# Guoxs/DODT

Measured on AMD Instinct MI355X. Metric: frame-pairs/sec (whole node) KITTI-shape tau=2, higher is better.
Workload: dtype f32

## Files before the change

dodt_amd/_lib.py:

```python
import ctypes as C
import os

_HERE = os.path.dirname(os.path.abspath(__file__))
LIB_PATH = os.environ.get('DODT_HIP_LIB') or os.path.join(_HERE, 'lib', 'libdodt_hip.so')

OK, ERR_INVALID, ERR_HIP, ERR_UNSUPPORTED = 0, 1, 2, 3
PTS_VELO_XYZI, PTS_CAM_3XN = 0, 1
EXTRACTOR_VGG_PYR = 0
EXTRACTOR_VGG = 1
EXTRACTOR_SHARED_GPU = 0x100
EXTRACTOR_BF16 = 0x200
EXTRACTOR_SPLIT = 0x400
FC_RELU = 1
FC_BF16 = 2
CONFLICT_RAISE, CONFLICT_NEXT_BEST = 0, 1


class DodtError(RuntimeError):
    pass


class BevParams(C.Structure):
    _fields_ = [
        ('point_format', C.c_int32),
        ('num_slices', C.c_int32),
        ('velo_to_cam', C.c_double * 12),
        ('p2', C.c_double * 12),
        ('im_w', C.c_double),
        ('im_h', C.c_double),
        ('plane', C.c_double * 4),
        ('extents', C.c_double * 6),
        ('voxel_size', C.c_double),
        ('height_lo', C.c_double),
        ('height_hi', C.c_double),
        ('occ_lo', C.c_double),
        ('occ_hi', C.c_double),
        ('has_pre_transform', C.c_int32),
        ('reserved_', C.c_int32),
        ('pre_translate', C.c_double * 3),
        ('pre_rotate', C.c_double * 9),
    ]


class LayerInfo(C.Structure):
    _fields_ = [('name', C.c_char * 32), ('kernel', C.c_char * 48), ('launches', C.c_int32),
                ('items', C.c_int32), ('flops_direct', C.c_double), ('flops_executed', C.c_double),
                ('bytes', C.c_double), ('ms', C.c_float), ('reserved_', C.c_int32)]


_vp = C.c_void_p
_i = C.c_int
_f = C.c_float
_d = C.c_double
_pi32 = C.c_void_p
_pf = C.c_void_p
_hf = C.c_void_p

SIGNATURES = {
    'dodt_version': (_i, []),
    'dodt_last_error': (C.c_char_p, []),
    'dodt_ctx_create': (_i, [_i, C.POINTER(_vp)]),
    'dodt_mark': (_i, [_vp, _i]),
    'dodt_ctx_wait_mark': (_i, [_vp, _vp, _i]),
    'dodt_mark_elapsed': (_i, [_vp, _i, _vp, _i, C.POINTER(_f)]),
    'dodt_ctx_create_high_priority': (_i, [_i, C.POINTER(_vp)]),
    'dodt_ctx_create_on_stream': (_i, [_i, _vp, C.POINTER(_vp)]),
    'dodt_ctx_destroy': (_i, [_vp]),
    'dodt_ctx_sync': (_i, [_vp]),
    'dodt_ctx_wait_for': (_i, [_vp, _vp]),
    'dodt_malloc': (_i, [_vp, C.c_size_t, C.POINTER(_vp)]),
    'dodt_free': (_i, [_vp, _vp]),
    'dodt_memcpy_h2d': (_i, [_vp, _vp, _vp, C.c_size_t]),
    'dodt_memcpy_d2h': (_i, [_vp, _vp, _vp, C.c_size_t]),
    'dodt_memset': (_i, [_vp, _vp, _i, C.c_size_t]),
    'dodt_pinned_alloc': (_i, [_vp, C.c_size_t, C.POINTER(_vp)]),
    'dodt_pinned_free': (_i, [_vp, _vp]),
    'dodt_memcpy_h2d_async': (_i, [_vp, _vp, _vp, C.c_size_t]),
    'dodt_fetch_i32_begin': (_i, [_vp, _pi32, _i, _i]),
    'dodt_fetch_i32_end': (_i, [_vp, _i, C.POINTER(C.c_int32), _i]),
    'dodt_timer_start': (_i, [_vp]),
    'dodt_timer_stop': (_i, [_vp, C.POINTER(_f)]),
    'dodt_bev_slices': (_i, [_vp, _vp, _i, C.POINTER(BevParams), _pf, _vp]),
    'dodt_bev_status': (_i, [_vp, C.POINTER(_i)]),
    'dodt_bev_support_mask': (_i, [C.POINTER(BevParams), _i, _vp, _i, _i]),
    'dodt_anchor_filter': (_i, [_vp, _vp, _i, _i, _pi32, _i, _i, _pi32, _pi32]),
    'dodt_project_anchors_f64': (_i, [_vp, _vp, _pi32, _i, _pi32,
                                      C.POINTER(_d), C.POINTER(_d), _d, _d,
                                      _pf, _pf, _pf]),
    'dodt_project_anchors_f32': (_i, [_vp, _pf, _i, _pi32, C.POINTER(_f),
                                      C.POINTER(_f), _f, _f, _pf, _pf, _pf]),
    'dodt_img_preprocess': (_i, [_vp, _vp, _i, _i, _i, _i, _i,
                                 C.POINTER(_f), _pf]),
    'dodt_conv_mode': (_i, []),
    'dodt_extractor_create': (_i, [_vp, _i, _i, _i, _i, _i, _i,
                                   C.POINTER(_vp)]),
    'dodt_extractor_destroy': (_i, [_vp]),
    'dodt_extractor_set_layer': (_i, [_vp, C.c_char_p, _vp, _i, _i, _i, _i,
                                      _vp, _vp, _vp]),
    'dodt_extractor_input': (_i, [_vp, C.POINTER(_vp), C.POINTER(C.c_longlong)]),
    'dodt_extractor_forward': (_i, [_vp, _pf, _pf, _pf]),
    'dodt_extractor_forward_padded': (_i, [_vp, _pf, _pf, _pf]),
    'dodt_extractor_set_input': (_i, [_vp, _pf]),
    'dodt_extractor_set_input_support': (_i, [_vp, _vp, _i, _i, C.POINTER(C.c_longlong)]),
    'dodt_extractor_set_frame_tables': (_i, [_vp, _i, C.POINTER(_i)]),
    'dodt_extractor_frame_items': (_i, [_vp, C.POINTER(_i), _i]),
    'dodt_extractor_frame_split': (_i, [_vp, C.POINTER(_i), C.POINTER(_i), _i]),
    'dodt_extractor_store_bytes': (C.c_longlong, [_vp]),
    'dodt_frame_tables_host': (_i, [_vp, _i, _i, _i, _i, _i, _i, _vp, _i, _vp, _vp, C.POINTER(_i)]),
    'dodt_frame_restore_host': (_i, [_vp, _i, _i, _i, _i, _i, _i, _i, _i, _i, _vp, _vp, _vp, _vp]),
    'dodt_frame_lists_host': (_i, [_vp, _i, _i, _i, _i, _i, _i, _vp, _i, _vp, _vp, C.POINTER(_i), _vp, C.POINTER(_i)]),
    'dodt_extractor_read_activation': (_i, [_vp, C.c_char_p, _vp,
                                            C.POINTER(_i), C.POINTER(_i),
                                            C.POINTER(_i)]),
    'dodt_extractor_output_shape': (_i, [_vp, C.POINTER(_i), C.POINTER(_i), C.POINTER(_i)]),
    'dodt_extractor_first_layers_folded': (_i, [_vp]),
    'dodt_extractor_flops': (_d, [_vp]),
    'dodt_extractor_mfma_flops': (_d, [_vp]),
    'dodt_extractor_bytes': (_d, [_vp]),
    'dodt_extractor_layer_count': (_i, [_vp]),
    'dodt_extractor_forward_timed': (_i, [_vp, _pf, _pf, _pf, C.POINTER(LayerInfo), _i]),
    'dodt_crop_and_resize': (_i, [_vp, _pf, _i, _i, _i, _pf, _i, _pi32, _i, _i,
                                  _pf]),
    'dodt_crop_and_resize_strided': (_i, [_vp, _pf, _i, _i, _i, _pf, _i, _pi32, _i, _i, _pf,
                                          C.c_longlong]),
    'dodt_correlation': (_i, [_vp, _pf, _pf, _i, _i, _i, _i, _i, _i, _pf]),
    'dodt_mean_fusion': (_i, [_vp, _pf, _pf, _i, _pi32, _i, _pf]),
    'dodt_fc_create': (_i, [_vp, _i, _i, _hf, _hf, _i, C.POINTER(_vp)]),
    'dodt_fc_create_ex': (_i, [_vp, _i, _i, _hf, _hf, _i, C.POINTER(_vp)]),
    'dodt_fc_destroy': (_i, [_vp]),
    'dodt_fc_forward': (_i, [_vp, _vp, _pf, _pf, _i, _i, _pi32, _pf, _i]),
    'dodt_fc_forward_split': (_i, [_vp, _vp, _pf, _i, _i, _pi32, _i, C.POINTER(_i), C.POINTER(_vp)]),
    'dodt_fc_flops': (_d, [_vp, _i]),
    'dodt_fc_bf16_row_elems': (_i, [_vp]),
    'dodt_fc_forward_bf16': (_i, [_vp, _vp, _vp, _i, _i, _pi32, _vp, _i, _i]),
    'dodt_fc_forward_split_bf16': (_i, [_vp, _vp, _vp, _i, _i, _pi32, _i, C.POINTER(_i), C.POINTER(_vp)]),
    'dodt_rows_to_bf16': (_i, [_vp, _pf, _pf, _i, _pi32, _i, _i, _vp, _i]),
    'dodt_nms': (_i, [_vp, _pf, _pf, _i, _pi32, _i, _f, _pi32, _pi32]),
    'dodt_offset_to_anchor': (_i, [_vp, _pf, _pf, _i, _pi32, _pf]),
    'dodt_softmax_fg': (_i, [_vp, _pf, _i, _pi32, _pf]),
    'dodt_rpn_decode': (_i, [_vp, _pf, _pf, _pf, _i, _pi32, C.POINTER(_f), _pf, _pf, _pf]),
    'dodt_gather_project': (_i, [_vp, _pf, _pi32, _i, _pi32, C.POINTER(_f), C.POINTER(_f), _f, _f, _pf, _pf, _pf]),
    'dodt_final_decode': (_i, [_vp, _pf, _pf, _pf, _pf, _i, _pi32, C.POINTER(_f), C.POINTER(_f),
                               _pf, _pf, _pf, _pf, _pf, _pf]),
    'dodt_gather_rows': (_i, [_vp, _pf, _i, _pi32, _i, _pi32, _pf]),
    'dodt_max_fg_logit': (_i, [_vp, _pf, _i, _i, _pi32, _pf]),
    'dodt_pack_detections': (_i, [_vp, _pf, _pf, _pf, _pf, _pi32, _pi32, _i, _f, _pf, _pi32]),
    'dodt_angle_vector_to_orientation': (_i, [_vp, _pf, _i, _pi32, _pf]),
    'dodt_box_4c_decode': (_i, [_vp, _pf, _pf, _i, _pi32, C.POINTER(_f),
                                C.POINTER(_f), _pf, _pf, _pf]),
    'dodt_comm_unique_id': (_i, [_vp]),
    'dodt_comm_create': (_i, [_vp, _i, _i, _vp, C.POINTER(_vp)]),
    'dodt_comm_destroy': (_i, [_vp]),
    'dodt_comm_attach': (_i, [_vp, _vp]),
    'dodt_comm_rank': (_i, [_vp, C.POINTER(_i), C.POINTER(_i)]),
    'dodt_comm_set_late_peer': (_i, [_vp, _d]),
    'dodt_all_gather_records': (_i, [_vp, _vp, _i, _pf, _pi32, _i, _i, _i, _i, _pf, _pi32]),
    'dodt_comm_join': (_i, [_vp, _i, _vp]),
    'dodt_comm_sync': (_i, [_vp]),
    'dodt_comm_barrier': (_i, [_vp]),
    'dodt_comm_max_f64': (_i, [_vp, C.POINTER(_d)]),
    'dodt_three_d_iou_matrix': (_i, [_vp, _vp, _i, _vp, _i, _vp]),
    'dodt_interpolate_pairs': (_i, [_vp, _vp, _i, _pi32, _i, _i, _i, _d, _i, _vp, C.POINTER(_d), _i, _vp,
                                    _pi32, _pi32]),
    'dodt_track_state_bytes': (_i, [_i, C.POINTER(C.c_size_t)]),
    'dodt_track_reset': (_i, [_vp, _vp, _i]),
    'dodt_track_flush': (_i, [_vp, _vp, _d, _i]),
    'dodt_track_encode': (_i, [_vp, _vp, _i, _pi32, _i, _i, C.POINTER(_d), _d, _d, _d, _pf, _pf, _pi32]),
    'dodt_track_pairs': (_i, [_vp, _vp, _vp, _i, _pi32, _i, _i, C.POINTER(_d), _d, _d, _d, _d, _d, _i]),
    'dodt_track_encoded': (_i, [_vp, _vp, _pf, _pf, _pi32, _i, _i, _d, _d, _i]),
}
COMM_ID_BYTES = 128

_lib = None


def load():
    global _lib
    if _lib is not None:
        return _lib
    if not os.path.exists(LIB_PATH):
        raise DodtError(
            'libdodt_hip.so not found at %s -- build it with '
            '`make -C dodt_amd/csrc` (there is no CPU fallback)' % LIB_PATH)
    lib = C.CDLL(LIB_PATH)
    for name, (res, args) in SIGNATURES.items():
        fn = getattr(lib, name)
        fn.restype = res
        fn.argtypes = args
    _lib = lib
    return lib


def check(rc, what=''):
    if rc == OK:
        return
    msg = load().dodt_last_error().decode('utf-8', 'replace')
    if rc == ERR_INVALID:
        raise ValueError(msg or what)
    raise DodtError('%s: %s (status %d)' % (what, msg, rc))
```

dodt_amd/csrc/anchors.hip:

```cpp
#include "common.h"

namespace {

__device__ __forceinline__ int box_count(const uint32_t* __restrict__ occ, int wpr, int x1,
                                         int z1, int x2, int z2, int thr) {
    int cnt = 0;
    if (x2 <= x1) return 0;
    const int w0 = x1 >> 5, w1 = (x2 - 1) >> 5;
    for (int z = z1; z < z2; ++z) {
        for (int w = w0; w <= w1; ++w) {
            uint32_t word = occ[z * wpr + w];
            const int lo = (w == w0) ? (x1 & 31) : 0;
            const int hi = (w == w1) ? ((x2 - 1) & 31) : 31;
            uint32_t m = (hi == 31 ? 0xFFFFFFFFu : ((1u << (hi + 1)) - 1u)) & ~((1u << lo) - 1u);
            cnt += __popc(word & m);
        }
        if (cnt >= thr) return cnt;
    }
    return cnt;
}

constexpr int kMaskBlock = 64;
__global__ void __launch_bounds__(kMaskBlock)
anchor_mask_kernel(const uint32_t* __restrict__ occ, int wpr, int nx, int nz,
                   const int4* __restrict__ cells, int n, int thr,
                   uint8_t* __restrict__ mask, int* __restrict__ block_counts) {
    const int i = blockIdx.x * blockDim.x + threadIdx.x;
    int keep = 0;
    if (i < n) {
        int4 b = cells[i];
        const int x1 = min(max(b.x, 0), nx), z1 = min(max(b.y, 0), nz);
        const int x2 = min(max(b.z, 0), nx), z2 = min(max(b.w, 0), nz);
        keep = box_count(occ, wpr, x1, z1, x2, z2, thr) >= thr;
        mask[i] = (uint8_t)keep;
    }
    const int total = __popcll(__ballot(keep));
    if (threadIdx.x == 0) block_counts[blockIdx.x] = total;
}

__global__ void __launch_bounds__(256)
anchor_compact_kernel(const uint8_t* __restrict__ mask, const int* __restrict__ block_counts,
                      int n, int* __restrict__ keep_idx, int* __restrict__ count_out) {
    __shared__ int s_part[256];
    __shared__ int s_wave[4];
    const int tid = threadIdx.x;
    int part = 0;
    for (int j = tid; j < (int)blockIdx.x * (256 / kMaskBlock); j += 256) part += block_counts[j];
    s_part[tid] = part;
    __syncthreads();
    for (int s = 128; s > 0; s >>= 1) {
        if (tid < s) s_part[tid] += s_part[tid + s];
        __syncthreads();
    }
    const int block_off = s_part[0];
    const int i = blockIdx.x * 256 + tid;
    const int keep = (i < n) ? mask[i] : 0;
    const unsigned long long bal = __ballot(keep);
    const int lane = tid & 63, wave = tid >> 6;
    const int before = __popcll(bal & ((1ull << lane) - 1ull));
    if (lane == 0) s_wave[wave] = __popcll(bal);
    __syncthreads();
    int wave_off = 0;
    for (int w = 0; w < wave; ++w) wave_off += s_wave[w];
    if (keep) keep_idx[block_off + wave_off + before] = i;
    if (blockIdx.x == gridDim.x - 1 && tid == 0)
        *count_out = block_off + s_wave[0] + s_wave[1] + s_wave[2] + s_wave[3];
}

struct ProjParams64 {
    double x_min, x_max, z_min, z_max;
    double p[12];
    double im_w, im_h;
};

__device__ __forceinline__ void proj_corner64(const double* p, double x, double y, double z,
                                              double& u, double& v) {
    const double un = fma(p[2], z, fma(p[1], y, p[0] * x)) + p[3];
    const double vn = fma(p[6], z, fma(p[5], y, p[4] * x)) + p[7];
    const double w = fma(p[10], z, fma(p[9], y, p[8] * x)) + p[11];
    u = un / w;
    v = vn / w;
}

__global__ void __launch_bounds__(256)
project_f64_kernel(const double* __restrict__ anchors, const int* __restrict__ idx, int n,
                   const int* __restrict__ d_n, const ProjParams64 P,
                   float* __restrict__ bev_norm, float* __restrict__ img_norm,
                   float* __restrict__ anchors_f32) {
    const int i = blockIdx.x * blockDim.x + threadIdx.x;
    const int lim = d_n ? min(*d_n, n) : n;
    if (i >= lim) return;
    const int row = idx ? idx[i] : i;
    const double* a = anchors + (size_t)row * 6;
    const double x = a[0], y = a[1], z = a[2], dx = a[3], dy = a[4], dz = a[5];
    if (anchors_f32) {
        float* o = anchors_f32 + (size_t)i * 6;
        o[0] = (float)x; o[1] = (float)y; o[2] = (float)z;
        o[3] = (float)dx; o[4] = (float)dy; o[5] = (float)dz;
    }
    const double hx = dx / 2.0, hz = dz / 2.0;
    if (bev_norm) {
        const double xr = P.x_max - P.x_min, zr = P.z_max - P.z_min;
        const double x1 = (x - hx) - P.x_min, x2 = (x + hx) - P.x_min;
        const double z1 = (P.z_max - (z + hz)) - P.z_min, z2 = (P.z_max - (z - hz)) - P.z_min;
        float* o = bev_norm + (size_t)i * 4;
        o[0] = (float)(z1 / zr); o[1] = (float)(x1 / xr);
        o[2] = (float)(z2 / zr); o[3] = (float)(x2 / xr);
    }
    if (img_norm) {
        double umin = 1e300, umax = -1e300, vmin = 1e300, vmax = -1e300;
        const double xs[2] = {x + hx, x - hx};
        const double ys[2] = {y, y - dy};
        const double zs[2] = {z + hz, z - hz};
#pragma unroll
        for (int k = 0; k < 8; ++k) {
            double u, v;
            proj_corner64(P.p, xs[(k >> 1) & 1], ys[k >> 2], zs[((k + 1) >> 1) & 1], u, v);
            umin = (u < umin || u != u) ? u : umin; umax = (u > umax || u != u) ? u : umax;
            vmin = (v < vmin || v != v) ? v : vmin; vmax = (v > vmax || v != v) ? v : vmax;
        }
        float* o = img_norm + (size_t)i * 4;
        o[0] = (float)(vmin / P.im_h); o[1] = (float)(umin / P.im_w);
        o[2] = (float)(vmax / P.im_h); o[3] = (float)(umax / P.im_w);
    }
}

struct ProjParams32 {
    float x_min, x_max, z_min, z_max;
    float p[12];
    float im_w, im_h;
};

__device__ __forceinline__ void bev_box32(float x, float z, float dx, float dz,
                                          const ProjParams32& P, float& x1, float& z1,
                                          float& x2, float& z2) {
    const float hx = dx / 2.0f, hz = dz / 2.0f;
    x1 = (x - hx) - P.x_min;
    x2 = (x + hx) - P.x_min;
    z1 = (P.z_max - (z + hz)) - P.z_min;
    z2 = (P.z_max - (z - hz)) - P.z_min;
}

__device__ __forceinline__ void project_f32_elem(int i, float x, float y, float z, float dx, float dy, float dz,
                                                 const ProjParams32& P, float* __restrict__ bev,
                                                 float* __restrict__ bev_norm_tf, float* __restrict__ img_norm_tf) {
    float x1, z1, x2, z2;
    bev_box32(x, z, dx, dz, P, x1, z1, x2, z2);
    if (bev) {
        float* o = bev + (size_t)i * 4;
        o[0] = x1; o[1] = z1; o[2] = x2; o[3] = z2;
    }
    if (bev_norm_tf) {
        const float xr = P.x_max - P.x_min, zr = P.z_max - P.z_min;
        float* o = bev_norm_tf + (size_t)i * 4;
        o[0] = z1 / zr; o[1] = x1 / xr; o[2] = z2 / zr; o[3] = x2 / xr;
    }
    if (img_norm_tf) {
        const float hx = dx / 2.0f, hz = dz / 2.0f;
        const float xs[2] = {x + hx, x - hx};
        const float ys[2] = {y, y - dy};
        const float zs[2] = {z + hz, z - hz};
        float umin = 3.0e38f, umax = -3.0e38f, vmin = 3.0e38f, vmax = -3.0e38f;
#pragma unroll
        for (int k = 0; k < 8; ++k) {
            const float cx = xs[(k >> 1) & 1], cy = ys[k >> 2], cz = zs[((k + 1) >> 1) & 1];
            const float un = ((P.p[0] * cx + P.p[1] * cy) + P.p[2] * cz) + P.p[3];
            const float vn = ((P.p[4] * cx + P.p[5] * cy) + P.p[6] * cz) + P.p[7];
            const float w = ((P.p[8] * cx + P.p[9] * cy) + P.p[10] * cz) + P.p[11];
            const float u = un / w, v = vn / w;
            umin = fminf(umin, u); umax = fmaxf(umax, u);
            vmin = fminf(vmin, v); vmax = fmaxf(vmax, v);
        }
        float* o = img_norm_tf + (size_t)i * 4;
        o[0] = vmin / P.im_h; o[1] = umin / P.im_w; o[2] = vmax / P.im_h; o[3] = umax / P.im_w;
    }
}

__global__ void __launch_bounds__(256)
project_f32_kernel(const float* __restrict__ anchors, int n, const int* __restrict__ d_n,
                   const ProjParams32 P, float* __restrict__ bev, float* __restrict__ bev_norm_tf,
                   float* __restrict__ img_norm_tf) {
    const int i = blockIdx.x * blockDim.x + threadIdx.x;
    const int lim = d_n ? min(*d_n, n) : n;
    if (i >= lim) return;
    const float* a = anchors + (size_t)i * 6;
    project_f32_elem(i, a[0], a[1], a[2], a[3], a[4], a[5], P, bev, bev_norm_tf, img_norm_tf);
}

__device__ __forceinline__ void offset_to_anchor_elem(const float* __restrict__ a, const float* __restrict__ t, float o[6]) {
    o[0] = (t[0] * a[3]) + a[0];
    o[1] = (t[1] * a[4]) + a[1];
    o[2] = (t[2] * a[5]) + a[2];
    o[3] = expf(logf(a[3]) + t[3]);
    o[4] = expf(logf(a[4]) + t[4]);
    o[5] = expf(logf(a[5]) + t[5]);
}

__global__ void __launch_bounds__(256)
offset_to_anchor_kernel(const float* __restrict__ anchors, const float* __restrict__ off, int n,
                        const int* __restrict__ d_n, float* __restrict__ out) {
    const int i = blockIdx.x * blockDim.x + threadIdx.x;
    const int lim = d_n ? min(*d_n, n) : n;
    if (i >= lim) return;
    float o[6];
    offset_to_anchor_elem(anchors + (size_t)i * 6, off + (size_t)i * 6, o);
#pragma unroll
    for (int k = 0; k < 6; ++k) out[(size_t)i * 6 + k] = o[k];
}

__device__ __forceinline__ float softmax_fg_elem(float l0, float l1) {
    const float m = fmaxf(l0, l1);
    const float e0 = expf(l0 - m), e1 = expf(l1 - m);
    return e1 / (e0 + e1);
}

__global__ void __launch_bounds__(256)
softmax_fg_kernel(const float* __restrict__ logits, int n, const int* __restrict__ d_n,
                  float* __restrict__ out) {
    const int i = blockIdx.x * blockDim.x + threadIdx.x;
    const int lim = d_n ? min(*d_n, n) : n;
    if (i >= lim) return;
    out[i] = softmax_fg_elem(logits[2 * (size_t)i], logits[2 * (size_t)i + 1]);
}

__global__ void __launch_bounds__(256)
rpn_decode_kernel(const float* __restrict__ anchors, const float* __restrict__ off, const float* __restrict__ logits,
                  int n, const int* __restrict__ d_n, const ProjParams32 P, float* __restrict__ regressed,
                  float* __restrict__ bev_norm_tf, float* __restrict__ scores) {
    const int i = blockIdx.x * blockDim.x + threadIdx.x;
    const int lim = d_n ? min(*d_n, n) : n;
    if (i >= lim) return;
    float o[6];
    offset_to_anchor_elem(anchors + (size_t)i * 6, off + (size_t)i * 6, o);
#pragma unroll
    for (int k = 0; k < 6; ++k) regressed[(size_t)i * 6 + k] = o[k];
    project_f32_elem(i, o[0], o[1], o[2], o[3], o[4], o[5], P, nullptr, bev_norm_tf, nullptr);
    scores[i] = softmax_fg_elem(logits[2 * (size_t)i], logits[2 * (size_t)i + 1]);
}

__global__ void __launch_bounds__(256)
gather_project_kernel(const float* __restrict__ src, const int* __restrict__ idx, int n, const int* __restrict__ d_n,
                      const ProjParams32 P, float* __restrict__ rows, float* __restrict__ bev_norm_tf,
                      float* __restrict__ img_norm_tf) {
    const int i = blockIdx.x * blockDim.x + threadIdx.x;
    const int lim = d_n ? min(*d_n, n) : n;
    if (i >= lim) return;
    const float* a = src + (size_t)idx[i] * 6;
    float o[6];
#pragma unroll
    for (int k = 0; k < 6; ++k) { o[k] = a[k]; rows[(size_t)i * 6 + k] = o[k]; }
    project_f32_elem(i, o[0], o[1], o[2], o[3], o[4], o[5], P, nullptr, bev_norm_tf, img_norm_tf);
}

__global__ void __launch_bounds__(256)
gather_rows_kernel(const float* __restrict__ src, int width, const int* __restrict__ idx, int n,
                   const int* __restrict__ d_n, float* __restrict__ out) {
    const int t = blockIdx.x * blockDim.x + threadIdx.x;
    const int lim = d_n ? min(*d_n, n) : n;
    const int i = t / width, c = t - i * width;
    if (i >= lim) return;
    out[(size_t)i * width + c] = src[(size_t)idx[i] * width + c];
}

__global__ void __launch_bounds__(256)
max_fg_logit_kernel(const float* __restrict__ logits, int n_cls, int n,
                    const int* __restrict__ d_n, float* __restrict__ out) {
    const int i = blockIdx.x * blockDim.x + threadIdx.x;
    const int lim = d_n ? min(*d_n, n) : n;
    if (i >= lim) return;
    float m = logits[(size_t)i * n_cls + 1];
    for (int c = 2; c < n_cls; ++c) m = fmaxf(m, logits[(size_t)i * n_cls + c]);
    out[i] = m;
}

__device__ __forceinline__ void orientation_correct(float b[7], float ori) {
    const float kPi = (float)M_PI, kTwoPi = (float)(2.0 * M_PI);
    const float q1 = (float)(0.25 * M_PI), q2 = (float)(0.50 * M_PI), q3 = (float)(0.75 * M_PI);
    float diff = b[6] - ori;
    if (diff < -kPi) diff += kTwoPi;
    if (diff > kPi) diff -= kTwoPi;
    const bool pos = q1 < diff && diff < q3;
    const bool neg = -q1 > diff && diff > -q3;
    if (pos || neg) {
        const float l = b[3];
        b[3] = b[4];
        b[4] = l;
    }
    if (pos) b[6] += q2;
    if (neg) b[6] -= q2;
    if (fabsf(diff) >= q3) b[6] += kPi;
    if (b[6] > kPi) b[6] -= kTwoPi;
}

__global__ void __launch_bounds__(256)
pack_detections_kernel(const float* __restrict__ boxes_3d, const float* __restrict__ scores,
                       const float* __restrict__ orientations, const float* __restrict__ corr,
                       const int* __restrict__ sel, const int* __restrict__ d_count, int max_det,
                       float frame_mark, float* __restrict__ rec, int* __restrict__ count_out) {
    const int t = blockIdx.x * blockDim.x + threadIdx.x;
    const int cnt = min(*d_count, max_det);
    if (t == 0) *count_out = cnt;
    if (t >= max_det * 17) return;
    const int row = t / 17, col = t - row * 17;
    float v = 0.0f;
    if (row < cnt) {
        const int src = sel[row];
        if (col == 7) v = scores[src];
        else if (col == 16) v = frame_mark;
        else if (col < 7 || (col >= 9 && corr)) {
            float b[7];
#pragma unroll
            for (int k = 0; k < 7; ++k) b[k] = boxes_3d[(size_t)src * 7 + k];
            if (orientations) orientation_correct(b, orientations[src]);
            if (col >= 9) {
                b[0] += corr[(size_t)src * 3 + 0];
                b[2] += corr[(size_t)src * 3 + 1];
                b[6] += corr[(size_t)src * 3 + 2];
            }
            const int c = col < 7 ? col : col - 9;
#pragma unroll
            for (int k = 0; k < 7; ++k)
                if (k == c) v = b[k];
        }
    }
    rec[t] = v;
}

__global__ void __launch_bounds__(256)
angle_vector_to_orientation_kernel(const float* __restrict__ vec, int n,
                                   const int* __restrict__ d_n, float* __restrict__ out) {
    const int i = blockIdx.x * blockDim.x + threadIdx.x;
    if (d_n) n = min(n, *d_n);
    if (i < n) out[i] = atan2f(vec[2 * i + 1], vec[2 * i]);
}

__device__ __forceinline__ void box_info32(float vx, float vz, float mag, const float* px,
                                           const float* pz, float mx, float mz, float& cx,
                                           float& cz, float& len, float& wid, float& ry) {
    const float nx = vx / mag, nz = vz / mag;
    const float ox = -nz, oz = nx;
    float lmin = 3.0e38f, lmax = -3.0e38f, wmin = 3.0e38f, wmax = -3.0e38f;
#pragma unroll
    for (int k = 0; k < 4; ++k) {
        const float rx = px[k] - mx, rz = pz[k] - mz;
        const float l = rx * nx + rz * nz;
        const float w = rx * ox + rz * oz;
        lmin = fminf(lmin, l); lmax = fmaxf(lmax, l);
        wmin = fminf(wmin, w); wmax = fmaxf(wmax, w);
    }
    len = lmax - lmin;
    wid = wmax - wmin;
    const float wdiff = wmax + wmin;
    ry = -atan2f(vz, vx);
    const float half = (lmin + lmax);
    cx = (mx + (nx * half) / 2.0f) + ox * wdiff;
    cz = (mz + (nz * half) / 2.0f) + oz * wdiff;
}

struct DecodeParams {
    float a, b, c, d;
    float x_min, x_max, z_min, z_max;
};

__device__ __forceinline__ void box_4c_decode_elem(int i, const float* __restrict__ top_anchors,
                                                   const float* __restrict__ offsets, const DecodeParams& P,
                                                   float* __restrict__ boxes_3d, float* __restrict__ pred_anchors,
                                                   float* __restrict__ bev_tf) {
    const float* a = top_anchors + (size_t)i * 6;
    const float half_pi = (float)(M_PI / 2);
    float bx = a[0], by = a[1], bz = a[2];
    float bl = a[3], bw = a[5], bh = a[4], bry = 0.0f;
    if (bw > bl) { const float t = bl; bl = bw; bw = t; bry = -half_pi; }
    float ortho = rintf(bry / half_pi) * half_pi;
    float co = fabsf(cosf(ortho)), si = fabsf(sinf(ortho));
    const float dimx = bl * co + bw * si, dimy = bh, dimz = bw * co + bl * si;
    const float hx = dimx / 2, hz = dimz / 2;
    const float diff = bry - ortho;
    const float cd = cosf(diff), sd = sinf(diff);
    const float xs[4] = {hx, hx, -hx, -hx};
    const float zs[4] = {hz, -hz, -hz, hz};
    float px[4], pz[4];
    const float* t = offsets + (size_t)i * 10;
#pragma unroll
    for (int k = 0; k < 4; ++k) {
        px[k] = ((cd * xs[k] + sd * zs[k]) + bx) + t[k];
        pz[k] = (((-sd) * xs[k] + cd * zs[k]) + bz) + t[4 + k];
    }
    const float gy = -((P.a * bx + P.c * bz) + P.d) / P.b;
    const float h1 = (gy - by) + t[8];
    const float h2 = ((gy - by) + dimy) + t[9];
    const float m12x = (px[0] + px[1]) / 2.0f, m12z = (pz[0] + pz[1]) / 2.0f;
    const float m23x = (px[1] + px[2]) / 2.0f, m23z = (pz[1] + pz[2]) / 2.0f;
    const float m34x = (px[2] + px[3]) / 2.0f, m34z = (pz[2] + pz[3]) / 2.0f;
    const float m14x = (px[0] + px[3]) / 2.0f, m14z = (pz[0] + pz[3]) / 2.0f;
    const float vax = m12x - m34x, vaz = m12z - m34z;
    const float vbx = m14x - m23x, vbz = m14z - m23z;
    const float ma = sqrtf(vax * vax + vaz * vaz), mb = sqrtf(vbx * vbx + vbz * vbz);
    float cax, caz, la, wa, ra, cbx, cbz, lb, wb, rb;
    box_info32(vax, vaz, ma, px, pz, m34x, m34z, cax, caz, la, wa, ra);
    box_info32(vbx, vbz, mb, px, pz, m23x, m23z, cbx, cbz, lb, wb, rb);
    const float fa = (ma > mb) ? 1.0f : 0.0f, fb = 1.0f - fa;
    const float cx = cax * fa + cbx * fb, cz = caz * fa + cbz * fb;
    const float len = la * fa + lb * fb, wid = wa * fa + wb * fb, ry = ra * fa + rb * fb;
    const float gy2 = -((P.a * cx + P.c * cz) + P.d) / P.b;
    const float cy = gy2 - h1, hgt = h2 - h1;
    if (boxes_3d) {
        float* o = boxes_3d + (size_t)i * 7;
        o[0] = cx; o[1] = cy; o[2] = cz; o[3] = len; o[4] = wid; o[5] = hgt; o[6] = ry;
    }
    ortho = rintf(ry / half_pi) * half_pi;
    co = fabsf(cosf(ortho));
    si = fabsf(sinf(ortho));
    const float adx = len * co + wid * si, adz = wid * co + len * si;
    if (pred_anchors) {
        float* o = pred_anchors + (size_t)i * 6;
        o[0] = cx; o[1] = cy; o[2] = cz; o[3] = adx; o[4] = hgt; o[5] = adz;
    }
    if (bev_tf) {
        const float ahx = adx / 2.0f, ahz = adz / 2.0f;
        const float x1 = (cx - ahx) - P.x_min, x2 = (cx + ahx) - P.x_min;
        const float z1 = (P.z_max - (cz + ahz)) - P.z_min, z2 = (P.z_max - (cz - ahz)) - P.z_min;
        float* o = bev_tf + (size_t)i * 4;
        o[0] = z1; o[1] = x1; o[2] = z2; o[3] = x2;
    }
}

__global__ void __launch_bounds__(256)
box_4c_decode_kernel(const float* __restrict__ top_anchors, const float* __restrict__ offsets,
                     int n, const int* __restrict__ d_n, const DecodeParams P,
                     float* __restrict__ boxes_3d, float* __restrict__ pred_anchors,
                     float* __restrict__ bev_tf) {
    const int i = blockIdx.x * blockDim.x + threadIdx.x;
    const int lim = d_n ? min(*d_n, n) : n;
    if (i >= lim) return;
    box_4c_decode_elem(i, top_anchors, offsets, P, boxes_3d, pred_anchors, bev_tf);
}

__global__ void __launch_bounds__(256)
final_decode_kernel(const float* __restrict__ top_anchors, const float* __restrict__ offsets,
                    const float* __restrict__ cls_logits, const float* __restrict__ angle_vec, int n,
                    const int* __restrict__ d_n, const DecodeParams P, float* __restrict__ boxes_3d,
                    float* __restrict__ pred_anchors, float* __restrict__ bev_tf, float* __restrict__ nms_scores,
                    float* __restrict__ det_scores, float* __restrict__ orientations) {
    const int i = blockIdx.x * blockDim.x + threadIdx.x;
    const int lim = d_n ? min(*d_n, n) : n;
    if (i >= lim) return;
    box_4c_decode_elem(i, top_anchors, offsets, P, boxes_3d, pred_anchors, bev_tf);
    const float l0 = cls_logits[2 * (size_t)i], l1 = cls_logits[2 * (size_t)i + 1];
    nms_scores[i] = l1;
    det_scores[i] = softmax_fg_elem(l0, l1);
    if (orientations) orientations[i] = atan2f(angle_vec[2 * i + 1], angle_vec[2 * i]);
}

}

extern "C" {

int dodt_anchor_filter(dodt_ctx* ctx, const uint32_t* d_occ_bits, int nx, int nz,
                       const int32_t* d_anchor_cells, int n_anchors, int density_threshold,
                       int32_t* d_keep_idx_out, int32_t* d_count_out) {
    DODT_REQUIRE(ctx && d_occ_bits && d_anchor_cells && d_keep_idx_out && d_count_out,
                 "dodt_anchor_filter: NULL argument");
    DODT_REQUIRE(nx > 0 && nz > 0 && n_anchors >= 0, "dodt_anchor_filter: bad sizes");
    if (n_anchors == 0) {
        DODT_HIP_CHECK(hipMemsetAsync(d_count_out, 0, sizeof(int32_t), ctx->stream));
        return DODT_OK;
    }
    const int blocks = dodt::ceil_div(n_anchors, 256), mask_blocks = dodt::ceil_div(n_anchors, kMaskBlock);
    const size_t mask_bytes = dodt::align_up((size_t)n_anchors, 256);
    int rc = ctx->anchor_ws.reserve(mask_bytes + (size_t)mask_blocks * sizeof(int));
    if (rc) return rc;
    uint8_t* mask = reinterpret_cast<uint8_t*>(ctx->anchor_ws.ptr);
    int* block_counts = reinterpret_cast<int*>(mask + mask_bytes);
    hipLaunchKernelGGL(anchor_mask_kernel, dim3(mask_blocks), dim3(kMaskBlock), 0, ctx->stream, d_occ_bits,
                       dodt::ceil_div(nx, 32), nx, nz,
                       reinterpret_cast<const int4*>(d_anchor_cells), n_anchors,
                       density_threshold, mask, block_counts);
    DODT_LAUNCH_CHECK();
    hipLaunchKernelGGL(anchor_compact_kernel, dim3(blocks), dim3(256), 0, ctx->stream, mask,
                       block_counts, n_anchors, d_keep_idx_out, d_count_out);
    DODT_LAUNCH_CHECK();
    return DODT_OK;
}

int dodt_project_anchors_f64(dodt_ctx* ctx, const double* d_anchors, const int32_t* d_idx, int n,
                             const int32_t* d_n, const double bev_extents[4],
                             const double p2[12], double im_w, double im_h,
                             float* d_bev_norm_out, float* d_img_norm_out,
                             float* d_anchors_f32_out) {
    DODT_REQUIRE(ctx && d_anchors && bev_extents && p2, "dodt_project_anchors_f64: NULL argument");
    if (n <= 0) return DODT_OK;
    ProjParams64 P;
    P.x_min = bev_extents[0]; P.x_max = bev_extents[1];
    P.z_min = bev_extents[2]; P.z_max = bev_extents[3];
    for (int k = 0; k < 12; ++k) P.p[k] = p2[k];
    P.im_w = im_w; P.im_h = im_h;
    hipLaunchKernelGGL(project_f64_kernel, dim3(dodt::ceil_div(n, 256)), dim3(256), 0,
                       ctx->stream, d_anchors, d_idx, n, d_n, P, d_bev_norm_out, d_img_norm_out,
                       d_anchors_f32_out);
    DODT_LAUNCH_CHECK();
    return DODT_OK;
}

int dodt_project_anchors_f32(dodt_ctx* ctx, const float* d_anchors, int n, const int32_t* d_n,
                             const float bev_extents[4], const float p2[12], float im_w,
                             float im_h, float* d_bev_out, float* d_bev_norm_tf_out,
                             float* d_img_norm_tf_out) {
    DODT_REQUIRE(ctx && d_anchors && bev_extents && p2, "dodt_project_anchors_f32: NULL argument");
    if (n <= 0) return DODT_OK;
    ProjParams32 P;
    P.x_min = bev_extents[0]; P.x_max = bev_extents[1];
    P.z_min = bev_extents[2]; P.z_max = bev_extents[3];
    for (int k = 0; k < 12; ++k) P.p[k] = p2[k];
    P.im_w = im_w; P.im_h = im_h;
    hipLaunchKernelGGL(project_f32_kernel, dim3(dodt::ceil_div(n, 256)), dim3(256), 0,
                       ctx->stream, d_anchors, n, d_n, P, d_bev_out, d_bev_norm_tf_out,
                       d_img_norm_tf_out);
    DODT_LAUNCH_CHECK();
    return DODT_OK;
}

int dodt_rpn_decode(dodt_ctx* ctx, const float* d_anchors, const float* d_offsets, const float* d_logits2, int n,
                    const int32_t* d_n, const float bev_extents[4], float* d_regressed_out,
                    float* d_bev_norm_tf_out, float* d_scores_out) {
    DODT_REQUIRE(ctx && d_anchors && d_offsets && d_logits2 && bev_extents && d_regressed_out && d_bev_norm_tf_out &&
                     d_scores_out, "dodt_rpn_decode: NULL argument");
    if (n <= 0) return DODT_OK;
    ProjParams32 P = {};
    P.x_min = bev_extents[0]; P.x_max = bev_extents[1];
    P.z_min = bev_extents[2]; P.z_max = bev_extents[3];
    hipLaunchKernelGGL(rpn_decode_kernel, dim3(dodt::ceil_div(n, 256)), dim3(256), 0, ctx->stream, d_anchors,
                       d_offsets, d_logits2, n, d_n, P, d_regressed_out, d_bev_norm_tf_out, d_scores_out);
    DODT_LAUNCH_CHECK();
    return DODT_OK;
}

int dodt_gather_project(dodt_ctx* ctx, const float* d_src, const int32_t* d_idx, int n, const int32_t* d_n,
                        const float bev_extents[4], const float p2[12], float im_w, float im_h,
                        float* d_rows_out, float* d_bev_norm_tf_out, float* d_img_norm_tf_out) {
    DODT_REQUIRE(ctx && d_src && d_idx && bev_extents && p2 && d_rows_out && d_bev_norm_tf_out && d_img_norm_tf_out,
                 "dodt_gather_project: NULL argument");
    if (n <= 0) return DODT_OK;
    ProjParams32 P;
    P.x_min = bev_extents[0]; P.x_max = bev_extents[1];
    P.z_min = bev_extents[2]; P.z_max = bev_extents[3];
    for (int k = 0; k < 12; ++k) P.p[k] = p2[k];
    P.im_w = im_w; P.im_h = im_h;
    hipLaunchKernelGGL(gather_project_kernel, dim3(dodt::ceil_div(n, 256)), dim3(256), 0, ctx->stream, d_src, d_idx,
                       n, d_n, P, d_rows_out, d_bev_norm_tf_out, d_img_norm_tf_out);
    DODT_LAUNCH_CHECK();
    return DODT_OK;
}

int dodt_final_decode(dodt_ctx* ctx, const float* d_top_anchors, const float* d_offsets, const float* d_cls_logits2,
                      const float* d_angle_vectors, int n, const int32_t* d_n, const float plane[4],
                      const float bev_extents[4], float* d_boxes_3d_out, float* d_pred_anchors_out,
                      float* d_bev_tf_out, float* d_nms_scores_out, float* d_det_scores_out,
                      float* d_orientations_out) {
    DODT_REQUIRE(ctx && d_top_anchors && d_offsets && d_cls_logits2 && plane && bev_extents && d_nms_scores_out &&
                     d_det_scores_out && (d_angle_vectors != nullptr) == (d_orientations_out != nullptr),
                 "dodt_final_decode: bad argument");
    if (n <= 0) return DODT_OK;
    DecodeParams P;
    P.a = plane[0]; P.b = plane[1]; P.c = plane[2]; P.d = plane[3];
    P.x_min = bev_extents[0]; P.x_max = bev_extents[1];
    P.z_min = bev_extents[2]; P.z_max = bev_extents[3];
    hipLaunchKernelGGL(final_decode_kernel, dim3(dodt::ceil_div(n, 256)), dim3(256), 0, ctx->stream, d_top_anchors,
                       d_offsets, d_cls_logits2, d_angle_vectors, n, d_n, P, d_boxes_3d_out, d_pred_anchors_out,
                       d_bev_tf_out, d_nms_scores_out, d_det_scores_out, d_orientations_out);
    DODT_LAUNCH_CHECK();
    return DODT_OK;
}

int dodt_offset_to_anchor(dodt_ctx* ctx, const float* d_anchors, const float* d_offsets, int n,
                          const int32_t* d_n, float* d_out) {
    DODT_REQUIRE(ctx && d_anchors && d_offsets && d_out, "dodt_offset_to_anchor: NULL argument");
    if (n <= 0) return DODT_OK;
    hipLaunchKernelGGL(offset_to_anchor_kernel, dim3(dodt::ceil_div(n, 256)), dim3(256), 0,
                       ctx->stream, d_anchors, d_offsets, n, d_n, d_out);
    DODT_LAUNCH_CHECK();
    return DODT_OK;
}

int dodt_softmax_fg(dodt_ctx* ctx, const float* d_logits2, int n, const int32_t* d_n,
                    float* d_scores_out) {
    DODT_REQUIRE(ctx && d_logits2 && d_scores_out, "dodt_softmax_fg: NULL argument");
    if (n <= 0) return DODT_OK;
    hipLaunchKernelGGL(softmax_fg_kernel, dim3(dodt::ceil_div(n, 256)), dim3(256), 0,
                       ctx->stream, d_logits2, n, d_n, d_scores_out);
    DODT_LAUNCH_CHECK();
    return DODT_OK;
}

int dodt_gather_rows(dodt_ctx* ctx, const float* d_src, int width, const int32_t* d_idx, int n,
                     const int32_t* d_n, float* d_out) {
    DODT_REQUIRE(ctx && d_src && d_idx && d_out && width > 0, "dodt_gather_rows: bad argument");
    if (n <= 0) return DODT_OK;
    hipLaunchKernelGGL(gather_rows_kernel, dim3(dodt::ceil_div(n * width, 256)), dim3(256), 0,
                       ctx->stream, d_src, width, d_idx, n, d_n, d_out);
    DODT_LAUNCH_CHECK();
    return DODT_OK;
}

int dodt_max_fg_logit(dodt_ctx* ctx, const float* d_logits, int n_cls, int n, const int32_t* d_n,
                      float* d_scores_out) {
    DODT_REQUIRE(ctx && d_logits && d_scores_out && n_cls >= 2, "dodt_max_fg_logit: bad argument");
    if (n <= 0) return DODT_OK;
    hipLaunchKernelGGL(max_fg_logit_kernel, dim3(dodt::ceil_div(n, 256)), dim3(256), 0,
                       ctx->stream, d_logits, n_cls, n, d_n, d_scores_out);
    DODT_LAUNCH_CHECK();
    return DODT_OK;
}

int dodt_pack_detections(dodt_ctx* ctx, const float* d_boxes_3d, const float* d_scores,
                         const float* d_orientations, const float* d_corr_offsets,
                         const int32_t* d_sel, const int32_t* d_count, int max_det,
                         float frame_mark, float* d_rec_out, int32_t* d_count_out) {
    DODT_REQUIRE(ctx && d_boxes_3d && d_scores && d_sel && d_count && d_rec_out && d_count_out &&
                     max_det > 0,
                 "dodt_pack_detections: bad argument");
    hipLaunchKernelGGL(pack_detections_kernel, dim3(dodt::ceil_div(max_det * 17, 256)), dim3(256),
                       0, ctx->stream, d_boxes_3d, d_scores, d_orientations, d_corr_offsets, d_sel,
                       d_count, max_det, frame_mark, d_rec_out, d_count_out);
    DODT_LAUNCH_CHECK();
    return DODT_OK;
}

int dodt_angle_vector_to_orientation(dodt_ctx* ctx, const float* d_angle_vectors, int n,
                                     const int32_t* d_n, float* d_orientations_out) {
    DODT_REQUIRE(ctx && d_angle_vectors && d_orientations_out,
                 "dodt_angle_vector_to_orientation: NULL argument");
    if (n <= 0) return DODT_OK;
    hipLaunchKernelGGL(angle_vector_to_orientation_kernel, dim3(dodt::ceil_div(n, 256)), dim3(256),
                       0, ctx->stream, d_angle_vectors, n, d_n, d_orientations_out);
    DODT_LAUNCH_CHECK();
    return DODT_OK;
}

int dodt_box_4c_decode(dodt_ctx* ctx, const float* d_top_anchors, const float* d_offsets, int n,
                       const int32_t* d_n, const float plane[4], const float bev_extents[4],
                       float* d_boxes_3d_out, float* d_pred_anchors_out, float* d_bev_tf_out) {
    DODT_REQUIRE(ctx && d_top_anchors && d_offsets && plane && bev_extents,
                 "dodt_box_4c_decode: NULL argument");
    if (n <= 0) return DODT_OK;
    DecodeParams P;
    P.a = plane[0]; P.b = plane[1]; P.c = plane[2]; P.d = plane[3];
    P.x_min = bev_extents[0]; P.x_max = bev_extents[1];
    P.z_min = bev_extents[2]; P.z_max = bev_extents[3];
    hipLaunchKernelGGL(box_4c_decode_kernel, dim3(dodt::ceil_div(n, 256)), dim3(256), 0,
                       ctx->stream, d_top_anchors, d_offsets, n, d_n, P, d_boxes_3d_out,
                       d_pred_anchors_out, d_bev_tf_out);
    DODT_LAUNCH_CHECK();
    return DODT_OK;
}

}
```

dodt_amd/csrc/correlation.hip:

```cpp
#include <algorithm>
#include <mutex>
#include <type_traits>
#include <vector>

#include "common.h"
#include "lds_dma.h"

namespace {

constexpr int kTW = 16;
constexpr int kTH = 32;
constexpr int kC = 32;
constexpr int kCH = 16;
constexpr int kPS = kCH + 4;

typedef float f32x4 __attribute__((ext_vector_type(4)));
typedef float f32x2 __attribute__((ext_vector_type(2)));

template <int S2, int CH, int WGS>
__global__ void __launch_bounds__(256, WGS)
correlation_kernel(const float* __restrict__ A, const float* __restrict__ B, int H, int W,
                   int d, int pad, int OH, int OW, int tiles_x, int n_tiles, float* __restrict__ out) {
    constexpr int r = 2, R = r * S2, GW = 2 * r + 1, K = GW * GW, PS = CH + 4;
    constexpr int PW = kTW + 2 * R, PH = kTH + 2 * R;
    static_assert(S2 == 2, "a lane's pixel pair (y, y + 2) shares neighbourhood rows only for stride_2 = 2");
    extern __shared__ __attribute__((aligned(16))) float smem[];
    const int tid = threadIdx.x;
    const int per = (n_tiles + 7) / 8;
    const int tile = (blockIdx.x % 8) * per + blockIdx.x / 8;
    if (tile >= n_tiles) return;
    const int oy0 = (tile / tiles_x) * kTH, ox0 = (tile % tiles_x) * kTW;
    const int shift = d - pad;
    const int l5 = tid & 31;
    const bool grp_a = l5 < 4 || (l5 >= 12 && l5 < 16) || (l5 >= 20 && l5 < 28);
    const int lx = grp_a ? (l5 < 4 ? l5 : l5 < 16 ? l5 - 8 : l5 - 12)
                         : (l5 < 12 ? l5 - 4 : l5 < 20 ? l5 - 8 : l5 - 16);
    const int lr = (tid >> 5) * 2 + (grp_a ? 0 : 1);
    const int ly = 4 * (lr >> 1) + (lr & 1);
    f32x2 res[2][K];
#pragma unroll
    for (int px = 0; px < 2; ++px)
#pragma unroll
        for (int k = 0; k < K; ++k) res[px][k] = f32x2{0.f, 0.f};
#pragma unroll 1
    for (int pass = 0; pass < kC / CH; ++pass) {
        if (pass) __syncthreads();
        f32x4 ah[2][CH / 4];
#pragma unroll
        for (int px = 0; px < 2; ++px) {
            const int ay = oy0 + ly + 2 * px + shift, ax = ox0 + lx + shift;
            const bool in = ay >= 0 && ay < H && ax >= 0 && ax < W;
#pragma unroll
            for (int q = 0; q < CH / 4; ++q) {
                ah[px][q] = f32x4{0.f, 0.f, 0.f, 0.f};
                if (in)
                    ah[px][q] = *reinterpret_cast<const f32x4*>(A + ((size_t)ay * W + ax) * kC + pass * CH + q * 4);
            }
        }
        constexpr int kQuads = PW * PH * (CH / 4), kTrips = (kQuads + 255) / 256, kGroup = kTrips < 8 ? kTrips : 8;
        int stid = tid;
        asm volatile("" : "+v"(stid));
#pragma unroll
        for (int g0 = 0; g0 < kTrips; g0 += kGroup) {
            f32x4 stage[kGroup];
#pragma unroll
            for (int i = 0; i < kGroup; ++i) {
                const int t = stid + 256 * (g0 + i);
                const int q = t % (CH / 4), p = t / (CH / 4);
                const int py = p / PW, pxl = p - py * PW;
                const int gy = oy0 + shift - R + py, gx = ox0 + shift - R + pxl;
                stage[i] = f32x4{0.f, 0.f, 0.f, 0.f};
                if (g0 + i < kTrips && t < kQuads && gy >= 0 && gy < H && gx >= 0 && gx < W)
                    stage[i] = *reinterpret_cast<const f32x4*>(B + ((size_t)gy * W + gx) * kC + pass * CH + q * 4);
            }
#pragma unroll
            for (int i = 0; i < kGroup; ++i) {
                const int t = stid + 256 * (g0 + i);
                const int q = t % (CH / 4), p = t / (CH / 4);
                if (g0 + i < kTrips && t < kQuads)
                    *reinterpret_cast<f32x4*>(smem + p * PS + q * 4) = stage[i];
            }
            __builtin_amdgcn_sched_barrier(0);
        }
        __syncthreads();
#pragma unroll
        for (int tr = 0; tr < GW + 1; ++tr) {
#pragma unroll
            for (int j = 0; j < GW; ++j) {
                const float* b = smem + (ly * PW + lx) * PS + (S2 * tr * PW + S2 * j) * PS;
                f32x4 bv[CH / 4];
#pragma unroll
                for (int q = 0; q < CH / 4; ++q) bv[q] = *reinterpret_cast<const f32x4*>(b + q * 4);
#pragma unroll
                for (int px = 0; px < 2; ++px) {
                    const int krow = tr - px;
                    if (krow < 0 || krow >= GW) continue;
                    f32x2 sum = res[px][krow * GW + j];
#pragma unroll
                    for (int q = 0; q < CH / 4; ++q) {
                        const f32x4 av = ah[px][q];
                        sum = __builtin_elementwise_fma(f32x2{av[0], av[1]}, f32x2{bv[q][0], bv[q][1]}, sum);
                        sum = __builtin_elementwise_fma(f32x2{av[2], av[3]}, f32x2{bv[q][2], bv[q][3]}, sum);
                    }
                    res[px][krow * GW + j] = sum;
                }
            }
            __builtin_amdgcn_sched_barrier(0);
        }
    }
    __syncthreads();
#pragma unroll
    for (int px = 0; px < 2; ++px)
#pragma unroll
        for (int k = 0; k < K; ++k)
            smem[((ly + 2 * px) * kTW + lx) * K + k] = (res[px][k][0] + res[px][k][1]) * (1.0f / (float)kC);
    __syncthreads();
    constexpr int kRow = kTW * K;
    if ((OW * K) % 4 == 0 && kRow % 4 == 0 && ox0 + kTW <= OW) {
        for (int t = tid; t < kTH * (kRow / 4); t += 256) {
            const int row = t / (kRow / 4), off = t - row * (kRow / 4);
            const int y = oy0 + row;
            if (y < OH)
                *reinterpret_cast<f32x4*>(out + ((size_t)y * OW + ox0) * K + off * 4) =
                    *reinterpret_cast<const f32x4*>(smem + row * kRow + off * 4);
        }
    } else {
        for (int t = tid; t < kTH * kRow; t += 256) {
            const int row = t / kRow, off = t - row * kRow;
            const int y = oy0 + row, x = ox0 + off / K;
            if (y < OH && x < OW) out[((size_t)y * OW + ox0) * K + off] = smem[t];
        }
    }
}

constexpr int kSpT = 16;
constexpr int kSpR = 4;
constexpr int kSpP = kSpT + 2 * kSpR;
constexpr int kSpLds = kSpP * kSpP * kC * 4;

template <int HALVES>
__global__ void __launch_bounds__(256 * HALVES, 2 * HALVES)
correlation_sp_kernel(const float* __restrict__ A, const float* __restrict__ B, int H, int W, int d, int pad,
                      int OH, int OW, const int* __restrict__ tile_list, int n_tiles, float* __restrict__ out,
                      int* __restrict__ stamps) {
    constexpr int GW = 5, K = GW * GW, S2 = 2, QH = kC / 4 / HALVES;
    constexpr int NW = 4 * HALVES;
    extern __shared__ __attribute__((aligned(16))) float smem[];
    const int tid = threadIdx.x;
    const bool stamp = stamps != nullptr && blockIdx.x == 9 && tid == 0;
    int n_stamp = 0;
#define CORR_STAMP(i) do { if (stamp && n_stamp < 6) stamps[n_stamp * 8 + (i)] = (int)__builtin_amdgcn_s_memrealtime(); } while (0)
    const int per = (n_tiles + 7) / 8;
    const int xcd = blockIdx.x % 8, wg = blockIdx.x / 8, stride = gridDim.x / 8;
    const int first = xcd * per, last = min(first + per, n_tiles);
    const int shift = d - pad;
    const int lane = tid & 63, wave = tid >> 6;
    const int half = HALVES == 2 ? lane >> 5 : 0;
    const int l5 = lane & 31;
    const bool grp_a = l5 < 4 || (l5 >= 12 && l5 < 16) || (l5 >= 20 && l5 < 28);
    const int lx = grp_a ? (l5 < 4 ? l5 : l5 < 16 ? l5 - 8 : l5 - 12)
                         : (l5 < 12 ? l5 - 4 : l5 < 20 ? l5 - 8 : l5 - 16);
    const int ly = (HALVES == 2 ? wave * 2 : (tid >> 5) * 2) + (grp_a ? 0 : 1);
    const dodt::i32x4_t rsrc = dodt::make_rsrc(B, (unsigned)((size_t)H * W * kC * 4));

    auto load_a = [&](int oy0, int ox0, f32x4 (&ah)[QH]) {
        const int ay = oy0 + ly + shift, ax = ox0 + lx + shift;
        const bool in = ay >= 0 && ay < H && ax >= 0 && ax < W;
#pragma unroll
        for (int q = 0; q < QH; ++q) {
            ah[q] = f32x4{0.f, 0.f, 0.f, 0.f};
            if (in) ah[q] = *reinterpret_cast<const f32x4*>(A + ((size_t)ay * W + ax) * kC + (half * QH + q) * 4);
        }
    };
    constexpr int kOutCopies = (kSpT * kSpT * K * 4 + 1023) / 1024;
    auto stage_b = [&](int oy0, int ox0, auto part) {
        constexpr int PART = decltype(part)::value;
        int slane = lane;
        asm volatile("" : "+v"(slane));
#pragma unroll
        for (int k = 0; k < (kSpP * kSpP * 8 / 64) / NW; ++k) {
            const int j = wave + NW * k;
            if (PART == 1 && j < kOutCopies) continue;
            if (PART == 2 && j >= kOutCopies) continue;
            const int s = j * 64 + slane;
            const int p = s >> 3, q = (s & 7) ^ ((p >> 1) & 7);
            const int py = p / kSpP, px = p - py * kSpP;
            const int gy = oy0 + shift - kSpR + py, gx = ox0 + shift - kSpR + px;
            const bool ok = gy >= 0 && gy < H && gx >= 0 && gx < W;
            dodt::blds16(rsrc, ok ? ((gy * W + gx) * kC + q * 4) * 4 : dodt::kOob, 0, smem + j * 256);
        }
    };
    using All = std::integral_constant<int, 0>;
    using Early = std::integral_constant<int, 1>;
    using Late = std::integral_constant<int, 2>;
    int slot = first + wg;
    if (slot >= last) return;
    int tile = tile_list[slot];
    f32x4 ah[QH];
    load_a((tile >> 16) * kSpT, (tile & 0xffff) * kSpT, ah);
    stage_b((tile >> 16) * kSpT, (tile & 0xffff) * kSpT, All{});
    const int p0_lane = ly * kSpP + lx;
    while (true) {
        const int oy0 = (tile >> 16) * kSpT, ox0 = (tile & 0xffff) * kSpT;
        int p0 = p0_lane;
        asm volatile("" : "+v"(p0));
        const char* lane_base = reinterpret_cast<const char*>(smem) + p0 * (kC * 4);
        CORR_STAMP(0);
        __builtin_amdgcn_s_waitcnt(0);
        CORR_STAMP(1);
        __syncthreads();
        CORR_STAMP(2);
        const int nslot = slot + stride;
        const bool more = nslot < last;
        const int ntile = more ? tile_list[nslot] : 0;
        f32x4 an[QH];
        if (more) load_a((ntile >> 16) * kSpT, (ntile & 0xffff) * kSpT, an);
        f32x2 res[K];
#pragma unroll
        for (int k = 0; k < K; ++k) res[k] = f32x2{0.f, 0.f};
        f32x4 bv[2][QH];
        auto read_step = [&](int st, f32x4 (&dst)[QH]) {
            const int j = st / GW, i = st % GW;
            const int sj = ((p0 >> 1) + j) & 7;
#pragma unroll
            for (int q = 0; q < QH; ++q)
                dst[q] = *reinterpret_cast<const f32x4*>(lane_base + (((half * QH + q) ^ sj) << 4) + S2 * j * (kC * 4) +
                                                         S2 * i * kSpP * (kC * 4));
        };
        read_step(0, bv[0]);
#pragma unroll
        for (int st = 0; st < K; ++st) {
            if (st + 1 < K) read_step(st + 1, bv[(st + 1) & 1]);
            __builtin_amdgcn_sched_barrier(0);
            const int j = st / GW, i = st % GW;
            float s0 = res[i * GW + j][0], s1 = res[i * GW + j][1];
#pragma unroll
            for (int q = 0; q < QH; ++q) {
                s0 = __builtin_fmaf(ah[q][0], bv[st & 1][q][0], s0);
                s1 = __builtin_fmaf(ah[q][1], bv[st & 1][q][1], s1);
                s0 = __builtin_fmaf(ah[q][2], bv[st & 1][q][2], s0);
                s1 = __builtin_fmaf(ah[q][3], bv[st & 1][q][3], s1);
            }
            res[i * GW + j] = f32x2{s0, s1};
            __builtin_amdgcn_sched_barrier(0);
        }
        float tot[K];
#pragma unroll
        for (int k = 0; k < K; ++k) {
            tot[k] = res[k][0] + res[k][1];
            if (HALVES == 2) {
                const float other = __shfl_xor(tot[k], 32, 64);
                tot[k] = half == 0 ? tot[k] + other : other + tot[k];
            }
        }
#pragma unroll
        for (int k = 0; k < K; ++k) asm volatile("" : "+v"(tot[k]));
        CORR_STAMP(3);
        __syncthreads();
        CORR_STAMP(4);
        if (more) stage_b((ntile >> 16) * kSpT, (ntile & 0xffff) * kSpT, Early{});
        if (half == 0) {
#pragma unroll
            for (int k = 0; k < K; ++k) smem[(ly * kSpT + lx) * K + k] = tot[k] * (1.0f / (float)kC);
        }
        __syncthreads();
        CORR_STAMP(5);
        {
            constexpr int kRow = kSpT * K;
            if ((OW * K) % 4 == 0 && ox0 + kSpT <= OW) {
                for (int t = tid; t < kSpT * (kRow / 4); t += 256 * HALVES) {
                    const int row = t / (kRow / 4), off = t - row * (kRow / 4);
                    const int y = oy0 + row;
                    if (y < OH)
                        *reinterpret_cast<f32x4*>(out + ((size_t)y * OW + ox0) * K + off * 4) =
                            *reinterpret_cast<const f32x4*>(smem + row * kRow + off * 4);
                }
            } else {
                for (int t = tid; t < kSpT * kRow; t += 256 * HALVES) {
                    const int row = t / kRow, off = t - row * kRow;
                    const int y = oy0 + row, x = ox0 + off / K;
                    if (y < OH && x < OW) out[((size_t)y * OW + ox0) * K + off] = smem[t];
                }
            }
        }
        CORR_STAMP(6);
        if (!more) break;
        __syncthreads();
        stage_b((ntile >> 16) * kSpT, (ntile & 0xffff) * kSpT, Late{});
        CORR_STAMP(7);
        ++n_stamp;
        slot = nslot;
        tile = ntile;
#pragma unroll
        for (int q = 0; q < QH; ++q) ah[q] = an[q];
    }
#undef CORR_STAMP
}

struct SpTileList {
    int device, tiles_y, tiles_x;
    int* d_list;
};
int sp_tile_list(dodt_ctx* ctx, int tiles_y, int tiles_x, const int** out) {
    static std::mutex mu;
    static std::vector<SpTileList> cache;
    std::lock_guard<std::mutex> lock(mu);
    for (const SpTileList& e : cache)
        if (e.device == ctx->device && e.tiles_y == tiles_y && e.tiles_x == tiles_x) {
            *out = e.d_list;
            return DODT_OK;
        }
    std::vector<int> h;
    h.reserve((size_t)tiles_y * tiles_x);
    for (int by = 0; by < tiles_y; by += 8)
        for (int bx = 0; bx < tiles_x; bx += 8)
            for (int ty = by; ty < std::min(by + 8, tiles_y); ++ty)
                for (int tx = bx; tx < std::min(bx + 8, tiles_x); ++tx) h.push_back(ty << 16 | tx);
    int* d = nullptr;
    DODT_HIP_CHECK(hipMalloc(&d, h.size() * sizeof(int)));
    DODT_HIP_CHECK(hipMemcpy(d, h.data(), h.size() * sizeof(int), hipMemcpyHostToDevice));
    cache.push_back(SpTileList{ctx->device, tiles_y, tiles_x, d});
    *out = d;
    return DODT_OK;
}

constexpr int kT = 16;


__global__ void __launch_bounds__(256, 3)
correlation_generic_kernel(const float* __restrict__ A, const float* __restrict__ B, int H, int W,
                   int d, int pad, int s2, int r, int OH, int OW, float* __restrict__ out) {
    extern __shared__ __attribute__((aligned(16))) float smem[];
    const int R = r * s2;
    const int PT = kT + 2 * R;
    const int gw = 2 * r + 1, K = gw * gw;
    const int tid = threadIdx.x;
    const int oy0 = blockIdx.y * kT, ox0 = blockIdx.x * kT;
    const int shift = d - pad;
    const int ly = tid / kT, lx = tid % kT;
    const int oy = oy0 + ly, ox = ox0 + lx;
    const int ay = oy + shift, ax = ox + shift;
    f32x4 a[kC / 4];
    const bool a_in = ay >= 0 && ay < H && ax >= 0 && ax < W;
#pragma unroll
    for (int q = 0; q < kC / 4; ++q) {
        a[q] = f32x4{0.f, 0.f, 0.f, 0.f};
        if (a_in) a[q] = *reinterpret_cast<const f32x4*>(A + ((size_t)ay * W + ax) * kC + q * 4);
    }
    float res[32];
#pragma unroll
    for (int k = 0; k < 32; ++k) res[k] = 0.0f;
#pragma unroll
    for (int pass = 0; pass < kC / kCH; ++pass) {
        if (pass) __syncthreads();
        for (int t = tid; t < PT * PT * (kCH / 4); t += 256) {
            const int q = t % (kCH / 4), p = t / (kCH / 4);
            const int py = p / PT, px = p - py * PT;
            const int gy = oy0 + shift - R + py, gx = ox0 + shift - R + px;
            f32x4 v = {0.f, 0.f, 0.f, 0.f};
            if (gy >= 0 && gy < H && gx >= 0 && gx < W)
                v = *reinterpret_cast<const f32x4*>(B + ((size_t)gy * W + gx) * kC + pass * kCH +
                                                    q * 4);
            *reinterpret_cast<f32x4*>(smem + p * kPS + q * 4) = v;
        }
        __syncthreads();
        for (int k = 0; k < K; ++k) {
            const int s2p = (k / gw - r) * s2, s2o = (k % gw - r) * s2;
            const float* b = smem + ((ly + R + s2p) * PT + (lx + R + s2o)) * kPS;
            float sum = res[k];
#pragma unroll
            for (int q = 0; q < kCH / 4; ++q) {
                const f32x4 bv = *reinterpret_cast<const f32x4*>(b + q * 4);
                const f32x4 av = a[pass * (kCH / 4) + q];
                sum += av[0] * bv[0];
                sum += av[1] * bv[1];
                sum += av[2] * bv[2];
                sum += av[3] * bv[3];
            }
            res[k] = sum;
        }
    }
    for (int k = 0; k < K; ++k) res[k] = res[k] / (float)kC;
    __syncthreads();
    for (int k = 0; k < K; ++k) smem[tid * K + k] = res[k];
    __syncthreads();
    for (int t = tid; t < kT * kT * K; t += 256) {
        const int row = t / (kT * K), off = t - row * (kT * K);
        const int y = oy0 + row, x = ox0 + off / K;
        if (y < OH && x < OW) out[((size_t)y * OW + ox0) * K + off] = smem[t];
    }
}

}

extern "C" int dodt_correlation(dodt_ctx* ctx, const float* d_a, const float* d_b, int H, int W,
                                int C, int max_displacement, int stride_2, int pad,
                                float* d_out) {
    DODT_REQUIRE(ctx && d_a && d_b && d_out, "dodt_correlation: NULL argument");
    DODT_REQUIRE(C == kC, "dodt_correlation: C = %d, only %d channels are supported", C, kC);
    DODT_REQUIRE(H > 0 && W > 0 && max_displacement >= 0 && stride_2 >= 1 && pad >= 0,
                 "dodt_correlation: bad sizes");
    const int r = max_displacement / stride_2;
    const int K = (2 * r + 1) * (2 * r + 1);
    DODT_REQUIRE(K <= 32, "dodt_correlation: %d displacement channels exceed 32", K);
    const int OH = H + 2 * pad - 2 * max_displacement, OW = W + 2 * pad - 2 * max_displacement;
    DODT_REQUIRE(OH >= 1 && OW >= 1, "dodt_correlation: empty output");
    if (!(stride_2 == 2 && r == 2)) {
        const int PT = kT + 2 * r * stride_2;
        size_t glds = (size_t)PT * PT * kPS * sizeof(float);
        const size_t lds_out = (size_t)kT * kT * K * sizeof(float);
        if (glds < lds_out) glds = lds_out;
        DODT_REQUIRE(glds <= 160 * 1024, "dodt_correlation: neighbourhood does not fit LDS");
        static bool gprepared = false;
        if (!gprepared) {
            DODT_HIP_CHECK(hipFuncSetAttribute(reinterpret_cast<const void*>(&correlation_generic_kernel),
                                               hipFuncAttributeMaxDynamicSharedMemorySize, 160 * 1024));
            gprepared = true;
        }
        hipLaunchKernelGGL(correlation_generic_kernel, dim3(dodt::ceil_div(OW, kT), dodt::ceil_div(OH, kT)),
                           dim3(256), glds, ctx->stream, d_a, d_b, H, W, max_displacement, pad, stride_2, r, OH,
                           OW, d_out);
        DODT_LAUNCH_CHECK();
        return DODT_OK;
    }
    static const bool two_pass = getenv("DODT_CORR_TWO_PASS") && atoi(getenv("DODT_CORR_TWO_PASS")) != 0;
    if (!two_pass && (size_t)H * W * kC * 4 < (1ull << 31) && H < 65536 * kSpT && W < 65536 * kSpT) {
        const int ty = dodt::ceil_div(OH, kSpT), tx = dodt::ceil_div(OW, kSpT);
        const int* d_list = nullptr;
        if (int rc = sp_tile_list(ctx, ty, tx, &d_list)) return rc;
        static const int halves = getenv("DODT_CORR_HALVES") && atoi(getenv("DODT_CORR_HALVES")) == 2 ? 2 : 1;
        static bool prepared = false;
        if (!prepared) {
            DODT_HIP_CHECK(hipFuncSetAttribute(reinterpret_cast<const void*>(&correlation_sp_kernel<1>),
                                               hipFuncAttributeMaxDynamicSharedMemorySize, kSpLds));
            DODT_HIP_CHECK(hipFuncSetAttribute(reinterpret_cast<const void*>(&correlation_sp_kernel<2>),
                                               hipFuncAttributeMaxDynamicSharedMemorySize, kSpLds));
            prepared = true;
        }
        const int n = ty * tx;
        static const int grid_env = getenv("DODT_CORR_GRID") ? atoi(getenv("DODT_CORR_GRID")) : 0;
        int grid = grid_env > 0 ? grid_env / 8 * 8 : 2 * ctx->num_cus / 8 * 8;
        if (grid > 8 * dodt::ceil_div(n, 8)) grid = 8 * dodt::ceil_div(n, 8);
        static const bool want_stamps = getenv("DODT_CORR_STAMPS") != nullptr;
        static int* d_stamps = nullptr;
        if (want_stamps && !d_stamps) {
            DODT_HIP_CHECK(hipMalloc(&d_stamps, 64 * sizeof(int)));
            DODT_HIP_CHECK(hipMemset(d_stamps, 0, 64 * sizeof(int)));
        }
        if (halves == 2)
            hipLaunchKernelGGL(correlation_sp_kernel<2>, dim3(grid), dim3(512), kSpLds, ctx->stream,
                               d_a, d_b, H, W, max_displacement, pad, OH, OW, d_list, n, d_out, d_stamps);
        else
            hipLaunchKernelGGL(correlation_sp_kernel<1>, dim3(grid), dim3(256), kSpLds, ctx->stream,
                               d_a, d_b, H, W, max_displacement, pad, OH, OW, d_list, n, d_out, d_stamps);
        DODT_LAUNCH_CHECK();
        if (want_stamps) {
            int h[64];
            (void)hipStreamSynchronize(ctx->stream);
            (void)hipMemcpy(h, d_stamps, sizeof(h), hipMemcpyDeviceToHost);
            fprintf(stderr, "[dodt] correlation, workgroup 9, us per phase: wait copies | barrier | arithmetic | barrier | "
                            "early copies + outputs to LDS | stores | barrier + late copies\n");
            for (int t = 0; t < 4; ++t) {
                fprintf(stderr, "[dodt]   tile %d:", t);
                for (int k = 0; k < 7; ++k) fprintf(stderr, " %6.2f", (h[t * 8 + k + 1] - h[t * 8 + k]) / 100.0);
                fprintf(stderr, "   next tile's top +%.2f\n", (h[(t + 1) * 8] - h[t * 8]) / 100.0);
            }
        }
        return DODT_OK;
    }
    const int R = r * stride_2;
    const int tiles_x = dodt::ceil_div(OW, kTW), n_tiles = tiles_x * dodt::ceil_div(OH, kTH);
    auto go = [&](auto kernel, int CH) -> int {
        size_t lds = (size_t)(kTW + 2 * R) * (kTH + 2 * R) * (CH + 4) * sizeof(float);
        const size_t lds_out = (size_t)kTW * kTH * K * sizeof(float);
        if (lds < lds_out) lds = lds_out;
        static bool prepared = false;
        if (!prepared) {
            DODT_HIP_CHECK(hipFuncSetAttribute(reinterpret_cast<const void*>(kernel),
                                               hipFuncAttributeMaxDynamicSharedMemorySize, 160 * 1024));
            prepared = true;
        }
        hipLaunchKernelGGL(kernel, dim3(8 * dodt::ceil_div(n_tiles, 8)), dim3(256), lds, ctx->stream,
                           d_a, d_b, H, W, max_displacement, pad, OH, OW, tiles_x, n_tiles, d_out);
        return DODT_OK;
    };
    if (int rc = go(&correlation_kernel<2, 16, 2>, 16)) return rc;
    DODT_LAUNCH_CHECK();
    return DODT_OK;
}
```

dodt_amd/csrc/crop.hip:

```cpp
#include "common.h"

namespace {

template <int VEC>
__global__ void __launch_bounds__(256)
crop_kernel(const float* __restrict__ img, int H, int W, int C, const float* __restrict__ boxes,
            int n, const int* __restrict__ d_n, int ch, int cw, float* __restrict__ out,
            long long out_stride) {
    const int groups = C / VEC;
    const long long t = (long long)blockIdx.x * blockDim.x + threadIdx.x;
    const int lim = d_n ? min(*d_n, n) : n;
    const long long total = (long long)lim * ch * cw * groups;
    if (t >= total) return;
    const int g = (int)(t % groups);
    long long r = t / groups;
    const int ix = (int)(r % cw); r /= cw;
    const int iy = (int)(r % ch);
    const int b = (int)(r / ch);
    const float4 bx = reinterpret_cast<const float4*>(boxes)[b];
    const float y1 = bx.x, x1 = bx.y, y2 = bx.z, x2 = bx.w;
    const float hm1 = (float)(H - 1), wm1 = (float)(W - 1);
    const float hs = (ch > 1) ? (y2 - y1) * hm1 / (float)(ch - 1) : 0.0f;
    const float ws = (cw > 1) ? (x2 - x1) * wm1 / (float)(cw - 1) : 0.0f;
    const float in_y = (ch > 1) ? y1 * hm1 + (float)iy * hs : 0.5f * (y1 + y2) * hm1;
    const float in_x = (cw > 1) ? x1 * wm1 + (float)ix * ws : 0.5f * (x1 + x2) * wm1;
    float* o = out + (size_t)b * out_stride + (((size_t)iy * cw + ix) * C + (size_t)g * VEC);
    const bool ok = (in_y >= 0.0f) && (in_y <= hm1) && (in_x >= 0.0f) && (in_x <= wm1);
    if (!ok) {
#pragma unroll
        for (int k = 0; k < VEC; ++k) o[k] = 0.0f;
        return;
    }
    const int ty = (int)floorf(in_y), by = (int)ceilf(in_y);
    const int lx_i = (int)floorf(in_x), rx_i = (int)ceilf(in_x);
    const float ly = in_y - (float)ty, lx = in_x - (float)lx_i;
    const float* ptl = img + ((size_t)ty * W + lx_i) * C + (size_t)g * VEC;
    const float* ptr = img + ((size_t)ty * W + rx_i) * C + (size_t)g * VEC;
    const float* pbl = img + ((size_t)by * W + lx_i) * C + (size_t)g * VEC;
    const float* pbr = img + ((size_t)by * W + rx_i) * C + (size_t)g * VEC;
#pragma unroll
    for (int k = 0; k < VEC; ++k) {
        const float tl = ptl[k], tr = ptr[k], bl = pbl[k], br = pbr[k];
        const float top = tl + (tr - tl) * lx;
        const float bot = bl + (br - bl) * lx;
        o[k] = top + (bot - top) * ly;
    }
}

}

extern "C" int dodt_crop_and_resize(dodt_ctx* ctx, const float* d_image, int H, int W, int C,
                                    const float* d_boxes, int n, const int32_t* d_n, int crop_h,
                                    int crop_w, float* d_out) {
    return dodt_crop_and_resize_strided(ctx, d_image, H, W, C, d_boxes, n, d_n, crop_h, crop_w, d_out,
                                        (long long)crop_h * crop_w * C);
}

extern "C" int dodt_crop_and_resize_strided(dodt_ctx* ctx, const float* d_image, int H, int W, int C,
                                            const float* d_boxes, int n, const int32_t* d_n, int crop_h,
                                            int crop_w, float* d_out, long long out_box_stride) {
    DODT_REQUIRE(ctx && d_image && d_out && (n == 0 || d_boxes),
                 "dodt_crop_and_resize: NULL argument");
    DODT_REQUIRE(H > 0 && W > 0 && C > 0 && crop_h > 0 && crop_w > 0 && n >= 0,
                 "dodt_crop_and_resize: bad sizes");
    DODT_REQUIRE(out_box_stride >= (long long)crop_h * crop_w * C,
                 "dodt_crop_and_resize: output stride %lld shorter than a crop", out_box_stride);
    if (n == 0) return DODT_OK;
    const int vec = (C % 4 == 0 && out_box_stride % 4 == 0) ? 4 : 1;
    const long long total = (long long)n * crop_h * crop_w * (C / vec);
    const int blocks = (int)((total + 255) / 256);
    if (vec == 4)
        hipLaunchKernelGGL(crop_kernel<4>, dim3(blocks), dim3(256), 0, ctx->stream, d_image, H, W,
                           C, d_boxes, n, d_n, crop_h, crop_w, d_out, out_box_stride);
    else
        hipLaunchKernelGGL(crop_kernel<1>, dim3(blocks), dim3(256), 0, ctx->stream, d_image, H, W,
                           C, d_boxes, n, d_n, crop_h, crop_w, d_out, out_box_stride);
    DODT_LAUNCH_CHECK();
    return DODT_OK;
}
```

dodt_amd/ops.py:

```python
import ctypes as C
import os

import numpy as np

from dodt_amd import _lib


def _arr(ctype, values):
    values = [float(v) for v in np.asarray(values, dtype=np.float64).reshape(-1)]
    return (ctype * len(values))(*values)


def _p(a):
    return None if a is None else C.c_void_p(a.ptr)


def make_bev_params(cfg, velo_to_cam=None, p2=None, im_wh=None,
                    point_format=_lib.PTS_VELO_XYZI, ground_plane=None,
                    area_extents=None, voxel_size=None):
    bp = _lib.BevParams()
    bp.point_format = point_format
    bp.num_slices = int(cfg['num_slices'])
    m = np.zeros(12) if velo_to_cam is None else \
        np.asarray(velo_to_cam, dtype=np.float64).reshape(-1)[:12]
    p = np.zeros(12) if p2 is None else np.asarray(p2, dtype=np.float64).reshape(-1)
    bp.velo_to_cam = (C.c_double * 12)(*m)
    bp.p2 = (C.c_double * 12)(*p)
    bp.im_w, bp.im_h = (0.0, 0.0) if im_wh is None else (float(im_wh[0]), float(im_wh[1]))
    plane = cfg['ground_plane'] if ground_plane is None else ground_plane
    bp.plane = (C.c_double * 4)(*[float(v) for v in plane])
    ext = cfg['area_extents'] if area_extents is None else area_extents
    bp.extents = (C.c_double * 6)(*[float(v) for v in np.asarray(ext).reshape(-1)])
    bp.voxel_size = float(cfg['voxel_size'] if voxel_size is None else voxel_size)
    bp.height_lo = float(cfg['height_lo'])
    bp.height_hi = float(cfg['height_hi'])
    bp.occ_lo = float(cfg['anchor_filter_lo'])
    bp.occ_hi = float(cfg['anchor_filter_hi'])
    bp.has_pre_transform = 0
    return bp


def with_ego_motion(bev_params, trans, matrix):
    bp = _lib.BevParams.from_buffer_copy(bev_params)
    t = np.asarray(trans, np.float64).reshape(3)
    m = np.asarray(matrix, np.float64).reshape(9)
    bp.has_pre_transform = 1
    bp.pre_translate = (C.c_double * 3)(*t)
    bp.pre_rotate = (C.c_double * 9)(*m)
    return bp


def bev_slices(ctx, d_points, n_points, bev_params, d_bev_out, d_occ_bits=None):
    _lib.check(ctx.lib.dodt_bev_slices(ctx.handle, _p(d_points), int(n_points),
                                       C.byref(bev_params), _p(d_bev_out),
                                       _p(d_occ_bits)), 'dodt_bev_slices')


def bev_support_mask(bev_params, pad_top=0, lib=None):
    lib = lib or _lib.load()
    vs = bev_params.voxel_size
    ext = list(bev_params.extents)
    nx = int(np.ceil(ext[1] / vs - 1) - np.floor(ext[0] / vs) + 1)
    nz = int(np.ceil(ext[5] / vs - 1) - np.floor(ext[4] / vs) + 1)
    out = np.zeros((int(pad_top) + nz, nx), np.uint8)
    _lib.check(lib.dodt_bev_support_mask(C.byref(bev_params), int(pad_top), out.ctypes.data, out.shape[0],
                                         out.shape[1]), 'dodt_bev_support_mask')
    return out


def frame_tables_host(masks, layer, th, tw, items, prev=None, lib=None):
    lib = lib or _lib.load()
    masks = np.ascontiguousarray(masks, dtype=np.uint8)
    items = np.ascontiguousarray(items, dtype=np.int32).reshape(-1, 4)
    prev = None if prev is None else np.ascontiguousarray(prev, dtype=np.uint8)
    run = np.zeros((max(len(items), 1), 4), np.int32)
    n = C.c_int()
    _lib.check(lib.dodt_frame_tables_host(masks.ctypes.data, masks.shape[0], masks.shape[1], masks.shape[2], int(layer),
                                          int(th), int(tw), items.ctypes.data, len(items),
                                          None if prev is None else prev.ctypes.data, run.ctypes.data, C.byref(n)),
               'dodt_frame_tables_host')
    return run[:n.value].copy()


def frame_lists_host(masks, layer, th, tw, items, prev=None, lib=None):
    lib = lib or _lib.load()
    masks = np.ascontiguousarray(masks, dtype=np.uint8)
    items = np.ascontiguousarray(items, dtype=np.int32).reshape(-1, 4)
    prev = None if prev is None else np.ascontiguousarray(prev, dtype=np.uint8)
    run = np.zeros((max(len(items), 1), 4), np.int32)
    restore = np.zeros((max(len(items), 1), 4), np.int32)
    n, nr = C.c_int(), C.c_int()
    _lib.check(lib.dodt_frame_lists_host(masks.ctypes.data, masks.shape[0], masks.shape[1], masks.shape[2], int(layer),
                                         int(th), int(tw), items.ctypes.data, len(items),
                                         None if prev is None else prev.ctypes.data, run.ctypes.data, C.byref(n),
                                         restore.ctypes.data, C.byref(nr)),
               'dodt_frame_lists_host')
    return run[:n.value].copy(), restore[:nr.value].copy()


def frame_restore_host(item, f, th, tw, bn, ch0, dst, src, dst2=None, src2=None, pad_top=-1, lib=None):
    lib = lib or _lib.load()
    for a in (dst, src, dst2, src2):
        assert a is None or (a.dtype == np.float32 and a.flags.c_contiguous)
    item = np.ascontiguousarray(item, dtype=np.int32)
    if pad_top < 0:
        rows, cols, channels = dst.shape[2], dst.shape[3], dst.shape[1] * 8
    else:
        rows, cols, channels = dst.shape[1] + pad_top, dst.shape[2], dst.shape[3]
    _lib.check(lib.dodt_frame_restore_host(item.ctypes.data, int(f), int(th), int(tw), int(bn), int(ch0), rows, cols,
                                           channels, int(pad_top), dst.ctypes.data, src.ctypes.data,
                                           None if dst2 is None else dst2.ctypes.data,
                                           None if src2 is None else src2.ctypes.data), 'dodt_frame_restore_host')


def bev_status(ctx):
    f = C.c_int()
    _lib.check(ctx.lib.dodt_bev_status(ctx.handle, C.byref(f)), 'dodt_bev_status')
    return f.value


def anchor_filter(ctx, d_occ_bits, nx, nz, d_cells, n_anchors, d_keep_idx, d_count,
                  density_threshold=1):
    _lib.check(ctx.lib.dodt_anchor_filter(
        ctx.handle, _p(d_occ_bits), int(nx), int(nz), _p(d_cells), int(n_anchors),
        int(density_threshold), _p(d_keep_idx), _p(d_count)), 'dodt_anchor_filter')


def project_anchors_f64(ctx, d_anchors, d_idx, n, d_n, bev_extents, p2, im_wh,
                        d_bev_norm=None, d_img_norm=None, d_anchors_f32=None):
    _lib.check(ctx.lib.dodt_project_anchors_f64(
        ctx.handle, _p(d_anchors), _p(d_idx), int(n), _p(d_n),
        _arr(C.c_double, bev_extents), _arr(C.c_double, p2),
        float(im_wh[0]), float(im_wh[1]), _p(d_bev_norm), _p(d_img_norm),
        _p(d_anchors_f32)), 'dodt_project_anchors_f64')


def project_anchors_f32(ctx, d_anchors, n, d_n, bev_extents, p2, im_wh,
                        d_bev=None, d_bev_norm_tf=None, d_img_norm_tf=None):
    _lib.check(ctx.lib.dodt_project_anchors_f32(
        ctx.handle, _p(d_anchors), int(n), _p(d_n), _arr(C.c_float, bev_extents),
        _arr(C.c_float, p2), float(im_wh[0]), float(im_wh[1]), _p(d_bev),
        _p(d_bev_norm_tf), _p(d_img_norm_tf)), 'dodt_project_anchors_f32')


def img_preprocess(ctx, d_img_u8, in_hw, out_hw, out_c, mean_rgb, d_out):
    _lib.check(ctx.lib.dodt_img_preprocess(
        ctx.handle, _p(d_img_u8), int(in_hw[0]), int(in_hw[1]), int(out_hw[0]),
        int(out_hw[1]), int(out_c), _arr(C.c_float, mean_rgb), _p(d_out)),
        'dodt_img_preprocess')


def crop_and_resize(ctx, d_image, hwc, d_boxes, n, d_n, crop_hw, d_out, out_box_stride=None):
    if out_box_stride is None:
        out_box_stride = int(crop_hw[0]) * int(crop_hw[1]) * int(hwc[2])
    _lib.check(ctx.lib.dodt_crop_and_resize_strided(
        ctx.handle, _p(d_image), int(hwc[0]), int(hwc[1]), int(hwc[2]), _p(d_boxes),
        int(n), _p(d_n), int(crop_hw[0]), int(crop_hw[1]), _p(d_out), int(out_box_stride)),
        'dodt_crop_and_resize')


def nms(ctx, d_boxes, d_scores, n, d_n, max_out, iou_threshold, d_sel, d_count):
    _lib.check(ctx.lib.dodt_nms(
        ctx.handle, _p(d_boxes), _p(d_scores), int(n), _p(d_n), int(max_out),
        float(iou_threshold), _p(d_sel), _p(d_count)), 'dodt_nms')


def offset_to_anchor(ctx, d_anchors, d_offsets, n, d_n, d_out):
    _lib.check(ctx.lib.dodt_offset_to_anchor(
        ctx.handle, _p(d_anchors), _p(d_offsets), int(n), _p(d_n), _p(d_out)),
        'dodt_offset_to_anchor')


def softmax_fg(ctx, d_logits, n, d_n, d_scores):
    _lib.check(ctx.lib.dodt_softmax_fg(
        ctx.handle, _p(d_logits), int(n), _p(d_n), _p(d_scores)), 'dodt_softmax_fg')


def rpn_decode(ctx, d_anchors, d_offsets, d_logits, n, d_n, bev_extents, d_regressed, d_bev_norm_tf, d_scores):
    _lib.check(ctx.lib.dodt_rpn_decode(
        ctx.handle, _p(d_anchors), _p(d_offsets), _p(d_logits), int(n), _p(d_n), _arr(C.c_float, bev_extents),
        _p(d_regressed), _p(d_bev_norm_tf), _p(d_scores)), 'dodt_rpn_decode')


def gather_project(ctx, d_src, d_idx, n, d_n, bev_extents, p2, im_wh, d_rows, d_bev_norm_tf, d_img_norm_tf):
    _lib.check(ctx.lib.dodt_gather_project(
        ctx.handle, _p(d_src), _p(d_idx), int(n), _p(d_n), _arr(C.c_float, bev_extents), _arr(C.c_float, p2),
        float(im_wh[0]), float(im_wh[1]), _p(d_rows), _p(d_bev_norm_tf), _p(d_img_norm_tf)), 'dodt_gather_project')


def final_decode(ctx, d_top_anchors, d_offsets, d_cls_logits, d_angle_vectors, n, d_n, plane, bev_extents,
                 d_boxes_3d, d_pred_anchors, d_bev_tf, d_nms_scores, d_det_scores, d_orientations):
    _lib.check(ctx.lib.dodt_final_decode(
        ctx.handle, _p(d_top_anchors), _p(d_offsets), _p(d_cls_logits), _p(d_angle_vectors), int(n), _p(d_n),
        _arr(C.c_float, plane), _arr(C.c_float, bev_extents), _p(d_boxes_3d), _p(d_pred_anchors), _p(d_bev_tf),
        _p(d_nms_scores), _p(d_det_scores), _p(d_orientations)), 'dodt_final_decode')


def gather_rows(ctx, d_src, width, d_idx, n, d_n, d_out):
    _lib.check(ctx.lib.dodt_gather_rows(
        ctx.handle, _p(d_src), int(width), _p(d_idx), int(n), _p(d_n), _p(d_out)),
        'dodt_gather_rows')


def box_4c_decode(ctx, d_top_anchors, d_offsets, n, d_n, plane, bev_extents,
                  d_boxes_3d=None, d_pred_anchors=None, d_bev_tf=None):
    _lib.check(ctx.lib.dodt_box_4c_decode(
        ctx.handle, _p(d_top_anchors), _p(d_offsets), int(n), _p(d_n),
        _arr(C.c_float, plane), _arr(C.c_float, bev_extents), _p(d_boxes_3d),
        _p(d_pred_anchors), _p(d_bev_tf)), 'dodt_box_4c_decode')


def max_fg_logit(ctx, d_logits, n_cls, n, d_n, d_scores):
    _lib.check(ctx.lib.dodt_max_fg_logit(
        ctx.handle, _p(d_logits), int(n_cls), int(n), _p(d_n), _p(d_scores)),
        'dodt_max_fg_logit')


def angle_vector_to_orientation(ctx, d_angle_vectors, n, d_n, d_orientations):
    _lib.check(ctx.lib.dodt_angle_vector_to_orientation(
        ctx.handle, _p(d_angle_vectors), int(n), _p(d_n), _p(d_orientations)),
        'dodt_angle_vector_to_orientation')


def pack_detections(ctx, d_boxes_3d, d_scores, d_sel, d_count, max_det, frame_mark,
                    d_rec, d_count_out, d_corr_offsets=None, d_orientations=None):
    _lib.check(ctx.lib.dodt_pack_detections(
        ctx.handle, _p(d_boxes_3d), _p(d_scores), _p(d_orientations), _p(d_corr_offsets),
        _p(d_sel), _p(d_count), int(max_det), float(frame_mark), _p(d_rec), _p(d_count_out)),
        'dodt_pack_detections')


def fetch_i32_begin(ctx, d_src, n, slot):
    _lib.check(ctx.lib.dodt_fetch_i32_begin(ctx.handle, _p(d_src), int(n), int(slot)),
               'dodt_fetch_i32_begin')


def fetch_i32_end(ctx, slot, n):
    buf = (C.c_int32 * n)()
    _lib.check(ctx.lib.dodt_fetch_i32_end(ctx.handle, int(slot), buf, int(n)),
               'dodt_fetch_i32_end')
    return list(buf)


def correlation(ctx, d_a, d_b, hwc, max_displacement, stride_2, pad, d_out):
    _lib.check(ctx.lib.dodt_correlation(
        ctx.handle, _p(d_a), _p(d_b), int(hwc[0]), int(hwc[1]), int(hwc[2]),
        int(max_displacement), int(stride_2), int(pad), _p(d_out)), 'dodt_correlation')


def mean_fusion(ctx, d_a, d_b, rows, d_n, row_floats, d_out):
    _lib.check(ctx.lib.dodt_mean_fusion(ctx.handle, _p(d_a), _p(d_b), int(rows), _p(d_n),
                                        int(row_floats), _p(d_out)), 'dodt_mean_fusion')


def rows_to_bf16(ctx, d_a, d_b, rows, d_n, row_floats, in_ld, d_out, out_ld):
    _lib.check(ctx.lib.dodt_rows_to_bf16(ctx.handle, _p(d_a), _p(d_b), int(rows), _p(d_n), int(row_floats),
                                         int(in_ld), _p(d_out), int(out_ld)), 'dodt_rows_to_bf16')


def bf16_to_float(a):
    return (np.asarray(a, np.uint16).astype(np.uint32) << 16).view(np.float32)


class FullyConnected(object):

    def __init__(self, ctx, w, b, relu, dtype='f32'):
        if dtype not in ('f32', 'bf16'):
            raise ValueError("dtype must be 'f32' or 'bf16'")
        w = np.ascontiguousarray(w, dtype=np.float32)
        b = np.ascontiguousarray(b, dtype=np.float32)
        if w.ndim != 2 or b.shape != (w.shape[1],):
            raise ValueError('weights must be (K,N) and bias (N,)')
        self.ctx, self.K, self.N, self.dtype = ctx, int(w.shape[0]), int(w.shape[1]), dtype
        h = C.c_void_p()
        flags = (_lib.FC_RELU if relu else 0) | (_lib.FC_BF16 if dtype == 'bf16' else 0)
        _lib.check(ctx.lib.dodt_fc_create_ex(ctx.handle, self.K, self.N,
                                             w.ctypes.data_as(C.c_void_p),
                                             b.ctypes.data_as(C.c_void_p), flags, C.byref(h)),
                   'dodt_fc_create_ex')
        self.handle = h

    def forward(self, d_x, M, d_y, ldx=None, ldy=None, d_x2=None, d_m=None, ctx=None):
        c = ctx or self.ctx
        _lib.check(c.lib.dodt_fc_forward(
            self.handle, c.handle, _p(d_x), _p(d_x2), int(self.K if ldx is None else ldx),
            int(M), _p(d_m), _p(d_y), int(self.N if ldy is None else ldy)), 'dodt_fc_forward')

    def can_split(self, ldx=None):
        return self.N <= 32 and self.K % 16 == 0 and \
            (self.K if ldx is None else ldx) % 4 == 0 and os.environ.get('DODT_FC_SKINNY') != '0'

    def forward_split(self, d_x, M, d_ys, widths, ldx=None, d_m=None, ctx=None):
        c = ctx or self.ctx
        w = (C.c_int * len(widths))(*[int(v) for v in widths])
        ys = (C.c_void_p * len(d_ys))(*[_p(y) for y in d_ys])
        _lib.check(c.lib.dodt_fc_forward_split(
            self.handle, c.handle, _p(d_x), int(self.K if ldx is None else ldx), int(M), _p(d_m),
            len(widths), w, ys), 'dodt_fc_forward_split')

    def bf16_row_elems(self):
        return int(self.ctx.lib.dodt_fc_bf16_row_elems(self.handle)) if self.dtype == 'bf16' else 0

    def forward_bf16(self, d_x, M, d_y, ldx, ldy=None, d_m=None, y_bf16=True, ctx=None):
        c = ctx or self.ctx
        _lib.check(c.lib.dodt_fc_forward_bf16(self.handle, c.handle, _p(d_x), int(ldx), int(M), _p(d_m), _p(d_y),
                                              int(self.N if ldy is None else ldy), 1 if y_bf16 else 0),
                   'dodt_fc_forward_bf16')

    def forward_split_bf16(self, d_x, M, d_ys, widths, ldx, d_m=None, ctx=None):
        c = ctx or self.ctx
        w = (C.c_int * len(widths))(*[int(v) for v in widths])
        ys = (C.c_void_p * len(d_ys))(*[_p(y) for y in d_ys])
        _lib.check(c.lib.dodt_fc_forward_split_bf16(
            self.handle, c.handle, _p(d_x), int(ldx), int(M), _p(d_m), len(widths), w, ys), 'dodt_fc_forward_split_bf16')

    def flops(self, M):
        return 2.0 * M * self.K * self.N

    def close(self):
        if self.handle is not None:
            self.ctx.lib.dodt_fc_destroy(self.handle)
            self.handle = None


def three_d_iou_matrix(ctx, d_a, na, d_b, nb, d_iou_out):
    _lib.check(ctx.lib.dodt_three_d_iou_matrix(ctx.handle, _p(d_a), int(na), _p(d_b), int(nb), _p(d_iou_out)),
               'dodt_three_d_iou_matrix')


def temporal_calib(r0_rect, tr_velo_to_cam):
    r0 = np.asarray(r0_rect, np.float64).reshape(3, 3)
    tr = np.asarray(tr_velo_to_cam, np.float64).reshape(3, 4)
    inv = np.zeros_like(tr)
    inv[0:3, 0:3] = np.transpose(tr[0:3, 0:3])
    inv[0:3, 3] = np.dot(-np.transpose(tr[0:3, 0:3]), tr[0:3, 3])
    return np.concatenate([np.linalg.inv(r0).reshape(-1), inv.reshape(-1), tr.reshape(-1), r0.reshape(-1)])


def temporal_ego(ego, n_frames):
    if len(ego) != n_frames - 1:
        raise ValueError('recovery needs one (trans, matrix, delta) per frame 1..n_frames-1')
    out = np.zeros((n_frames, 13))
    for i, (trans, matrix, delta) in enumerate(ego):
        out[i + 1, 0:3] = np.asarray(trans, np.float64).reshape(3)
        out[i + 1, 3:12] = np.linalg.inv(np.asarray(matrix, np.float64).reshape(3, 3)).reshape(-1)
        out[i + 1, 12] = float(delta)
    return out


def interpolate_pairs(ctx, d_records, d_counts, n_pairs, max_det, n_frames, threshold, on_conflict, d_out,
                      d_out_counts, d_status, d_recover=None, calib=None, max_out=None):
    if on_conflict not in ('raise', 'next_best'):
        raise ValueError("on_conflict must be 'raise' or 'next_best'")
    if d_records.dtype not in (np.float32, np.float64):
        raise ValueError('records must be float32 or float64')
    cal = None if calib is None else _arr(C.c_double, calib)
    _lib.check(ctx.lib.dodt_interpolate_pairs(
        ctx.handle, _p(d_records), int(d_records.dtype == np.float64), _p(d_counts), int(n_pairs), int(max_det),
        int(n_frames), float(threshold), _lib.CONFLICT_NEXT_BEST if on_conflict == 'next_best' else _lib.CONFLICT_RAISE,
        _p(d_recover), cal, int(2 * max_det if max_out is None else max_out), _p(d_out), _p(d_out_counts),
        _p(d_status)), 'dodt_interpolate_pairs')


def track_state_bytes(log_capacity):
    n = C.c_size_t()
    _lib.check(_lib.load().dodt_track_state_bytes(int(log_capacity), C.byref(n)), 'dodt_track_state_bytes')
    return int(n.value)


def track_reset(ctx, d_state, log_capacity):
    _lib.check(ctx.lib.dodt_track_reset(ctx.handle, _p(d_state), int(log_capacity)), 'dodt_track_reset')


def track_flush(ctx, d_state, high_threshold, t_min):
    _lib.check(ctx.lib.dodt_track_flush(ctx.handle, _p(d_state), float(high_threshold), int(t_min)), 'dodt_track_flush')


def track_encode(ctx, d_records, d_counts, n_pairs, max_det, p2, image_wh, threshold, d_track, d_ious, d_enc_counts):
    if d_records.dtype not in (np.float32, np.float64):
        raise ValueError('records must be float32 or float64')
    _lib.check(ctx.lib.dodt_track_encode(
        ctx.handle, _p(d_records), int(d_records.dtype == np.float64), _p(d_counts), int(n_pairs), int(max_det),
        _arr(C.c_double, np.asarray(p2, np.float64).reshape(12)), float(image_wh[0]), float(image_wh[1]),
        float(threshold), _p(d_track), _p(d_ious), _p(d_enc_counts)), 'dodt_track_encode')


def track_pairs(ctx, d_state, d_records, d_counts, n_pairs, max_det, p2, image_wh, score_threshold, high_threshold,
                iou_threshold, t_min):
    if d_records.dtype not in (np.float32, np.float64):
        raise ValueError('records must be float32 or float64')
    _lib.check(ctx.lib.dodt_track_pairs(
        ctx.handle, _p(d_state), _p(d_records), int(d_records.dtype == np.float64), _p(d_counts), int(n_pairs),
        int(max_det), _arr(C.c_double, np.asarray(p2, np.float64).reshape(12)), float(image_wh[0]),
        float(image_wh[1]), float(score_threshold), float(high_threshold), float(iou_threshold), int(t_min)),
        'dodt_track_pairs')


def track_encoded(ctx, d_state, d_track, d_ious, d_counts, n_pairs, max_rows, high_threshold, iou_threshold, t_min):
    _lib.check(ctx.lib.dodt_track_encoded(
        ctx.handle, _p(d_state), _p(d_track), _p(d_ious), _p(d_counts), int(n_pairs), int(max_rows),
        float(high_threshold), float(iou_threshold), int(t_min)), 'dodt_track_encoded')
```

dodt_amd/pipeline.py:

```python
import os

import numpy as np

from dodt_amd import config as _config
from dodt_amd import _lib, device, ops, tracking
from dodt_amd.core.anchor_generators import grid_anchor_3d_generator as gen
from dodt_amd.core.avod_fc_layers.fusion_fc_layers import EarlyFusionFcLayers
from dodt_amd.core.feature_extractors.vgg import BevVgg, ImgVgg
from dodt_amd.core.feature_extractors.vgg_pyramid import BevVggPyr, ImgVggPyr
from dodt_amd.core.models.anchor_predictor import AnchorPredictor
from dodt_amd.temporal import unpack_frames

EXTRACTORS = {'vgg_pyr': (BevVggPyr, ImgVggPyr), 'vgg': (BevVgg, ImgVgg)}

MAX_DET = 100
REC_COLS = 17
ROI = 7
CORR_MAX_DISP, CORR_STRIDE2, CORR_PAD = 5, 2, 5
CORR_CH = (2 * (CORR_MAX_DISP // CORR_STRIDE2) + 1) ** 2


class FramePairPipeline(object):

    def __init__(self, ctx, cfg, bev_params, img_params, p2=_config.KITTI_P2,
                 r0_rect=_config.KITTI_R0_RECT, tr_velo_to_cam=_config.KITTI_TR_VELO_TO_CAM,
                 image_wh=_config.KITTI_IMAGE_WH, n_points_max=120000, rpn_nms_size=1024,
                 pairs_per_step=1, side_streams=None, head_params=None, conv_dtype='f32',
                 head_dtype='f32', reuse_streams_of=None, tail_sets=None, temporal=None, tracker=None,
                 bev_input_skip=True, bev_frame_tables=True):
        self.ctx = ctx
        self.cfg = cfg
        self.p2 = np.asarray(p2, dtype=np.float64)
        self.image_wh = tuple(image_wh)
        self.P = int(rpn_nms_size)
        self.n_points_max = int(n_points_max)
        self.pairs = int(pairs_per_step)
        self.fps = int(cfg.get('frames_per_sample', 2))
        if self.fps not in (1, 2):
            raise ValueError('frames_per_sample must be 1 or 2')
        self.temporal = None
        if temporal is not None:
            if self.fps != 2:
                raise ValueError('temporal: needs frame pairs (frames_per_sample == 2)')
            t = dict(temporal)
            tm = dict(n_frames=int(t.pop('n_frames')), threshold=float(t.pop('threshold', 0.1)),
                      on_conflict=t.pop('on_conflict', 'raise'))
            if t:
                raise ValueError('temporal: unknown keys %s' % sorted(t))
            if tm['on_conflict'] not in ('raise', 'next_best'):
                raise ValueError("temporal: on_conflict must be 'raise' or 'next_best'")
            if not 1 <= tm['n_frames'] <= 64:
                raise ValueError('temporal: n_frames must be 1..64')
            self.temporal = tm
        self.tracker = None
        if tracker is not None:
            if self.fps != 2:
                raise ValueError('tracker: needs frame pairs (frames_per_sample == 2)')
            t = dict(tracker)
            tk = dict(score_threshold=float(t.pop('score_threshold', 0.1)),
                      high_threshold=float(t.pop('high_threshold', 0.5)),
                      iou_threshold=float(t.pop('iou_threshold', 0.005)), t_min=int(t.pop('t_min', 3)),
                      classes=tuple(t.pop('classes', ('Car',))), max_sequence_dets=int(t.pop('max_sequence_dets', 65536)))
            if t:
                raise ValueError('tracker: unknown keys %s' % sorted(t))
            if tk['max_sequence_dets'] < 1:
                raise ValueError('tracker: max_sequence_dets must be >= 1')
            self.tracker = tk
        self.nf = self.fps * self.pairs
        self.bev_h, self.bev_w = cfg['bev_dims']
        self.img_h, self.img_w = cfg['img_dims']
        self.n_slices = cfg['num_slices']
        self.bev_extents_flat = np.asarray(cfg['bev_extents'], np.float64).reshape(-1)
        self.bp = ops.make_bev_params(cfg, _config.velo_to_cam(r0_rect, tr_velo_to_cam),
                                      self.p2, self.image_wh)
        if tail_sets is None:
            tail_sets = 1
        tail_sets = int(os.environ.get('DODT_PIPE_TAIL_SETS', tail_sets))
        if tail_sets not in (1, 2):
            raise ValueError('tail_sets must be 1 or 2')
        if reuse_streams_of is not None:
            self.img_ctx = reuse_streams_of.img_ctx
            self.stream_sets = list(reuse_streams_of.stream_sets)
            while len(self.stream_sets) < tail_sets:
                self.stream_sets.append(self._make_side_streams(ctx, side_streams))
            self.stream_sets = self.stream_sets[:tail_sets]
        else:
            self.img_ctx = device.Context(ctx.device_id)
            self.stream_sets = [self._make_side_streams(ctx, side_streams) for _ in range(tail_sets)]
        self.sides, self.preps = self.stream_sets[0]
        boxes = gen.tile_anchors_3d(cfg['area_extents'], cfg['anchor_sizes'],
                                    cfg['anchor_stride'], cfg['ground_plane'])
        self.anchors_all = gen.box_3d_to_anchor(boxes)
        cells, self.nx, self.nz = gen.anchor_grid_cells(
            self.anchors_all, cfg['area_extents'], cfg['voxel_size'])
        self.n_all = len(self.anchors_all)
        self.d_anchor_table = ctx.array(self.anchors_all)
        self.d_cells = ctx.array(cells)

        bev_cls, img_cls = EXTRACTORS[cfg.get('extractor', 'vgg_pyr')]
        self.bev_net = bev_cls(ctx=ctx, shared_gpu=True, conv_dtype=conv_dtype)
        self.bev_net.load_params(bev_params)
        self.bev_net._ensure(self.nf, self.bev_h, self.bev_w, cfg['bev_depth'])
        self.bev_skipped_items = 0
        if bev_input_skip and conv_dtype == 'f32' and hasattr(self.bev_net, 'set_input_support') \
                and self.bp.point_format == _lib.PTS_VELO_XYZI:
            self.bev_skipped_items = self.bev_net.set_input_support(
                ops.bev_support_mask(self.bp, self.bev_net.PAD_TOP, ctx.lib), frame_tables=bev_frame_tables)
        self.img_net = img_cls(ctx=self.img_ctx, shared_gpu=True, conv_dtype=conv_dtype)
        self.img_net.load_params(img_params)
        self.img_net._ensure(self.nf, self.img_h, self.img_w, 4)
        self.bev_fh, self.bev_fw, self.feat_c = self.bev_net.output_shape()
        self.img_fh, self.img_fw, img_c = self.img_net.output_shape()
        if img_c != self.feat_c:
            raise ValueError('mean fusion needs equal feature depths')
        self.bev_pad = self.bev_net.PAD_TOP
        self.in_bev = [ctx.zeros((self.nf, self.bev_pad + self.bev_h, self.bev_w, cfg['bev_depth']), np.float32)
                       for _ in range(2)]
        self.in_img = [ctx.zeros((self.nf, self.img_net.PAD_TOP + self.img_h, self.img_w, 4), np.float32)
                       for _ in range(2)]
        self.d_bev_in = self._views(self.in_bev[0], (self.bev_h, self.bev_w, cfg['bev_depth']), self.bev_pad)

        f32, i32 = np.float32, np.int32
        N, P = self.n_all, self.P
        self.rpn_head = self.avod_head = self.corr_head = None
        rep = cfg.get('box_representation', 'box_4ca')
        if rep not in ('box_4c', 'box_4ca'):
            raise NotImplementedError('Regression not implemented for %s' % rep)
        self.box_4ca = rep == 'box_4ca'
        if head_params is not None:
            self.rpn_head = AnchorPredictor(ctx, head_params['rpn'], dtype=head_dtype)
            self.avod_head = EarlyFusionFcLayers(
                ctx, head_params['avod'], dtype=head_dtype,
                outputs=('cls_out', 'off_out') + (('ang_out',) if self.box_4ca else ()))
            if self.fps == 2:
                self.corr_head = EarlyFusionFcLayers(ctx, head_params['corr'],
                                                     outputs=('off_out',), dtype=head_dtype)
            self.head_scratch_sets = [[dict(rpn=self.rpn_head.make_scratch(N),
                                            fc=self.avod_head.make_scratch(P),
                                            corr_map=ctx.empty((self.bev_fh, self.bev_fw, CORR_CH), f32)
                                            if self.fps == 2 else None)
                                       for _ in sides] for sides, _ in self.stream_sets]
            self.head_scratch = self.head_scratch_sets[0]
            self.corr_maps = [[ctx.empty((self.bev_fh, self.bev_fw, CORR_CH), f32) for _ in range(self.pairs)]
                              for _ in range(2)] if self.fps == 2 else None

        FC = self.feat_c
        self.feat = [dict(
            bev_feat=ctx.empty((self.nf, self.bev_fh, self.bev_fw, FC), f32),
            bev_bneck=ctx.empty((self.nf, self.bev_fh, self.bev_fw, 1), f32),
            img_feat=ctx.empty((self.nf, self.img_fh, self.img_fw, FC), f32),
            img_bneck=ctx.empty((self.nf, self.img_fh, self.img_fw, 1), f32)) for _ in range(2)]
        self.prep3 = [[dict(occ=ctx.empty((self.nz, (self.nx + 31) // 32), np.uint32),
                            keep=ctx.empty((N,), i32), count=ctx.zeros((1,), i32),
                            bev_norm=ctx.empty((N, 4), f32), img_norm=ctx.empty((N, 4), f32),
                            anchors=ctx.empty((N, 6), f32)) for _ in range(self.nf)] for _ in range(3)]
        if 3 * self.nf > 32:
            raise ValueError('at most 10 frames per step (count fetch slots)')
        self.fr2 = [[], []]
        for f in range(2 * self.nf):
            b = dict(
                rpn_bev_roi=ctx.empty((N, 3, 3, 1), f32), rpn_img_roi=ctx.empty((N, 3, 3, 1), f32),
                regressed=ctx.empty((N, 6), f32), prop_bev=ctx.empty((N, 4), f32),
                scores=ctx.empty((N,), f32),
                top_idx=ctx.empty((P,), i32), top_count=ctx.zeros((1,), i32),
                top_anchors=ctx.empty((P, 6), f32),
                top_bev=ctx.empty((P, 4), f32), top_img=ctx.empty((P, 4), f32),
                bev_rois=ctx.empty((P, ROI, ROI, FC), f32),
                img_rois=ctx.empty((P, ROI, ROI, FC), f32),
                boxes_3d=ctx.empty((P, 7), f32), pred_anchors=ctx.empty((P, 6), f32),
                nms2_boxes=ctx.empty((P, 4), f32), nms2_scores=ctx.empty((P,), f32),
                det_idx=ctx.empty((MAX_DET,), i32), det_count=ctx.zeros((1,), i32),
                det_scores=ctx.empty((P,), f32), orientations=ctx.empty((P,), f32))
            if head_params is not None:
                b.update(rpn_logits=ctx.empty((N, 2), f32), rpn_offsets=ctx.empty((N, 6), f32),
                         cls_logits=ctx.empty((P, 2), f32), offsets_4c=ctx.empty((P, 10), f32))
                if self.box_4ca:
                    b.update(angle_vectors=ctx.empty((P, 2), f32))
                if self.fps == 2 and f % 2 == 0:
                    b.update(corr_rois=ctx.zeros((P, self.corr_head.in_ld), f32),
                             corr_offsets=ctx.empty((P, 3), f32))
            self.fr2[f // self.nf].append(b)
        self.fr = [dict(b, **p) for b, p in zip(self.fr2[0], self.prep3[0])]
        self.prepped = -1
        self.step_idx = 0
        self.pending = None
        self.rec2 = [ctx.empty((self.pairs, self.fps, MAX_DET, REC_COLS), f32) for _ in range(2)]
        self.cnt2 = [ctx.zeros((self.pairs, self.fps), i32) for _ in range(2)]
        self.d_records, self.d_rec_counts = self.rec2[0], self.cnt2[0]
        self.last_anchor_counts = [0] * self.nf
        self.on_records_reuse = None
        if self.temporal is not None:
            self.temporal_calib = ops.temporal_calib(r0_rect, tr_velo_to_cam)
            self._alloc_frames()
        if self.tracker is not None:
            tk = self.tracker
            self.track_state = tracking.Tracker(self.ctx, tk['max_sequence_dets'], tk['high_threshold'],
                                                tk['iou_threshold'], tk['t_min'], tk['score_threshold'])
            self.img_ctx.wait_for(self.ctx)
            self.last_sequence_tracks = None
        self.mark_steps = ()
        self.early_prep = os.environ.get('DODT_PIPE_EARLY_PREP', '1') != '0'
        self.marks = {}
        ctx.sync()

    def _mark(self, c, step, name):
        if step in self.mark_steps:
            slot = sum(1 for (cc, _) in self.marks.values() if cc is c)
            if slot < 64:
                c.mark(slot)
                self.marks['%d:%s' % (step, name)] = (c, slot)

    def _make_side_streams(self, ctx, side_streams):
        n_side = min(self.nf, 2) if side_streams is None else int(side_streams)
        hp = os.environ.get('DODT_PIPE_PRIO', '0') == '1'
        sides = [device.Context(ctx.device_id, high_priority=hp)
                 for _ in range(max(n_side, 1))]
        mode = os.environ.get('DODT_PIPE_STREAMS', 'shared')
        if mode == 'shared':
            preps = sides
        elif mode == 'conv':
            preps = [ctx if i % 2 == 0 else self.img_ctx for i in range(len(sides))]
        elif mode == 'one':
            one = device.Context(ctx.device_id, high_priority=hp)
            preps = [one for _ in sides]
        else:
            preps = [device.Context(ctx.device_id, high_priority=hp)
                     for _ in range(max(n_side, 1))]
        return sides, preps

    def _streams(self, cur):
        return self.stream_sets[cur % len(self.stream_sets)]

    def _views(self, arr, shape, pad_top=0):
        row = int(np.prod(shape[1:])) * 4
        frame = (pad_top + shape[0]) * row
        return [arr.offset(frame * f + pad_top * row, shape) for f in range(self.nf)]

    def use_record_buffers(self, rec_ptrs, cnt_ptrs):
        if len(rec_ptrs) < 2 or len(rec_ptrs) != len(cnt_ptrs):
            raise ValueError('use_record_buffers: at least two record and count buffers, as many of each')
        self.rec2 = [self.ctx.wrap(p, (self.pairs, self.fps, MAX_DET, REC_COLS), np.float32)
                     for p in rec_ptrs]
        self.cnt2 = [self.ctx.wrap(p, (self.pairs, self.fps), np.int32) for p in cnt_ptrs]
        self.d_records, self.d_rec_counts = self.rec2[0], self.cnt2[0]
        self._alloc_frames()

    def _alloc_frames(self):
        if self.temporal is None:
            return
        R, n = len(self.rec2), self.temporal['n_frames']
        self.frames2 = [self.ctx.empty((self.pairs, n, 2 * MAX_DET, 13), np.float64) for _ in range(R)]
        self.fcnt2 = [self.ctx.zeros((self.pairs, n), np.int32) for _ in range(R)]
        self.fst2 = [self.ctx.zeros((self.pairs,), np.int32) for _ in range(R)]
        self.ego2 = [self.img_ctx.zeros((self.pairs, n, 13), np.float64) for _ in range(R)]
        self.d_frames, self.d_frame_counts, self.d_frame_status = self.frames2[0], self.fcnt2[0], self.fst2[0]

    def use_record_ring(self, d_rec_ring, d_cnt_ring):
        R = d_rec_ring.shape[0]
        if tuple(d_rec_ring.shape[1:]) != (self.pairs, self.fps, MAX_DET, REC_COLS) or \
                tuple(d_cnt_ring.shape) != (R, self.pairs, self.fps):
            raise ValueError('use_record_ring: shapes do not match the pipeline')
        nr, nc = 4 * self.pairs * self.fps * MAX_DET * REC_COLS, 4 * self.pairs * self.fps
        self.use_record_buffers([d_rec_ring.ptr + nr * i for i in range(R)],
                                [d_cnt_ring.ptr + nc * i for i in range(R)])

    def _stage_from_host(self, k, h_points, n_points, h_images):
        cur = k & 1
        _, preps = self._streams(cur)
        ns = len(preps)
        if not hasattr(self, 'stage'):
            H, W = self.image_wh[1], self.image_wh[0]
            self.stage = [[(self.ctx.empty((self.n_points_max, 4), np.float32),
                            self.ctx.empty((H, W, 3), np.uint8)) for _ in range(self.nf)]
                          for _ in range(2)]
        d_pts, d_imgs = [], []
        for f in range(self.nf):
            c = preps[f % ns]
            dp, di = self.stage[cur][f]
            if n_points[f] > self.n_points_max:
                raise ValueError('frame %d has more than n_points_max points' % f)
            dp.upload_async(h_points[f], ctx=c, nbytes=16 * int(n_points[f]))
            di.upload_async(h_images[f], ctx=c)
            d_pts.append(dp)
            d_imgs.append(di)
        return d_pts, d_imgs

    def run_from_host(self, h_points, n_points, h_images, heads=None, ego_motion=None, lookahead=None):
        if self.prepped == self.step_idx:
            d_pts = d_imgs = None
        else:
            d_pts, d_imgs = self._stage_from_host(self.step_idx, h_points, n_points, h_images)
        if lookahead is not None:
            la = tuple(lookahead) + (None,) * (4 - len(lookahead))
            nd_pts, nd_imgs = self._stage_from_host(self.step_idx + 1, la[0], la[1], la[2])
            lookahead = (nd_pts, la[1], nd_imgs, la[3])
        return self.run(d_pts, n_points, d_imgs, heads, ego_motion, lookahead)

    PREP_DONE_MARK = 244

    def _prep(self, k, d_points, n_points, d_images, ego_motion, ahead):
        nf = self.nf
        mean = (self.img_net._R_MEAN, self.img_net._G_MEAN, self.img_net._B_MEAN)
        cur = k & 1
        sides, preps = self._streams(cur)
        ns = len(sides)
        bev_in = self._views(self.in_bev[cur], (self.bev_h, self.bev_w, self.cfg['bev_depth']), self.bev_pad)
        img_in = self._views(self.in_img[cur], (self.img_h, self.img_w, 4), self.img_net.PAD_TOP)
        if ahead and k >= 2:
            for c in set(preps):
                c.wait_mark(self.ctx, self.CONV_DONE_MARK + cur)
                c.wait_mark(self.img_ctx, self.CONV_DONE_MARK + cur)
        for f in range(nf):
            c, b = preps[f % ns], self.prep3[k % 3][f]
            self._mark(c, k, 'prep%d_start' % f)
            bp = self.bp
            if ego_motion is not None and self.fps == 2 and f % 2 == 1 \
                    and ego_motion[f // 2] is not None:
                bp = ops.with_ego_motion(self.bp, *ego_motion[f // 2])
            ops.bev_slices(c, d_points[f], n_points[f], bp, bev_in[f], b['occ'])
            ops.anchor_filter(c, b['occ'], self.nx, self.nz, self.d_cells, self.n_all,
                              b['keep'], b['count'])
            ops.fetch_i32_begin(c, b['count'], 1, 3 * f + k % 3)
            ops.project_anchors_f64(c, self.d_anchor_table, b['keep'], self.n_all, b['count'],
                                    self.bev_extents_flat, self.p2, self.image_wh,
                                    b['bev_norm'], b['img_norm'], b['anchors'])
            ops.img_preprocess(c, d_images[f], (self.image_wh[1], self.image_wh[0]),
                               (self.img_h, self.img_w), 4, mean, img_in[f])
            self._mark(c, k, 'prep%d_end' % f)
        for c in set(preps):
            c.mark(self.PREP_DONE_MARK + k % 3)
        self.prepped = k

    def run(self, d_points, n_points, d_images, heads=None, ego_motion=None, lookahead=None, recover=None):
        main, nf = self.ctx, self.nf
        if (heads is None) != (self.rpn_head is not None):
            raise ValueError('pass `heads` exactly when the pipeline has no head_params')
        if recover is not None:
            if self.temporal is None:
                raise ValueError('recover: the pipeline has no temporal module')
            if len(recover) != self.pairs:
                raise ValueError('recover: one entry per pair of the step')
            n = self.temporal['n_frames']
            self.ego2[self.step_idx % len(self.rec2)].upload(np.stack([ops.temporal_ego(e, n) for e in recover]))
        cur = self.step_idx & 1
        sides, preps = self._streams(cur)
        ns = len(sides)
        fr, feat = self.fr2[cur], self.feat[cur]
        k = self.step_idx
        if self.prepped != k:
            self._prep(k, d_points, n_points, d_images, ego_motion, ahead=False)
        for c in set(preps):
            main.wait_mark(c, self.PREP_DONE_MARK + k % 3)
            self.img_ctx.wait_mark(c, self.PREP_DONE_MARK + k % 3)
        self._mark(main, k, 'bev_start')
        self._mark(self.img_ctx, k, 'img_start')
        self.bev_net.forward_device_padded(self.in_bev[cur], feat['bev_feat'], feat['bev_bneck'])
        self.img_net.forward_device_padded(self.in_img[cur], feat['img_feat'], feat['img_bneck'])
        self._mark(main, k, 'bev_end')
        self._mark(self.img_ctx, k, 'img_end')
        main.mark(self.CONV_DONE_MARK + cur)
        self.img_ctx.mark(self.CONV_DONE_MARK + cur)
        if self._corr_on_img():
            self.img_ctx.wait_mark(main, self.CONV_DONE_MARK + cur)
            bev_hw, px = (self.bev_fh, self.bev_fw), self.bev_fh * self.bev_fw
            for pair in range(self.pairs):
                fb0 = feat['bev_feat'].offset(4 * px * self.feat_c * (2 * pair), bev_hw + (self.feat_c,))
                fb1 = feat['bev_feat'].offset(4 * px * self.feat_c * (2 * pair + 1), bev_hw + (self.feat_c,))
                ops.correlation(self.img_ctx, fb0, fb1, bev_hw + (self.feat_c,), CORR_MAX_DISP, CORR_STRIDE2, CORR_PAD,
                                self.corr_maps[cur][pair])
            self.img_ctx.mark(self.CORR_MAP_MARK + cur)
        if lookahead is not None:
            la = tuple(lookahead) + (None,) * (4 - len(lookahead))
            self._prep(k + 1, la[0], la[1], la[2], la[3], ahead=True)
        if self.pending is not None:
            self._wait_convs(self.pending)
            self._tail(self.pending)
            p_sides, p_preps = self._streams(self.pending['cur'])
            for i, s in enumerate(p_sides):
                s.mark(self.TAIL_DONE_MARK)
                main.wait_mark(s, self.TAIL_DONE_MARK)
                if os.environ.get('DODT_PIPE_IMG_WAIT', 'tail') != 'none':
                    self.img_ctx.wait_mark(s, self.TAIL_DONE_MARK)
                if p_preps[i] is not s:
                    p_preps[i].wait_mark(s, self.TAIL_DONE_MARK)
            self._temporal_step(self.pending)
            self._tracker_step(self.pending)
        self.pending = dict(cur=cur, heads=heads, step=k, rslot=k % len(self.rec2), recover=recover is not None)
        if not self.early_prep:
            for s in sides:
                s.wait_for(main)
                s.wait_for(self.img_ctx)
        self.step_idx += 1
        return cur

    def finish(self):
        st = self.pending
        if st is not None:
            self._wait_convs(st)
            self._tail(st)
            self.pending = None
        for sides, preps in self.stream_sets:
            for s in set(sides) | set(preps):
                self.ctx.wait_for(s)
        self.ctx.wait_for(self.img_ctx)
        if st is not None and (self.temporal is not None or self.tracker is not None):
            self.img_ctx.wait_for(self.ctx)
            self._temporal_step(st)
            self._tracker_step(st)
            self.ctx.wait_for(self.img_ctx)

    def _temporal_step(self, st):
        if self.temporal is None:
            return
        T, r, c = self.temporal, st['rslot'], self.img_ctx
        if os.environ.get('DODT_PIPE_IMG_WAIT', 'tail') == 'none':
            for s in self._streams(st['cur'])[0]:
                c.wait_mark(s, self.TAIL_DONE_MARK)
        self._mark(c, st['step'], 'temporal_start')
        ops.interpolate_pairs(c, self.rec2[r], self.cnt2[r], self.pairs, MAX_DET, T['n_frames'], T['threshold'],
                              T['on_conflict'], self.frames2[r], self.fcnt2[r], self.fst2[r],
                              d_recover=self.ego2[r] if st['recover'] else None,
                              calib=self.temporal_calib if st['recover'] else None, max_out=2 * MAX_DET)
        self._mark(c, st['step'], 'temporal_end')
        self.d_frames, self.d_frame_counts, self.d_frame_status = self.frames2[r], self.fcnt2[r], self.fst2[r]

    def _tracker_step(self, st):
        if self.tracker is None:
            return
        r, c = st['rslot'], self.img_ctx
        if self.temporal is None and os.environ.get('DODT_PIPE_IMG_WAIT', 'tail') == 'none':
            for s in self._streams(st['cur'])[0]:
                c.wait_mark(s, self.TAIL_DONE_MARK)
        self._mark(c, st['step'], 'tracker_start')
        self.track_state.track_records(self.rec2[r], self.cnt2[r], self.pairs, MAX_DET, self.p2, self.image_wh, ctx=c)
        self._mark(c, st['step'], 'tracker_end')

    def _frame_ids(self, frame_ids):
        if frame_ids is not None:
            ids = [tuple(f) for f in frame_ids]
            return lambda pair, kf: ids[pair][kf]
        tau = self.temporal['n_frames'] - 1 if self.temporal is not None else 1
        return lambda pair, kf: pair * tau + kf * tau

    def tracks_so_far(self, frame_ids=None):
        if self.tracker is None:
            raise ValueError('tracks_so_far: the pipeline has no tracker')
        self.ctx.wait_for(self.img_ctx)
        return tracking.tracks_from_log(self.track_state.read(), self._frame_ids(frame_ids), self.tracker['classes'])

    def end_sequence(self, frame_ids=None):
        if self.tracker is None:
            raise ValueError('end_sequence: the pipeline has no tracker')
        if self.pending is not None:
            raise ValueError('end_sequence: call finish() first (the last step is not tracked yet)')
        self.track_state.flush(ctx=self.img_ctx)
        tracks = self.tracks_so_far(frame_ids)
        self.track_state.reset(ctx=self.img_ctx)
        self.last_sequence_tracks = tracks
        return tracks

    def kitti_tracking_rows(self, tracks=None):
        from dodt_amd.core.dt_evaluator_utils import convert_trajectory_to_kitti_format
        if tracks is None:
            if self.tracker is None or self.last_sequence_tracks is None:
                raise ValueError('kitti_tracking_rows: no sequence has ended')
            tracks = self.last_sequence_tracks
        return convert_trajectory_to_kitti_format(tracks)

    def frames(self):
        if self.temporal is None:
            raise ValueError('frames: the pipeline has no temporal module')
        self.ctx.wait_for(self.img_ctx)
        return unpack_frames(self.d_frames.download(), self.d_frame_counts.download(),
                             self.d_frame_status.download(), self.temporal['on_conflict'])

    CONV_DONE_MARK = 250
    CORR_MAP_MARK = 248

    def _corr_on_img(self):
        return (self.rpn_head is not None and self.fps == 2 and len(self.sides) >= 2
                and not os.environ.get('DODT_PIPE_NO_CORR') and os.environ.get('DODT_PIPE_CORR_ON_F1', '1') != '0'
                and os.environ.get('DODT_PIPE_CORR_MAP', 'img') == 'img')

    def _wait_convs(self, st):
        if self.early_prep:
            for s in self._streams(st['cur'])[0]:
                s.wait_mark(self.ctx, self.CONV_DONE_MARK + st['cur'])
                s.wait_mark(self.img_ctx, self.CONV_DONE_MARK + st['cur'])

    def _tail(self, st):
        cfg, nf = self.cfg, self.nf
        cur = st['cur']
        sides, preps = self._streams(cur)
        ns = len(sides)
        head_scratch = self.head_scratch_sets[cur % len(self.stream_sets)] if self.rpn_head is not None else None
        fr, feat = self.fr2[cur], self.feat[cur]
        heads = st['heads']
        k3 = st['step'] % 3
        counts = [ops.fetch_i32_end(preps[f % ns], 3 * f + k3, 1)[0]
                  for f in range(nf)]
        self.last_anchor_counts = counts
        fr = [dict(b, **p) for b, p in zip(fr, self.prep3[k3])]
        self.fr = fr
        self.d_records, self.d_rec_counts = self.rec2[st['rslot']], self.cnt2[st['rslot']]
        self.d_bev_in = self._views(self.in_bev[cur], (self.bev_h, self.bev_w, self.cfg['bev_depth']), self.bev_pad)
        bev_px = self.bev_fh * self.bev_fw
        img_px = self.img_fh * self.img_fw
        FC = self.feat_c
        bev_hw, img_hw = (self.bev_fh, self.bev_fw), (self.img_fh, self.img_fw)
        plane = cfg['ground_plane']
        if os.environ.get('DODT_PIPE_NO_TAIL'):
            return
        if self.on_records_reuse is not None:
            self.on_records_reuse(st['rslot'], sides)
        computed = heads is None
        split_t = computed and self.fps == 2 and ns >= 2 and not os.environ.get('DODT_PIPE_NO_CORR') \
            and os.environ.get('DODT_PIPE_CORR_ON_F1', '1') != '0'
        corr_img = split_t and self._corr_on_img()
        fused_tail = os.environ.get('DODT_PIPE_FUSED_TAIL', '1') != '0'

        def t_branch_crops(cc, f0, scratch):
            fb0 = feat['bev_feat'].offset(4 * bev_px * FC * f0, bev_hw + (FC,))
            fb1 = feat['bev_feat'].offset(4 * bev_px * FC * (f0 + 1), bev_hw + (FC,))
            ops.correlation(cc, fb0, fb1, bev_hw + (FC,), CORR_MAX_DISP, CORR_STRIDE2, CORR_PAD,
                            scratch['corr_map'])
            ops.crop_and_resize(cc, scratch['corr_map'], bev_hw + (CORR_CH,), fr[f0]['top_bev'], self.P,
                                fr[f0]['top_count'], (ROI, ROI), fr[f0]['corr_rois'],
                                out_box_stride=self.corr_head.in_ld)

        def frame(f):
            c, b, A = sides[f % ns], fr[f], counts[f]
            h = b if computed else heads[f]
            scratch = head_scratch[f % ns] if computed else None
            self._mark(c, st['step'], 'tail%d_start' % f)
            bneck_b = feat['bev_bneck'].offset(4 * bev_px * f, bev_hw + (1,))
            bneck_i = feat['img_bneck'].offset(4 * img_px * f, img_hw + (1,))
            feat_b = feat['bev_feat'].offset(4 * bev_px * FC * f, bev_hw + (FC,))
            feat_i = feat['img_feat'].offset(4 * img_px * FC * f, img_hw + (FC,))
            ops.crop_and_resize(c, bneck_b, bev_hw + (1,), b['bev_norm'], A, None,
                                (3, 3), b['rpn_bev_roi'])
            ops.crop_and_resize(c, bneck_i, img_hw + (1,), b['img_norm'], A, None,
                                (3, 3), b['rpn_img_roi'])
            self._mark(c, st['step'], 'tail%d_crops' % f)
            if computed and not os.environ.get('DODT_PIPE_NO_RPN'):
                self.rpn_head.forward(c, b['rpn_bev_roi'], b['rpn_img_roi'], A, b['rpn_logits'],
                                      b['rpn_offsets'], scratch['rpn'])
            self._mark(c, st['step'], 'tail%d_rpn' % f)
            if fused_tail:
                ops.rpn_decode(c, b['anchors'], h['rpn_offsets'], h['rpn_logits'], A, None, self.bev_extents_flat,
                               b['regressed'], b['prop_bev'], b['scores'])
            else:
                ops.offset_to_anchor(c, b['anchors'], h['rpn_offsets'], A, None, b['regressed'])
                ops.project_anchors_f32(c, b['regressed'], A, None, self.bev_extents_flat, self.p2,
                                        self.image_wh, d_bev_norm_tf=b['prop_bev'])
                ops.softmax_fg(c, h['rpn_logits'], A, None, b['scores'])
            ops.nms(c, b['prop_bev'], b['scores'], A, None, self.P,
                    cfg['rpn_nms_iou_thresh'], b['top_idx'], b['top_count'])
            if fused_tail:
                ops.gather_project(c, b['regressed'], b['top_idx'], self.P, b['top_count'], self.bev_extents_flat,
                                   self.p2, self.image_wh, b['top_anchors'], b['top_bev'], b['top_img'])
                self._mark(c, st['step'], 'tail%d_nms1' % f)
            else:
                ops.gather_rows(c, b['regressed'], 6, b['top_idx'], self.P, b['top_count'],
                                b['top_anchors'])
                self._mark(c, st['step'], 'tail%d_nms1' % f)
                ops.project_anchors_f32(c, b['top_anchors'], self.P, b['top_count'],
                                        self.bev_extents_flat, self.p2, self.image_wh,
                                        d_bev_norm_tf=b['top_bev'], d_img_norm_tf=b['top_img'])
            ops.crop_and_resize(c, feat_b, bev_hw + (FC,), b['top_bev'], self.P,
                                b['top_count'], (ROI, ROI), b['bev_rois'])
            ops.crop_and_resize(c, feat_i, img_hw + (FC,), b['top_img'], self.P,
                                b['top_count'], (ROI, ROI), b['img_rois'])
            yield 'crops'
            pair = self.fps == 2
            corr_offsets = h.get('corr_offsets') if pair and f % 2 == 0 else None
            self._mark(c, st['step'], 'tail%d_crops2' % f)
            if computed:
                self.avod_head.forward(c, b['bev_rois'], b['img_rois'], self.P, b['top_count'],
                                       [b['cls_logits'], b['offsets_4c']]
                                       + ([b['angle_vectors']] if self.box_4ca else []),
                                       scratch['fc'])
                self._mark(c, st['step'], 'tail%d_fc2' % f)
                yield 'head'
                if pair and f % 2 == 0 and not os.environ.get('DODT_PIPE_NO_CORR'):
                    if corr_img:
                        pass
                    else:
                        if split_t:
                            c.wait_mark(sides[(f + 1) % ns], self.CORR_ROIS_MARK)
                        else:
                            t_branch_crops(c, f, scratch)
                        self._mark(c, st['step'], 'tail%d_corrmap' % f)
                        self.corr_head.forward(c, b['corr_rois'], None, self.P, b['top_count'],
                                               [b['corr_offsets']], scratch['fc'])
            self._mark(c, st['step'], 'tail%d_heads' % f)
            if fused_tail:
                ops.final_decode(c, b['top_anchors'], h['offsets_4c'], h['cls_logits'],
                                 h['angle_vectors'] if self.box_4ca else None, self.P, b['top_count'], plane,
                                 self.bev_extents_flat, b['boxes_3d'], b['pred_anchors'], b['nms2_boxes'],
                                 b['nms2_scores'], b['det_scores'], b['orientations'] if self.box_4ca else None)
                ops.nms(c, b['nms2_boxes'], b['nms2_scores'], self.P, b['top_count'], MAX_DET,
                        cfg['avod_nms_iou_thresh'], b['det_idx'], b['det_count'])
            else:
                ops.box_4c_decode(c, b['top_anchors'], h['offsets_4c'], self.P, b['top_count'],
                                  plane, self.bev_extents_flat, b['boxes_3d'], b['pred_anchors'],
                                  b['nms2_boxes'])
                ops.max_fg_logit(c, h['cls_logits'], 2, self.P, b['top_count'], b['nms2_scores'])
                ops.nms(c, b['nms2_boxes'], b['nms2_scores'], self.P, b['top_count'], MAX_DET,
                        cfg['avod_nms_iou_thresh'], b['det_idx'], b['det_count'])
                ops.softmax_fg(c, h['cls_logits'], self.P, b['top_count'], b['det_scores'])
                if self.box_4ca:
                    ops.angle_vector_to_orientation(c, h['angle_vectors'], self.P, b['top_count'],
                                                    b['orientations'])
            yield 'pack'
            ops.pack_detections(
                c, b['boxes_3d'], b['det_scores'], b['det_idx'], b['det_count'], MAX_DET,
                float(f % self.fps),
                self.d_records.offset(4 * MAX_DET * REC_COLS * f, (MAX_DET, REC_COLS)),
                self.d_rec_counts.offset(4 * f, (1,), np.int32), d_corr_offsets=corr_offsets,
                d_orientations=b['orientations'] if self.box_4ca else None)
            self._mark(c, st['step'], 'tail%d_end' % f)

        def drain(g):
            for _ in g:
                pass

        if not split_t:
            for f in range(nf):
                drain(frame(f))
            return
        for f0 in range(0, nf, 2):
            c0, c1 = sides[f0 % ns], sides[(f0 + 1) % ns]
            g0, g1 = frame(f0), frame(f0 + 1)
            while next(g0) != 'crops':
                pass
            c0.mark(self.PROPOSALS_MARK)
            if corr_img:
                while next(g0) != 'pack':
                    pass
                while next(g1) != 'crops':
                    pass
                c1.wait_mark(c0, self.PROPOSALS_MARK)
                c1.wait_mark(self.img_ctx, self.CORR_MAP_MARK + cur)
                ops.crop_and_resize(c1, self.corr_maps[cur][f0 // 2], bev_hw + (CORR_CH,), fr[f0]['top_bev'], self.P,
                                    fr[f0]['top_count'], (ROI, ROI), fr[f0]['corr_rois'],
                                    out_box_stride=self.corr_head.in_ld)
                self.corr_head.forward(c1, fr[f0]['corr_rois'], None, self.P, fr[f0]['top_count'],
                                       [fr[f0]['corr_offsets']], head_scratch[(f0 + 1) % ns]['fc'])
                c1.mark(self.CORR_ROIS_MARK)
                c0.wait_mark(c1, self.CORR_ROIS_MARK)
                drain(g0)
                drain(g1)
                continue
            while next(g0) != 'head':
                pass
            while next(g1) != 'crops':
                pass
            c1.wait_mark(c0, self.PROPOSALS_MARK)
            t_branch_crops(c1, f0, head_scratch[(f0 + 1) % ns])
            c1.mark(self.CORR_ROIS_MARK)
            drain(g1)
            drain(g0)

    PROPOSALS_MARK, CORR_ROIS_MARK = 252, 253
    TAIL_DONE_MARK = 247

    def sync(self):
        self.ctx.sync()

    def flops_per_step(self):
        return self.bev_net.flops() + self.img_net.flops()

    def mfma_flops_per_step(self):
        return self.bev_net.mfma_flops() + self.img_net.mfma_flops()

    def conv_bytes_per_step(self):
        return self.bev_net.bytes() + self.img_net.bytes()

    def head_flops_per_step(self, anchor_counts=None):
        if self.rpn_head is None:
            return 0.0
        counts = anchor_counts or self.last_anchor_counts
        return (sum(self.rpn_head.flops(a) for a in counts)
                + self.nf * self.avod_head.flops(self.P)
                + (self.pairs * self.corr_head.flops(self.P) if self.corr_head else 0.0))

    def flops_per_pair(self):
        return self.flops_per_step() / self.pairs

    def close(self):
        self.bev_net.close()
        self.img_net.close()
        for hd in (self.rpn_head, self.avod_head, self.corr_head):
            if hd is not None:
                hd.close()
```

include/dodt_hip.h:

```cpp
#ifndef DODT_HIP_H
#define DODT_HIP_H

#include <stddef.h>
#include <stdint.h>

#ifdef __cplusplus
extern "C" {
#endif

#define DODT_OK 0
#define DODT_ERR_INVALID 1
#define DODT_ERR_HIP 2
#define DODT_ERR_UNSUPPORTED 3

typedef struct dodt_ctx dodt_ctx;

int dodt_version(void);
const char* dodt_last_error(void);
int dodt_ctx_create(int device_id, dodt_ctx** out);
int dodt_ctx_create_high_priority(int device_id, dodt_ctx** out);
int dodt_ctx_create_on_stream(int device_id, void* hip_stream, dodt_ctx** out);
int dodt_ctx_destroy(dodt_ctx* ctx);
int dodt_ctx_sync(dodt_ctx* ctx);
int dodt_mark(dodt_ctx* ctx, int slot);
int dodt_ctx_wait_mark(dodt_ctx* ctx, dodt_ctx* other, int slot);
int dodt_mark_elapsed(dodt_ctx* from, int from_slot, dodt_ctx* to, int to_slot, float* ms);
int dodt_ctx_wait_for(dodt_ctx* ctx, dodt_ctx* other);
int dodt_malloc(dodt_ctx* ctx, size_t bytes, void** d_out);
int dodt_free(dodt_ctx* ctx, void* d_ptr);
int dodt_memcpy_h2d(dodt_ctx* ctx, void* d_dst, const void* src, size_t bytes);
int dodt_memcpy_d2h(dodt_ctx* ctx, void* dst, const void* d_src, size_t bytes);
int dodt_memset(dodt_ctx* ctx, void* d_dst, int value, size_t bytes);
int dodt_pinned_alloc(dodt_ctx* ctx, size_t bytes, void** out);
int dodt_pinned_free(dodt_ctx* ctx, void* ptr);
int dodt_memcpy_h2d_async(dodt_ctx* ctx, void* d_dst, const void* pinned_src, size_t bytes);

int dodt_fetch_i32_begin(dodt_ctx* ctx, const int32_t* d_src, int n, int slot);
int dodt_fetch_i32_end(dodt_ctx* ctx, int slot, int32_t* dst, int n);

int dodt_timer_start(dodt_ctx* ctx);
int dodt_timer_stop(dodt_ctx* ctx, float* ms_out);

#define DODT_PTS_VELO_XYZI 0
#define DODT_PTS_CAM_3XN 1

typedef struct dodt_bev_params {
    int32_t point_format;
    int32_t num_slices;
    double velo_to_cam[12];
    double p2[12];
    double im_w, im_h;
    double plane[4];
    double extents[6];
    double voxel_size;
    double height_lo, height_hi;
    double occ_lo, occ_hi;
    int32_t has_pre_transform;
    int32_t reserved_;
    double pre_translate[3];
    double pre_rotate[9];
} dodt_bev_params;

int dodt_bev_slices(dodt_ctx* ctx, const void* d_points, int n_points,
                    const dodt_bev_params* params, float* d_bev_out,
                    uint32_t* d_occ_bits_out);
int dodt_bev_status(dodt_ctx* ctx, int* flags);
int dodt_bev_support_mask(const dodt_bev_params* params, int pad_top, uint8_t* mask_out, int rows, int cols);

int dodt_anchor_filter(dodt_ctx* ctx, const uint32_t* d_occ_bits, int nx, int nz,
                       const int32_t* d_anchor_cells, int n_anchors,
                       int density_threshold, int32_t* d_keep_idx_out,
                       int32_t* d_count_out);

int dodt_project_anchors_f64(dodt_ctx* ctx, const double* d_anchors,
                             const int32_t* d_idx, int n, const int32_t* d_n,
                             const double bev_extents[4], const double p2[12],
                             double im_w, double im_h, float* d_bev_norm_out,
                             float* d_img_norm_out, float* d_anchors_f32_out);

int dodt_project_anchors_f32(dodt_ctx* ctx, const float* d_anchors, int n,
                             const int32_t* d_n, const float bev_extents[4],
                             const float p2[12], float im_w, float im_h,
                             float* d_bev_out, float* d_bev_norm_tf_out,
                             float* d_img_norm_tf_out);

int dodt_img_preprocess(dodt_ctx* ctx, const uint8_t* d_img_u8, int in_h, int in_w,
                        int out_h, int out_w, int out_c, const float mean_rgb[3],
                        float* d_out);

typedef struct dodt_extractor dodt_extractor;
#define DODT_EXTRACTOR_VGG_PYR 0
#define DODT_EXTRACTOR_VGG 1
#define DODT_EXTRACTOR_SHARED_GPU 0x100
#define DODT_EXTRACTOR_BF16 0x200
#define DODT_EXTRACTOR_SPLIT 0x400
#define DODT_CONV_MODE_DEFAULT 2
int dodt_conv_mode(void);
int dodt_extractor_create(dodt_ctx* ctx, int kind, int in_h, int in_w, int in_c,
                          int pad_top, int batch, dodt_extractor** out);
int dodt_extractor_destroy(dodt_extractor* ex);
int dodt_extractor_set_layer(dodt_extractor* ex, const char* name, const float* w,
                             int kh, int kw, int c_a, int c_b, const float* beta,
                             const float* mean, const float* var);
int dodt_extractor_input(dodt_extractor* ex, float** d_ptr, long long* frame_stride_floats);
int dodt_extractor_forward(dodt_extractor* ex, const float* d_in, float* d_feat_out,
                           float* d_bottleneck_out);
int dodt_extractor_forward_padded(dodt_extractor* ex, const float* d_x0, float* d_feat_out,
                                  float* d_bottleneck_out);
int dodt_extractor_set_input(dodt_extractor* ex, const float* d_x0);
int dodt_extractor_set_input_support(dodt_extractor* ex, const uint8_t* mask, int rows, int cols,
                                     long long* skipped_items);
int dodt_extractor_set_frame_tables(dodt_extractor* ex, int on, int* enabled);
int dodt_extractor_frame_items(dodt_extractor* ex, int* items, int n);
int dodt_extractor_frame_split(dodt_extractor* ex, int* computed, int* restored, int n);
long long dodt_extractor_store_bytes(const dodt_extractor* ex);
int dodt_frame_tables_host(const uint8_t* masks, int frames, int rows, int cols, int layer, int th, int tw,
                           const int* items, int n_items, const uint8_t* prev, int* run, int* n_run);
int dodt_frame_lists_host(const uint8_t* masks, int frames, int rows, int cols, int layer, int th, int tw,
                          const int* items, int n_items, const uint8_t* prev, int* run, int* n_run, int* restore,
                          int* n_restore);
int dodt_frame_restore_host(const int* item, int f, int th, int tw, int bn, int ch0, int rows, int cols, int channels,
                            int pad_top, float* dst, const float* src, float* dst2, const float* src2);
int dodt_extractor_output_shape(const dodt_extractor* ex, int* h, int* w, int* c);
int dodt_extractor_first_layers_folded(const dodt_extractor* ex);
int dodt_extractor_read_activation(dodt_extractor* ex, const char* name, float* dst,
                                   int* h, int* w, int* c);
double dodt_extractor_flops(const dodt_extractor* ex);
double dodt_extractor_mfma_flops(const dodt_extractor* ex);
double dodt_extractor_bytes(const dodt_extractor* ex);
typedef struct dodt_layer_info {
    char name[32];
    char kernel[48];
    int32_t launches;
    int32_t items;
    double flops_direct;
    double flops_executed;
    double bytes;
    float ms;
    int32_t reserved_;
} dodt_layer_info;
int dodt_extractor_layer_count(const dodt_extractor* ex);
int dodt_extractor_forward_timed(dodt_extractor* ex, const float* d_in, float* d_feat_out,
                                 float* d_bottleneck_out, dodt_layer_info* info, int n_info);

int dodt_crop_and_resize(dodt_ctx* ctx, const float* d_image, int H, int W, int C,
                         const float* d_boxes, int n, const int32_t* d_n, int crop_h,
                         int crop_w, float* d_out);
int dodt_crop_and_resize_strided(dodt_ctx* ctx, const float* d_image, int H, int W, int C,
                                 const float* d_boxes, int n, const int32_t* d_n, int crop_h,
                                 int crop_w, float* d_out, long long out_box_stride);

int dodt_correlation(dodt_ctx* ctx, const float* d_a, const float* d_b, int H, int W, int C,
                     int max_displacement, int stride_2, int pad, float* d_out);

int dodt_mean_fusion(dodt_ctx* ctx, const float* d_a, const float* d_b, int rows, const int32_t* d_n,
                     int row_floats, float* d_out);
typedef struct dodt_fc dodt_fc;
int dodt_fc_create(dodt_ctx* ctx, int K, int N, const float* w, const float* bias, int relu,
                   dodt_fc** out);
#define DODT_FC_RELU 1
#define DODT_FC_BF16 2
int dodt_fc_create_ex(dodt_ctx* ctx, int K, int N, const float* w, const float* bias, int flags,
                      dodt_fc** out);
int dodt_fc_destroy(dodt_fc* fc);
int dodt_fc_forward(dodt_fc* fc, dodt_ctx* ctx, const float* d_x, const float* d_x2, int ldx,
                    int M, const int32_t* d_m, float* d_y, int ldy);
int dodt_fc_forward_split(dodt_fc* fc, dodt_ctx* ctx, const float* d_x, int ldx, int M, const int32_t* d_m,
                          int parts, const int* widths, float* const* d_ys);
int dodt_fc_bf16_row_elems(const dodt_fc* fc);
int dodt_fc_forward_bf16(dodt_fc* fc, dodt_ctx* ctx, const void* d_x_bf16, int ldx, int M, const int32_t* d_m,
                         void* d_y, int ldy, int y_bf16);
int dodt_fc_forward_split_bf16(dodt_fc* fc, dodt_ctx* ctx, const void* d_x_bf16, int ldx, int M, const int32_t* d_m,
                               int parts, const int* widths, float* const* d_ys);
int dodt_rows_to_bf16(dodt_ctx* ctx, const float* d_a, const float* d_b, int rows, const int32_t* d_n,
                      int row_floats, int in_ld, void* d_out_bf16, int out_ld);
double dodt_fc_flops(const dodt_fc* fc, int M);

int dodt_nms(dodt_ctx* ctx, const float* d_boxes, const float* d_scores, int n,
             const int32_t* d_n, int max_out, float iou_threshold, int32_t* d_sel_out,
             int32_t* d_count_out);

int dodt_offset_to_anchor(dodt_ctx* ctx, const float* d_anchors, const float* d_offsets,
                          int n, const int32_t* d_n, float* d_out);
int dodt_softmax_fg(dodt_ctx* ctx, const float* d_logits2, int n, const int32_t* d_n,
                    float* d_scores_out);
int dodt_rpn_decode(dodt_ctx* ctx, const float* d_anchors, const float* d_offsets, const float* d_logits2, int n,
                    const int32_t* d_n, const float bev_extents[4], float* d_regressed_out,
                    float* d_bev_norm_tf_out, float* d_scores_out);
int dodt_gather_project(dodt_ctx* ctx, const float* d_src, const int32_t* d_idx, int n, const int32_t* d_n,
                        const float bev_extents[4], const float p2[12], float im_w, float im_h,
                        float* d_rows_out, float* d_bev_norm_tf_out, float* d_img_norm_tf_out);
int dodt_final_decode(dodt_ctx* ctx, const float* d_top_anchors, const float* d_offsets, const float* d_cls_logits2,
                      const float* d_angle_vectors, int n, const int32_t* d_n, const float plane[4],
                      const float bev_extents[4], float* d_boxes_3d_out, float* d_pred_anchors_out,
                      float* d_bev_tf_out, float* d_nms_scores_out, float* d_det_scores_out,
                      float* d_orientations_out);
int dodt_gather_rows(dodt_ctx* ctx, const float* d_src, int width, const int32_t* d_idx,
                     int n, const int32_t* d_n, float* d_out);
int dodt_max_fg_logit(dodt_ctx* ctx, const float* d_logits, int n_cls, int n,
                      const int32_t* d_n, float* d_scores_out);
int dodt_angle_vector_to_orientation(dodt_ctx* ctx, const float* d_angle_vectors, int n,
                                     const int32_t* d_n, float* d_orientations_out);
int dodt_pack_detections(dodt_ctx* ctx, const float* d_boxes_3d, const float* d_scores,
                         const float* d_orientations, const float* d_corr_offsets,
                         const int32_t* d_sel, const int32_t* d_count, int max_det,
                         float frame_mark, float* d_rec_out, int32_t* d_count_out);
int dodt_box_4c_decode(dodt_ctx* ctx, const float* d_top_anchors, const float* d_offsets,
                       int n, const int32_t* d_n, const float plane[4],
                       const float bev_extents[4], float* d_boxes_3d_out,
                       float* d_pred_anchors_out, float* d_bev_tf_out);

int dodt_three_d_iou_matrix(dodt_ctx* ctx, const double* d_a, int na, const double* d_b, int nb,
                            double* d_iou_out);
#define DODT_CONFLICT_RAISE 0
#define DODT_CONFLICT_NEXT_BEST 1
int dodt_interpolate_pairs(dodt_ctx* ctx, const void* d_records, int records_f64, const int32_t* d_counts,
                           int n_pairs, int max_det, int n_frames, double threshold, int on_conflict,
                           const double* d_recover, const double* calib, int max_out, double* d_out,
                           int32_t* d_out_counts, int32_t* d_status);

int dodt_track_state_bytes(int log_capacity, size_t* bytes);
int dodt_track_reset(dodt_ctx* ctx, void* d_state, int log_capacity);
int dodt_track_flush(dodt_ctx* ctx, void* d_state, double high_threshold, int t_min);
int dodt_track_encode(dodt_ctx* ctx, const void* d_records, int records_f64, const int32_t* d_counts,
                      int n_pairs, int max_det, const double* p2, double image_w, double image_h,
                      double score_threshold, float* d_track_out, float* d_ious_out, int32_t* d_counts_out);
int dodt_track_pairs(dodt_ctx* ctx, void* d_state, const void* d_records, int records_f64,
                     const int32_t* d_counts, int n_pairs, int max_det, const double* p2, double image_w,
                     double image_h, double score_threshold, double high_threshold, double iou_threshold,
                     int t_min);
int dodt_track_encoded(dodt_ctx* ctx, void* d_state, const float* d_track, const float* d_ious,
                       const int32_t* d_counts, int n_pairs, int max_rows, double high_threshold,
                       double iou_threshold, int t_min);

typedef struct dodt_comm dodt_comm;
#define DODT_COMM_ID_BYTES 128
int dodt_comm_unique_id(uint8_t* id_out);
int dodt_comm_create(dodt_ctx* ctx, int rank, int world, const uint8_t* id, dodt_comm** out);
int dodt_comm_destroy(dodt_comm* comm);
int dodt_comm_attach(dodt_comm* comm, dodt_ctx* ctx);
int dodt_comm_rank(const dodt_comm* comm, int* rank, int* world);
int dodt_comm_set_late_peer(dodt_comm* comm, double microseconds);
int dodt_all_gather_records(dodt_comm* comm, dodt_ctx* producer, int slot, const float* d_records,
                            const int32_t* d_counts, int pairs, int frames, int max_det, int cols,
                            float* d_all_records, int32_t* d_all_counts);
int dodt_comm_join(dodt_comm* comm, int slot, dodt_ctx* consumer);
int dodt_comm_sync(dodt_comm* comm);
int dodt_comm_barrier(dodt_comm* comm);
int dodt_comm_max_f64(dodt_comm* comm, double* value);

#ifdef __cplusplus
}
#endif
#endif
```

Before: 383.4.

## Compute correlation and corr head only for final detections via sparse tile list

Adds a path that, once detections are selected, builds a list of only the correlation-map tiles covered by detection boxes. The correlation kernel then runs on just those tiles, and crops are taken and the correlation head is run on the MAX_DET detections rather than on all proposals. Packing reads these compact per-detection offsets. The two frames of a pair are interleaved as generators. The aim is to avoid computing the full correlation map and the corr head over every proposal. The cost is an extra single-block tile-list kernel and a serial dependency on detection selection before correlation can start.

```diff
diff --git a/dodt_amd/_lib.py b/dodt_amd/_lib.py
--- a/dodt_amd/_lib.py
+++ b/dodt_amd/_lib.py
@@ -124,6 +124,10 @@
     'dodt_crop_and_resize_strided': (_i, [_vp, _pf, _i, _i, _i, _pf, _i, _pi32, _i, _i, _pf,
                                           C.c_longlong]),
     'dodt_correlation': (_i, [_vp, _pf, _pf, _i, _i, _i, _i, _i, _i, _pf]),
+    'dodt_crop_and_resize_indexed': (_i, [_vp, _pf, _i, _i, _i, _pf, _i, _pi32, _i, _pi32, _i, _i, _pf,
+                                          C.c_longlong]),
+    'dodt_correlation_tile_list': (_i, [_vp, _i, _i, _pf, _i, _pi32, _i, _pi32, _i, _i, _pi32, _i, _pi32]),
+    'dodt_correlation_tiles': (_i, [_vp, _pf, _pf, _i, _i, _i, _i, _i, _i, _pi32, _i, _pi32, _pf]),
     'dodt_mean_fusion': (_i, [_vp, _pf, _pf, _i, _pi32, _i, _pf]),
     'dodt_fc_create': (_i, [_vp, _i, _i, _hf, _hf, _i, C.POINTER(_vp)]),
     'dodt_fc_create_ex': (_i, [_vp, _i, _i, _hf, _hf, _i, C.POINTER(_vp)]),
@@ -145,6 +149,7 @@
     'dodt_gather_rows': (_i, [_vp, _pf, _i, _pi32, _i, _pi32, _pf]),
     'dodt_max_fg_logit': (_i, [_vp, _pf, _i, _i, _pi32, _pf]),
     'dodt_pack_detections': (_i, [_vp, _pf, _pf, _pf, _pf, _pi32, _pi32, _i, _f, _pf, _pi32]),
+    'dodt_pack_detections_compact': (_i, [_vp, _pf, _pf, _pf, _pf, _pi32, _pi32, _i, _f, _pf, _pi32]),
     'dodt_angle_vector_to_orientation': (_i, [_vp, _pf, _i, _pi32, _pf]),
     'dodt_box_4c_decode': (_i, [_vp, _pf, _pf, _i, _pi32, C.POINTER(_f),
                                 C.POINTER(_f), _pf, _pf, _pf]),
diff --git a/dodt_amd/csrc/anchors.hip b/dodt_amd/csrc/anchors.hip
--- a/dodt_amd/csrc/anchors.hip
+++ b/dodt_amd/csrc/anchors.hip
@@ -296,7 +296,7 @@
 pack_detections_kernel(const float* __restrict__ boxes_3d, const float* __restrict__ scores,
                        const float* __restrict__ orientations, const float* __restrict__ corr,
                        const int* __restrict__ sel, const int* __restrict__ d_count, int max_det,
-                       float frame_mark, float* __restrict__ rec, int* __restrict__ count_out) {
+                       float frame_mark, float* __restrict__ rec, int* __restrict__ count_out, int corr_compact) {
     const int t = blockIdx.x * blockDim.x + threadIdx.x;
     const int cnt = min(*d_count, max_det);
     if (t == 0) *count_out = cnt;
@@ -313,9 +313,10 @@
             for (int k = 0; k < 7; ++k) b[k] = boxes_3d[(size_t)src * 7 + k];
             if (orientations) orientation_correct(b, orientations[src]);
             if (col >= 9) {
-                b[0] += corr[(size_t)src * 3 + 0];
-                b[2] += corr[(size_t)src * 3 + 1];
-                b[6] += corr[(size_t)src * 3 + 2];
+                const size_t cr = corr_compact ? row : src;
+                b[0] += corr[cr * 3 + 0];
+                b[2] += corr[cr * 3 + 1];
+                b[6] += corr[cr * 3 + 2];
             }
             const int c = col < 7 ? col : col - 9;
 #pragma unroll
@@ -612,18 +613,36 @@
     return DODT_OK;
 }
 
-int dodt_pack_detections(dodt_ctx* ctx, const float* d_boxes_3d, const float* d_scores,
-                         const float* d_orientations, const float* d_corr_offsets,
-                         const int32_t* d_sel, const int32_t* d_count, int max_det,
-                         float frame_mark, float* d_rec_out, int32_t* d_count_out) {
+namespace {
+int launch_pack_detections(dodt_ctx* ctx, const float* d_boxes_3d, const float* d_scores,
+                           const float* d_orientations, const float* d_corr_offsets, int corr_compact,
+                           const int32_t* d_sel, const int32_t* d_count, int max_det,
+                           float frame_mark, float* d_rec_out, int32_t* d_count_out) {
     DODT_REQUIRE(ctx && d_boxes_3d && d_scores && d_sel && d_count && d_rec_out && d_count_out &&
                      max_det > 0,
                  "dodt_pack_detections: bad argument");
     hipLaunchKernelGGL(pack_detections_kernel, dim3(dodt::ceil_div(max_det * 17, 256)), dim3(256),
                        0, ctx->stream, d_boxes_3d, d_scores, d_orientations, d_corr_offsets, d_sel,
-                       d_count, max_det, frame_mark, d_rec_out, d_count_out);
-    DODT_LAUNCH_CHECK();
-    return DODT_OK;
+                       d_count, max_det, frame_mark, d_rec_out, d_count_out, corr_compact);
+    DODT_LAUNCH_CHECK();
+    return DODT_OK;
+}
+}
+
+int dodt_pack_detections(dodt_ctx* ctx, const float* d_boxes_3d, const float* d_scores,
+                         const float* d_orientations, const float* d_corr_offsets,
+                         const int32_t* d_sel, const int32_t* d_count, int max_det,
+                         float frame_mark, float* d_rec_out, int32_t* d_count_out) {
+    return launch_pack_detections(ctx, d_boxes_3d, d_scores, d_orientations, d_corr_offsets, 0, d_sel, d_count,
+                                  max_det, frame_mark, d_rec_out, d_count_out);
+}
+
+int dodt_pack_detections_compact(dodt_ctx* ctx, const float* d_boxes_3d, const float* d_scores,
+                                 const float* d_orientations, const float* d_det_offsets,
+                                 const int32_t* d_sel, const int32_t* d_count, int max_det,
+                                 float frame_mark, float* d_rec_out, int32_t* d_count_out) {
+    return launch_pack_detections(ctx, d_boxes_3d, d_scores, d_orientations, d_det_offsets, 1, d_sel, d_count,
+                                  max_det, frame_mark, d_rec_out, d_count_out);
 }
 
 int dodt_angle_vector_to_orientation(dodt_ctx* ctx, const float* d_angle_vectors, int n,
diff --git a/dodt_amd/csrc/correlation.hip b/dodt_amd/csrc/correlation.hip
--- a/dodt_amd/csrc/correlation.hip
+++ b/dodt_amd/csrc/correlation.hip
@@ -4,6 +4,7 @@
 #include <vector>
 
 #include "common.h"
+#include "crop_coords.h"
 #include "lds_dma.h"
 
 namespace {
@@ -141,9 +142,10 @@
 template <int HALVES>
 __global__ void __launch_bounds__(256 * HALVES, 2 * HALVES)
 correlation_sp_kernel(const float* __restrict__ A, const float* __restrict__ B, int H, int W, int d, int pad,
-                      int OH, int OW, const int* __restrict__ tile_list, int n_tiles, float* __restrict__ out,
-                      int* __restrict__ stamps) {
+                      int OH, int OW, const int* __restrict__ tile_list, int n_tiles,
+                      const int* __restrict__ d_n_tiles, float* __restrict__ out, int* __restrict__ stamps) {
     constexpr int GW = 5, K = GW * GW, S2 = 2, QH = kC / 4 / HALVES;
+    if (d_n_tiles) n_tiles = min(n_tiles, max(*d_n_tiles, 0));
     constexpr int NW = 4 * HALVES;
     extern __shared__ __attribute__((aligned(16))) float smem[];
     const int tid = threadIdx.x;
@@ -322,6 +324,125 @@
     cache.push_back(SpTileList{ctx->device, tiles_y, tiles_x, d});
     *out = d;
     return DODT_OK;
+}
+
+int launch_sp(dodt_ctx* ctx, const float* d_a, const float* d_b, int H, int W, int max_displacement, int pad,
+              int OH, int OW, const int* d_list, int n, const int* d_n_tiles, float* d_out) {
+    static const int halves = getenv("DODT_CORR_HALVES") && atoi(getenv("DODT_CORR_HALVES")) == 2 ? 2 : 1;
+    static bool prepared = false;
+    if (!prepared) {
+        DODT_HIP_CHECK(hipFuncSetAttribute(reinterpret_cast<const void*>(&correlation_sp_kernel<1>),
+                                           hipFuncAttributeMaxDynamicSharedMemorySize, kSpLds));
+        DODT_HIP_CHECK(hipFuncSetAttribute(reinterpret_cast<const void*>(&correlation_sp_kernel<2>),
+                                           hipFuncAttributeMaxDynamicSharedMemorySize, kSpLds));
+        prepared = true;
+    }
+    static const int grid_env = getenv("DODT_CORR_GRID") ? atoi(getenv("DODT_CORR_GRID")) : 0;
+    int grid = grid_env > 0 ? grid_env / 8 * 8 : 2 * ctx->num_cus / 8 * 8;
+    if (grid > 8 * dodt::ceil_div(n, 8)) grid = 8 * dodt::ceil_div(n, 8);
+    static const bool want_stamps = getenv("DODT_CORR_STAMPS") != nullptr;
+    static int* d_stamps = nullptr;
+    if (want_stamps && !d_stamps) {
+        DODT_HIP_CHECK(hipMalloc(&d_stamps, 64 * sizeof(int)));
+        DODT_HIP_CHECK(hipMemset(d_stamps, 0, 64 * sizeof(int)));
+    }
+    if (halves == 2)
+        hipLaunchKernelGGL(correlation_sp_kernel<2>, dim3(grid), dim3(512), kSpLds, ctx->stream,
+                           d_a, d_b, H, W, max_displacement, pad, OH, OW, d_list, n, d_n_tiles, d_out, d_stamps);
+    else
+        hipLaunchKernelGGL(correlation_sp_kernel<1>, dim3(grid), dim3(256), kSpLds, ctx->stream,
+                           d_a, d_b, H, W, max_displacement, pad, OH, OW, d_list, n, d_n_tiles, d_out, d_stamps);
+    DODT_LAUNCH_CHECK();
+    if (want_stamps) {
+        int h[64];
+        (void)hipStreamSynchronize(ctx->stream);
+        (void)hipMemcpy(h, d_stamps, sizeof(h), hipMemcpyDeviceToHost);
+        fprintf(stderr, "[dodt] correlation, workgroup 9, us per phase: wait copies | barrier | arithmetic | barrier | "
+                        "early copies + outputs to LDS | stores | barrier + late copies\n");
+        for (int t = 0; t < 4; ++t) {
+            fprintf(stderr, "[dodt]   tile %d:", t);
+            for (int k = 0; k < 7; ++k) fprintf(stderr, " %6.2f", (h[t * 8 + k + 1] - h[t * 8 + k]) / 100.0);
+            fprintf(stderr, "   next tile's top +%.2f\n", (h[(t + 1) * 8] - h[t * 8]) / 100.0);
+        }
+    }
+    return DODT_OK;
+}
+
+constexpr int kListThreads = 256;
+constexpr int kListMaxTiles = 8192;
+
+__global__ void __launch_bounds__(kListThreads)
+corr_tile_list_kernel(int OH, int OW, const float* __restrict__ boxes, int n_boxes, const int* __restrict__ box_idx,
+                      int n, const int* __restrict__ d_n, int ch, int cw, const int* __restrict__ curve,
+                      int* __restrict__ list, int* __restrict__ d_count) {
+    __shared__ int flag[kListMaxTiles];
+    __shared__ int part[kListThreads];
+    __shared__ int4 rect[kListThreads];
+    const int tid = threadIdx.x;
+    const int tiles_y = (OH + kSpT - 1) / kSpT, tiles_x = (OW + kSpT - 1) / kSpT, total = tiles_y * tiles_x;
+    for (int t = tid; t < total; t += kListThreads) flag[t] = 0;
+    __syncthreads();
+    const int lim = d_n ? min(max(*d_n, 0), n) : n;
+    auto range = [](float a, float b, int size, int crop, int& lo, int& hi) {
+        float mn = 3.0e38f, mx = -3.0e38f;
+        for (int i = 0; i < crop; ++i) {
+            const float v = dodt::crop_coord(a, b, size, crop, i);
+            if (v == v) { mn = fminf(mn, v); mx = fmaxf(mx, v); }
+        }
+        if (mn > mx) return false;
+        const float cap = (float)size + 1.0f;
+        lo = (int)floorf(fminf(fmaxf(mn, -2.0f), cap)) - 1;
+        hi = (int)floorf(fminf(fmaxf(mx, -4.0f), cap)) + 2;
+        lo = max(lo, 0);
+        hi = min(hi, size - 1);
+        return lo <= hi;
+    };
+    for (int base = 0; base < lim; base += kListThreads) {
+        const int j = base + tid;
+        int4 r = make_int4(0, -1, 0, -1);
+        if (j < lim) {
+            const int src = box_idx ? box_idx[j] : j;
+            if (src >= 0 && src < n_boxes) {
+                const float4 bx = reinterpret_cast<const float4*>(boxes)[src];
+                int y_lo, y_hi, x_lo, x_hi;
+                if (range(bx.x, bx.z, OH, ch, y_lo, y_hi) && range(bx.y, bx.w, OW, cw, x_lo, x_hi))
+                    r = make_int4(y_lo / kSpT, y_hi / kSpT, x_lo / kSpT, x_hi / kSpT);
+            }
+        }
+        rect[tid] = r;
+        __syncthreads();
+        const int here = min(lim - base, kListThreads);
+        for (int k = tid / 64; k < here; k += kListThreads / 64) {
+            const int4 q = rect[k];
+            const int rw = q.w - q.z + 1, cnt = (q.y - q.x + 1) * rw;
+            for (int t = tid % 64; t < cnt; t += 64) {
+                const int ty = q.x + t / rw, tx = q.z + t % rw;
+                const int by = ty / 8 * 8, bxs = tx / 8 * 8;
+                const int bh = min(8, tiles_y - by), bw = min(8, tiles_x - bxs);
+                flag[by * tiles_x + bxs * bh + (ty - by) * bw + (tx - bxs)] = 1;
+            }
+        }
+        __syncthreads();
+    }
+    const int run = (total + kListThreads - 1) / kListThreads;
+    const int p0 = min(tid * run, total), p1 = min(p0 + run, total);
+    int mine = 0;
+    for (int p = p0; p < p1; ++p) mine += flag[p];
+    part[tid] = mine;
+    __syncthreads();
+    if (tid == 0) {
+        int acc = 0;
+        for (int t = 0; t < kListThreads; ++t) {
+            const int c = part[t];
+            part[t] = acc;
+            acc += c;
+        }
+        *d_count = acc;
+    }
+    __syncthreads();
+    int o = part[tid];
+    for (int p = p0; p < p1; ++p)
+        if (flag[p]) list[o++] = curve[p];
 }
 
 constexpr int kT = 16;
@@ -428,44 +549,8 @@
         const int ty = dodt::ceil_div(OH, kSpT), tx = dodt::ceil_div(OW, kSpT);
         const int* d_list = nullptr;
         if (int rc = sp_tile_list(ctx, ty, tx, &d_list)) return rc;
-        static const int halves = getenv("DODT_CORR_HALVES") && atoi(getenv("DODT_CORR_HALVES")) == 2 ? 2 : 1;
-        static bool prepared = false;
-        if (!prepared) {
-            DODT_HIP_CHECK(hipFuncSetAttribute(reinterpret_cast<const void*>(&correlation_sp_kernel<1>),
-                                               hipFuncAttributeMaxDynamicSharedMemorySize, kSpLds));
-            DODT_HIP_CHECK(hipFuncSetAttribute(reinterpret_cast<const void*>(&correlation_sp_kernel<2>),
-                                               hipFuncAttributeMaxDynamicSharedMemorySize, kSpLds));
-            prepared = true;
-        }
-        const int n = ty * tx;
-        static const int grid_env = getenv("DODT_CORR_GRID") ? atoi(getenv("DODT_CORR_GRID")) : 0;
-        int grid = grid_env > 0 ? grid_env / 8 * 8 : 2 * ctx->num_cus / 8 * 8;
-        if (grid > 8 * dodt::ceil_div(n, 8)) grid = 8 * dodt::ceil_div(n, 8);
-        static const bool want_stamps = getenv("DODT_CORR_STAMPS") != nullptr;
-        static int* d_stamps = nullptr;
-        if (want_stamps && !d_stamps) {
-            DODT_HIP_CHECK(hipMalloc(&d_stamps, 64 * sizeof(int)));
-            DODT_HIP_CHECK(hipMemset(d_stamps, 0, 64 * sizeof(int)));
-        }
-        if (halves == 2)
-            hipLaunchKernelGGL(correlation_sp_kernel<2>, dim3(grid), dim3(512), kSpLds, ctx->stream,
-                               d_a, d_b, H, W, max_displacement, pad, OH, OW, d_list, n, d_out, d_stamps);
-        else
-            hipLaunchKernelGGL(correlation_sp_kernel<1>, dim3(grid), dim3(256), kSpLds, ctx->stream,
-                               d_a, d_b, H, W, max_displacement, pad, OH, OW, d_list, n, d_out, d_stamps);
-        DODT_LAUNCH_CHECK();
-        if (want_stamps) {
-            int h[64];
-            (void)hipStreamSynchronize(ctx->stream);
-            (void)hipMemcpy(h, d_stamps, sizeof(h), hipMemcpyDeviceToHost);
-            fprintf(stderr, "[dodt] correlation, workgroup 9, us per phase: wait copies | barrier | arithmetic | barrier | "
-                            "early copies + outputs to LDS | stores | barrier + late copies\n");
-            for (int t = 0; t < 4; ++t) {
-                fprintf(stderr, "[dodt]   tile %d:", t);
-                for (int k = 0; k < 7; ++k) fprintf(stderr, " %6.2f", (h[t * 8 + k + 1] - h[t * 8 + k]) / 100.0);
-                fprintf(stderr, "   next tile's top +%.2f\n", (h[(t + 1) * 8] - h[t * 8]) / 100.0);
-            }
-        }
+        if (int rc = launch_sp(ctx, d_a, d_b, H, W, max_displacement, pad, OH, OW, d_list, ty * tx, nullptr, d_out))
+            return rc;
         return DODT_OK;
     }
     const int R = r * stride_2;
@@ -488,3 +573,45 @@
     DODT_LAUNCH_CHECK();
     return DODT_OK;
 }
+
+namespace {
+bool sp_ok(int H, int W) {
+    return (size_t)H * W * kC * 4 < (1ull << 31) && H < 65536 * kSpT && W < 65536 * kSpT;
+}
+}
+
+extern "C" int dodt_correlation_tile_list(dodt_ctx* ctx, int OH, int OW, const float* d_boxes, int n_boxes,
+                                          const int32_t* d_box_idx, int n, const int32_t* d_n, int crop_h,
+                                          int crop_w, int32_t* d_tiles, int capacity, int32_t* d_n_tiles) {
+    DODT_REQUIRE(ctx && d_tiles && d_n_tiles && (n == 0 || d_boxes), "dodt_correlation_tile_list: NULL argument");
+    DODT_REQUIRE(OH > 0 && OW > 0 && n >= 0 && n_boxes >= 0 && crop_h > 0 && crop_w > 0,
+                 "dodt_correlation_tile_list: bad sizes");
+    const int ty = dodt::ceil_div(OH, kSpT), tx = dodt::ceil_div(OW, kSpT);
+    DODT_REQUIRE(ty * tx <= kListMaxTiles && ty < 65536 && tx < 65536,
+                 "dodt_correlation_tile_list: %d x %d tiles, at most %d", ty, tx, kListMaxTiles);
+    DODT_REQUIRE(capacity >= ty * tx, "dodt_correlation_tile_list: room for %d tiles, the map has %d", capacity,
+                 ty * tx);
+    const int* d_curve = nullptr;
+    if (int rc = sp_tile_list(ctx, ty, tx, &d_curve)) return rc;
+    hipLaunchKernelGGL(corr_tile_list_kernel, dim3(1), dim3(kListThreads), 0, ctx->stream, OH, OW, d_boxes, n_boxes,
+                       d_box_idx, n, d_n, crop_h, crop_w, d_curve, d_tiles, d_n_tiles);
+    DODT_LAUNCH_CHECK();
+    return DODT_OK;
+}
+
+extern "C" int dodt_correlation_tiles(dodt_ctx* ctx, const float* d_a, const float* d_b, int H, int W, int C,
+                                      int max_displacement, int stride_2, int pad, const int32_t* d_tiles,
+                                      int capacity, const int32_t* d_n_tiles, float* d_out) {
+    DODT_REQUIRE(ctx && d_a && d_b && d_out && d_tiles && d_n_tiles, "dodt_correlation_tiles: NULL argument");
+    DODT_REQUIRE(C == kC, "dodt_correlation_tiles: C = %d, only %d channels are supported", C, kC);
+    DODT_REQUIRE(H > 0 && W > 0 && max_displacement >= 0 && stride_2 >= 1 && pad >= 0 && capacity >= 0,
+                 "dodt_correlation_tiles: bad sizes");
+    const int OH = H + 2 * pad - 2 * max_displacement, OW = W + 2 * pad - 2 * max_displacement;
+    DODT_REQUIRE(OH >= 1 && OW >= 1, "dodt_correlation_tiles: empty output");
+    if (!(stride_2 == 2 && max_displacement / stride_2 == 2 && sp_ok(H, W))) {
+        dodt::set_error("dodt_correlation_tiles: only the 5 x 5 grid of displacements two pixels apart");
+        return DODT_ERR_UNSUPPORTED;
+    }
+    if (capacity == 0) return DODT_OK;
+    return launch_sp(ctx, d_a, d_b, H, W, max_displacement, pad, OH, OW, d_tiles, capacity, d_n_tiles, d_out);
+}
diff --git a/dodt_amd/csrc/crop.hip b/dodt_amd/csrc/crop.hip
--- a/dodt_amd/csrc/crop.hip
+++ b/dodt_amd/csrc/crop.hip
@@ -1,4 +1,5 @@
 #include "common.h"
+#include "crop_coords.h"
 
 namespace {
 
@@ -6,7 +7,7 @@
 __global__ void __launch_bounds__(256)
 crop_kernel(const float* __restrict__ img, int H, int W, int C, const float* __restrict__ boxes,
             int n, const int* __restrict__ d_n, int ch, int cw, float* __restrict__ out,
-            long long out_stride) {
+            long long out_stride, const int* __restrict__ box_idx, int n_boxes) {
     const int groups = C / VEC;
     const long long t = (long long)blockIdx.x * blockDim.x + threadIdx.x;
     const int lim = d_n ? min(*d_n, n) : n;
@@ -17,15 +18,14 @@
     const int ix = (int)(r % cw); r /= cw;
     const int iy = (int)(r % ch);
     const int b = (int)(r / ch);
-    const float4 bx = reinterpret_cast<const float4*>(boxes)[b];
-    const float y1 = bx.x, x1 = bx.y, y2 = bx.z, x2 = bx.w;
+    const int src = box_idx ? box_idx[b] : b;
+    const bool have = !box_idx || (src >= 0 && src < n_boxes);
+    const float4 bx = have ? reinterpret_cast<const float4*>(boxes)[src] : make_float4(0.f, 0.f, 0.f, 0.f);
     const float hm1 = (float)(H - 1), wm1 = (float)(W - 1);
-    const float hs = (ch > 1) ? (y2 - y1) * hm1 / (float)(ch - 1) : 0.0f;
-    const float ws = (cw > 1) ? (x2 - x1) * wm1 / (float)(cw - 1) : 0.0f;
-    const float in_y = (ch > 1) ? y1 * hm1 + (float)iy * hs : 0.5f * (y1 + y2) * hm1;
-    const float in_x = (cw > 1) ? x1 * wm1 + (float)ix * ws : 0.5f * (x1 + x2) * wm1;
+    const float in_y = dodt::crop_coord(bx.x, bx.z, H, ch, iy);
+    const float in_x = dodt::crop_coord(bx.y, bx.w, W, cw, ix);
     float* o = out + (size_t)b * out_stride + (((size_t)iy * cw + ix) * C + (size_t)g * VEC);
-    const bool ok = (in_y >= 0.0f) && (in_y <= hm1) && (in_x >= 0.0f) && (in_x <= wm1);
+    const bool ok = have && (in_y >= 0.0f) && (in_y <= hm1) && (in_x >= 0.0f) && (in_x <= wm1);
     if (!ok) {
 #pragma unroll
         for (int k = 0; k < VEC; ++k) o[k] = 0.0f;
@@ -47,6 +47,29 @@
     }
 }
 
+int launch_crop(dodt_ctx* ctx, const float* d_image, int H, int W, int C, const float* d_boxes, int n,
+                const int32_t* d_n, int crop_h, int crop_w, float* d_out, long long out_box_stride,
+                const int32_t* d_box_idx, int n_boxes) {
+    DODT_REQUIRE(ctx && d_image && d_out && (n == 0 || d_boxes),
+                 "dodt_crop_and_resize: NULL argument");
+    DODT_REQUIRE(H > 0 && W > 0 && C > 0 && crop_h > 0 && crop_w > 0 && n >= 0,
+                 "dodt_crop_and_resize: bad sizes");
+    DODT_REQUIRE(out_box_stride >= (long long)crop_h * crop_w * C,
+                 "dodt_crop_and_resize: output stride %lld shorter than a crop", out_box_stride);
+    if (n == 0) return DODT_OK;
+    const int vec = (C % 4 == 0 && out_box_stride % 4 == 0) ? 4 : 1;
+    const long long total = (long long)n * crop_h * crop_w * (C / vec);
+    const int blocks = (int)((total + 255) / 256);
+    if (vec == 4)
+        hipLaunchKernelGGL(crop_kernel<4>, dim3(blocks), dim3(256), 0, ctx->stream, d_image, H, W,
+                           C, d_boxes, n, d_n, crop_h, crop_w, d_out, out_box_stride, d_box_idx, n_boxes);
+    else
+        hipLaunchKernelGGL(crop_kernel<1>, dim3(blocks), dim3(256), 0, ctx->stream, d_image, H, W,
+                           C, d_boxes, n, d_n, crop_h, crop_w, d_out, out_box_stride, d_box_idx, n_boxes);
+    DODT_LAUNCH_CHECK();
+    return DODT_OK;
+}
+
 }
 
 extern "C" int dodt_crop_and_resize(dodt_ctx* ctx, const float* d_image, int H, int W, int C,
@@ -59,22 +82,14 @@
 extern "C" int dodt_crop_and_resize_strided(dodt_ctx* ctx, const float* d_image, int H, int W, int C,
                                             const float* d_boxes, int n, const int32_t* d_n, int crop_h,
                                             int crop_w, float* d_out, long long out_box_stride) {
-    DODT_REQUIRE(ctx && d_image && d_out && (n == 0 || d_boxes),
-                 "dodt_crop_and_resize: NULL argument");
-    DODT_REQUIRE(H > 0 && W > 0 && C > 0 && crop_h > 0 && crop_w > 0 && n >= 0,
-                 "dodt_crop_and_resize: bad sizes");
-    DODT_REQUIRE(out_box_stride >= (long long)crop_h * crop_w * C,
-                 "dodt_crop_and_resize: output stride %lld shorter than a crop", out_box_stride);
-    if (n == 0) return DODT_OK;
-    const int vec = (C % 4 == 0 && out_box_stride % 4 == 0) ? 4 : 1;
-    const long long total = (long long)n * crop_h * crop_w * (C / vec);
-    const int blocks = (int)((total + 255) / 256);
-    if (vec == 4)
-        hipLaunchKernelGGL(crop_kernel<4>, dim3(blocks), dim3(256), 0, ctx->stream, d_image, H, W,
-                           C, d_boxes, n, d_n, crop_h, crop_w, d_out, out_box_stride);
-    else
-        hipLaunchKernelGGL(crop_kernel<1>, dim3(blocks), dim3(256), 0, ctx->stream, d_image, H, W,
-                           C, d_boxes, n, d_n, crop_h, crop_w, d_out, out_box_stride);
-    DODT_LAUNCH_CHECK();
-    return DODT_OK;
+    return launch_crop(ctx, d_image, H, W, C, d_boxes, n, d_n, crop_h, crop_w, d_out, out_box_stride, nullptr, n);
 }
+
+extern "C" int dodt_crop_and_resize_indexed(dodt_ctx* ctx, const float* d_image, int H, int W, int C,
+                                            const float* d_boxes, int n_boxes, const int32_t* d_box_idx, int n,
+                                            const int32_t* d_n, int crop_h, int crop_w, float* d_out,
+                                            long long out_box_stride) {
+    DODT_REQUIRE(d_box_idx && n_boxes >= 0, "dodt_crop_and_resize_indexed: NULL index list");
+    return launch_crop(ctx, d_image, H, W, C, d_boxes, n, d_n, crop_h, crop_w, d_out, out_box_stride, d_box_idx,
+                       n_boxes);
+}
diff --git a/dodt_amd/csrc/crop_coords.h b/dodt_amd/csrc/crop_coords.h
--- /dev/null
+++ b/dodt_amd/csrc/crop_coords.h
@@ -0,0 +1,11 @@
+#pragma once
+
+namespace dodt {
+
+__device__ __forceinline__ float crop_coord(float lo, float hi, int size, int crop, int i) {
+    const float m1 = (float)(size - 1);
+    const float step = (crop > 1) ? (hi - lo) * m1 / (float)(crop - 1) : 0.0f;
+    return (crop > 1) ? lo * m1 + (float)i * step : 0.5f * (lo + hi) * m1;
+}
+
+}
diff --git a/dodt_amd/ops.py b/dodt_amd/ops.py
--- a/dodt_amd/ops.py
+++ b/dodt_amd/ops.py
@@ -159,6 +159,16 @@
         'dodt_crop_and_resize')
 
 
+def crop_and_resize_indexed(ctx, d_image, hwc, d_boxes, n_boxes, d_box_idx, n, d_n, crop_hw, d_out,
+                            out_box_stride=None):
+    if out_box_stride is None:
+        out_box_stride = int(crop_hw[0]) * int(crop_hw[1]) * int(hwc[2])
+    _lib.check(ctx.lib.dodt_crop_and_resize_indexed(
+        ctx.handle, _p(d_image), int(hwc[0]), int(hwc[1]), int(hwc[2]), _p(d_boxes), int(n_boxes),
+        _p(d_box_idx), int(n), _p(d_n), int(crop_hw[0]), int(crop_hw[1]), _p(d_out), int(out_box_stride)),
+        'dodt_crop_and_resize_indexed')
+
+
 def nms(ctx, d_boxes, d_scores, n, d_n, max_out, iou_threshold, d_sel, d_count):
     _lib.check(ctx.lib.dodt_nms(
         ctx.handle, _p(d_boxes), _p(d_scores), int(n), _p(d_n), int(max_out),
@@ -230,6 +240,14 @@
         'dodt_pack_detections')
 
 
+def pack_detections_compact(ctx, d_boxes_3d, d_scores, d_sel, d_count, max_det, frame_mark,
+                            d_rec, d_count_out, d_det_offsets=None, d_orientations=None):
+    _lib.check(ctx.lib.dodt_pack_detections_compact(
+        ctx.handle, _p(d_boxes_3d), _p(d_scores), _p(d_orientations), _p(d_det_offsets),
+        _p(d_sel), _p(d_count), int(max_det), float(frame_mark), _p(d_rec), _p(d_count_out)),
+        'dodt_pack_detections_compact')
+
+
 def fetch_i32_begin(ctx, d_src, n, slot):
     _lib.check(ctx.lib.dodt_fetch_i32_begin(ctx.handle, _p(d_src), int(n), int(slot)),
                'dodt_fetch_i32_begin')
@@ -246,6 +264,25 @@
     _lib.check(ctx.lib.dodt_correlation(
         ctx.handle, _p(d_a), _p(d_b), int(hwc[0]), int(hwc[1]), int(hwc[2]),
         int(max_displacement), int(stride_2), int(pad), _p(d_out)), 'dodt_correlation')
+
+
+def correlation_tile_list(ctx, out_hw, d_boxes, n_boxes, d_box_idx, n, d_n, crop_hw, d_tiles, capacity, d_n_tiles):
+    _lib.check(ctx.lib.dodt_correlation_tile_list(
+        ctx.handle, int(out_hw[0]), int(out_hw[1]), _p(d_boxes), int(n_boxes), _p(d_box_idx), int(n), _p(d_n),
+        int(crop_hw[0]), int(crop_hw[1]), _p(d_tiles), int(capacity), _p(d_n_tiles)), 'dodt_correlation_tile_list')
+
+
+def correlation_tiles(ctx, d_a, d_b, hwc, max_displacement, stride_2, pad, d_tiles, capacity, d_n_tiles, d_out):
+    _lib.check(ctx.lib.dodt_correlation_tiles(
+        ctx.handle, _p(d_a), _p(d_b), int(hwc[0]), int(hwc[1]), int(hwc[2]), int(max_displacement),
+        int(stride_2), int(pad), _p(d_tiles), int(capacity), _p(d_n_tiles), _p(d_out)), 'dodt_correlation_tiles')
+
+
+CORR_TILE_LIST_MAX = 8192
+
+
+def correlation_tile_capacity(out_hw):
+    return -(-int(out_hw[0]) // 16) * -(-int(out_hw[1]) // 16)
 
 
 def mean_fusion(ctx, d_a, d_b, rows, d_n, row_floats, d_out):
diff --git a/dodt_amd/pipeline.py b/dodt_amd/pipeline.py
--- a/dodt_amd/pipeline.py
+++ b/dodt_amd/pipeline.py
@@ -27,7 +27,12 @@
                  image_wh=_config.KITTI_IMAGE_WH, n_points_max=120000, rpn_nms_size=1024,
                  pairs_per_step=1, side_streams=None, head_params=None, conv_dtype='f32',
                  head_dtype='f32', reuse_streams_of=None, tail_sets=None, temporal=None, tracker=None,
-                 bev_input_skip=True, bev_frame_tables=True):
+                 bev_input_skip=True, bev_frame_tables=True, t_branch_rows=None):
+        if t_branch_rows not in (None, 'proposals', 'detections'):
+            raise ValueError("t_branch_rows must be None, 'proposals' or 'detections'")
+        self.t_branch_rows = t_branch_rows
+        self._t_form = None
+        self._caller_records = False
         self.ctx = ctx
         self.cfg = cfg
         self.p2 = np.asarray(p2, dtype=np.float64)
@@ -141,8 +146,10 @@
                                             if self.fps == 2 else None)
                                        for _ in sides] for sides, _ in self.stream_sets]
             self.head_scratch = self.head_scratch_sets[0]
-            self.corr_maps = [[ctx.empty((self.bev_fh, self.bev_fw, CORR_CH), f32) for _ in range(self.pairs)]
-                              for _ in range(2)] if self.fps == 2 else None
+            self.corr_maps = None
+            if t_branch_rows == 'detections' and self.corr_head is not None and not self._tile_list_fits():
+                raise ValueError("t_branch_rows='detections': the %d x %d map has more than %d tiles"
+                                 % (self.bev_fh, self.bev_fw, ops.CORR_TILE_LIST_MAX))
 
         FC = self.feat_c
         self.feat = [dict(
@@ -236,9 +243,45 @@
         frame = (pad_top + shape[0]) * row
         return [arr.offset(frame * f + pad_top * row, shape) for f in range(self.nf)]
 
+    def _tile_list_fits(self):
+        return ops.correlation_tile_capacity((self.bev_fh, self.bev_fw)) <= ops.CORR_TILE_LIST_MAX
+
+    def t_branch_form(self):
+        if self._t_form is not None:
+            return self._t_form
+        if self.t_branch_rows is not None:
+            return self.t_branch_rows
+        return 'detections' if self._caller_records and self._tile_list_fits() else 'proposals'
+
+    def _t_detections(self):
+        return self.corr_head is not None and self.t_branch_form() == 'detections'
+
+    def _resolve_t_branch(self):
+        if self._t_form is not None:
+            return
+        self._t_form = self.t_branch_form()
+        if self.corr_head is None:
+            return
+        ctx, f32, i32 = self.ctx, np.float32, np.int32
+        if self._t_form == 'proposals':
+            self.corr_maps = [[ctx.empty((self.bev_fh, self.bev_fw, CORR_CH), f32) for _ in range(self.pairs)]
+                              for _ in range(2)]
+            return
+        self.corr_tile_cap = ops.correlation_tile_capacity((self.bev_fh, self.bev_fw))
+        for scratch in self.head_scratch_sets:
+            for s in scratch:
+                s.update(corr_tiles=ctx.empty((self.corr_tile_cap,), i32), corr_ntiles=ctx.zeros((1,), i32))
+        for frames in self.fr2:
+            for f, b in enumerate(frames):
+                if f % 2 == 0:
+                    b.update(det_corr_rois=ctx.zeros((MAX_DET, self.corr_head.in_ld), f32),
+                             det_corr_offsets=ctx.zeros((MAX_DET, 3), f32))
+        ctx.sync()
+
     def use_record_buffers(self, rec_ptrs, cnt_ptrs):
         if len(rec_ptrs) < 2 or len(rec_ptrs) != len(cnt_ptrs):
             raise ValueError('use_record_buffers: at least two record and count buffers, as many of each')
+        self._caller_records = True
         self.rec2 = [self.ctx.wrap(p, (self.pairs, self.fps, MAX_DET, REC_COLS), np.float32)
                      for p in rec_ptrs]
         self.cnt2 = [self.ctx.wrap(p, (self.pairs, self.fps), np.int32) for p in cnt_ptrs]
@@ -335,6 +378,7 @@
         main, nf = self.ctx, self.nf
         if (heads is None) != (self.rpn_head is not None):
             raise ValueError('pass `heads` exactly when the pipeline has no head_params')
+        self._resolve_t_branch()
         if recover is not None:
             if self.temporal is None:
                 raise ValueError('recover: the pipeline has no temporal module')
@@ -478,7 +522,7 @@
     CORR_MAP_MARK = 248
 
     def _corr_on_img(self):
-        return (self.rpn_head is not None and self.fps == 2 and len(self.sides) >= 2
+        return (self.rpn_head is not None and self.fps == 2 and len(self.sides) >= 2 and not self._t_detections()
                 and not os.environ.get('DODT_PIPE_NO_CORR') and os.environ.get('DODT_PIPE_CORR_ON_F1', '1') != '0'
                 and os.environ.get('DODT_PIPE_CORR_MAP', 'img') == 'img')
 
@@ -514,8 +558,9 @@
         if self.on_records_reuse is not None:
             self.on_records_reuse(st['rslot'], sides)
         computed = heads is None
+        t_det = computed and self._t_detections()
         split_t = computed and self.fps == 2 and ns >= 2 and not os.environ.get('DODT_PIPE_NO_CORR') \
-            and os.environ.get('DODT_PIPE_CORR_ON_F1', '1') != '0'
+            and os.environ.get('DODT_PIPE_CORR_ON_F1', '1') != '0' and not t_det
         corr_img = split_t and self._corr_on_img()
         fused_tail = os.environ.get('DODT_PIPE_FUSED_TAIL', '1') != '0'
 
@@ -582,7 +627,7 @@
                                        scratch['fc'])
                 self._mark(c, st['step'], 'tail%d_fc2' % f)
                 yield 'head'
-                if pair and f % 2 == 0 and not os.environ.get('DODT_PIPE_NO_CORR'):
+                if pair and f % 2 == 0 and not os.environ.get('DODT_PIPE_NO_CORR') and not t_det:
                     if corr_img:
                         pass
                     else:
@@ -613,6 +658,29 @@
                     ops.angle_vector_to_orientation(c, h['angle_vectors'], self.P, b['top_count'],
                                                     b['orientations'])
             yield 'pack'
+            if t_det and pair and f % 2 == 0:
+                if not os.environ.get('DODT_PIPE_NO_CORR'):
+                    fb1 = feat['bev_feat'].offset(4 * bev_px * FC * (f + 1), bev_hw + (FC,))
+                    ops.correlation_tile_list(c, bev_hw, b['top_bev'], self.P, b['det_idx'], MAX_DET, b['det_count'],
+                                              (ROI, ROI), scratch['corr_tiles'], self.corr_tile_cap,
+                                              scratch['corr_ntiles'])
+                    ops.correlation_tiles(c, feat_b, fb1, bev_hw + (FC,), CORR_MAX_DISP, CORR_STRIDE2, CORR_PAD,
+                                          scratch['corr_tiles'], self.corr_tile_cap, scratch['corr_ntiles'],
+                                          scratch['corr_map'])
+                    self._mark(c, st['step'], 'tail%d_corrmap' % f)
+                    ops.crop_and_resize_indexed(c, scratch['corr_map'], bev_hw + (CORR_CH,), b['top_bev'], self.P,
+                                                b['det_idx'], MAX_DET, b['det_count'], (ROI, ROI),
+                                                b['det_corr_rois'], out_box_stride=self.corr_head.in_ld)
+                    self.corr_head.forward(c, b['det_corr_rois'], None, MAX_DET, b['det_count'],
+                                           [b['det_corr_offsets']], scratch['fc'])
+                ops.pack_detections_compact(
+                    c, b['boxes_3d'], b['det_scores'], b['det_idx'], b['det_count'], MAX_DET,
+                    float(f % self.fps),
+                    self.d_records.offset(4 * MAX_DET * REC_COLS * f, (MAX_DET, REC_COLS)),
+                    self.d_rec_counts.offset(4 * f, (1,), np.int32), d_det_offsets=b['det_corr_offsets'],
+                    d_orientations=b['orientations'] if self.box_4ca else None)
+                self._mark(c, st['step'], 'tail%d_end' % f)
+                return
             ops.pack_detections(
                 c, b['boxes_3d'], b['det_scores'], b['det_idx'], b['det_count'], MAX_DET,
                 float(f % self.fps),
@@ -625,6 +693,12 @@
             for _ in g:
                 pass
 
+        if t_det and ns >= 2:
+            for f0 in range(0, nf, 2):
+                gens = [frame(f0), frame(f0 + 1)]
+                while gens:
+                    gens = [g for g in gens if next(g, None) is not None]
+            return
         if not split_t:
             for f in range(nf):
                 drain(frame(f))
@@ -683,7 +757,8 @@
         counts = anchor_counts or self.last_anchor_counts
         return (sum(self.rpn_head.flops(a) for a in counts)
                 + self.nf * self.avod_head.flops(self.P)
-                + (self.pairs * self.corr_head.flops(self.P) if self.corr_head else 0.0))
+                + (self.pairs * self.corr_head.flops(MAX_DET if self._t_detections() else self.P)
+                   if self.corr_head else 0.0))
 
     def flops_per_pair(self):
         return self.flops_per_step() / self.pairs
diff --git a/include/dodt_hip.h b/include/dodt_hip.h
--- a/include/dodt_hip.h
+++ b/include/dodt_hip.h
@@ -149,9 +149,19 @@
 int dodt_crop_and_resize_strided(dodt_ctx* ctx, const float* d_image, int H, int W, int C,
                                  const float* d_boxes, int n, const int32_t* d_n, int crop_h,
                                  int crop_w, float* d_out, long long out_box_stride);
+int dodt_crop_and_resize_indexed(dodt_ctx* ctx, const float* d_image, int H, int W, int C,
+                                 const float* d_boxes, int n_boxes, const int32_t* d_box_idx, int n,
+                                 const int32_t* d_n, int crop_h, int crop_w, float* d_out,
+                                 long long out_box_stride);
 
 int dodt_correlation(dodt_ctx* ctx, const float* d_a, const float* d_b, int H, int W, int C,
                      int max_displacement, int stride_2, int pad, float* d_out);
+int dodt_correlation_tile_list(dodt_ctx* ctx, int OH, int OW, const float* d_boxes, int n_boxes,
+                               const int32_t* d_box_idx, int n, const int32_t* d_n, int crop_h, int crop_w,
+                               int32_t* d_tiles, int capacity, int32_t* d_n_tiles);
+int dodt_correlation_tiles(dodt_ctx* ctx, const float* d_a, const float* d_b, int H, int W, int C,
+                           int max_displacement, int stride_2, int pad, const int32_t* d_tiles, int capacity,
+                           const int32_t* d_n_tiles, float* d_out);
 
 int dodt_mean_fusion(dodt_ctx* ctx, const float* d_a, const float* d_b, int rows, const int32_t* d_n,
                      int row_floats, float* d_out);
@@ -205,6 +215,10 @@
                          const float* d_orientations, const float* d_corr_offsets,
                          const int32_t* d_sel, const int32_t* d_count, int max_det,
                          float frame_mark, float* d_rec_out, int32_t* d_count_out);
+int dodt_pack_detections_compact(dodt_ctx* ctx, const float* d_boxes_3d, const float* d_scores,
+                                 const float* d_orientations, const float* d_det_offsets,
+                                 const int32_t* d_sel, const int32_t* d_count, int max_det,
+                                 float frame_mark, float* d_rec_out, int32_t* d_count_out);
 int dodt_box_4c_decode(dodt_ctx* ctx, const float* d_top_anchors, const float* d_offsets,
                        int n, const int32_t* d_n, const float plane[4],
                        const float bev_extents[4], float* d_boxes_3d_out,
```

Measured after the change: 419.1 (median of 6 runs). 9.3% higher.
